# alazarteka/Self-Forcing

Hardware: AMD Instinct MI355X
Metric: decoded frames/sec/node, Wan-1.3B 832x480 4-step AR rollout (higher is better)
Workload: dtype bf16

## Files before the change

include/sf_hip.h:

```cpp
#ifndef SF_HIP_H
#define SF_HIP_H

#include <stddef.h>
#include <stdint.h>

#ifdef __cplusplus
extern "C" {
#endif

#define SF_HIP_ABI_VERSION 10

int sf_abi_version(void);
const char* sf_last_error(void);

enum sf_epilogue {
  SF_EPI_BIAS = 0,
  SF_EPI_BIAS_GELU = 1,
  SF_EPI_BIAS_RESID = 2,
  SF_EPI_BIAS_GATE_RESID = 3,
  SF_EPI_F32 = 4
};

typedef struct sf_gemm_args {
  const void* a;
  const void* w;
  const void* bias;
  void* out;
  const void* resid;
  const void* gate_mod;
  const void* gate_e0;
  int64_t gate_group_stride;
  int32_t rows_per_group;
  int32_t M, N, K;
  int32_t lda, ldw, ldo, ldr;
  int32_t epilogue;
  int32_t batch;
  int64_t a_bstride, w_bstride, o_bstride, r_bstride;
  int32_t structure;
} sf_gemm_args;

enum sf_gemm_structure { SF_GEMM_AUTO = 0, SF_GEMM_T128 = 1 ,
                         SF_GEMM_PP256 = 2 ,
                         SF_GEMM_PP128 = 3 ,
                         SF_GEMM_PP224 = 4, SF_GEMM_PP192 = 5  };

int sf_gemm_bf16(const sf_gemm_args* args, void* stream);

#define SF_FP8_AMAX_PARTS 1024
int sf_quantize_fp8(const void* x, int ldx, int M, int K, int rows_per_segment, void* q_out, float* scale_out, void* stream);

int sf_gemm_fp8(const sf_gemm_args* args, const float* a_scale, int rows_per_segment, const float* w_scale, void* stream);

int sf_small_linear_fp8(const void* x, const void* w_q, const float* w_scale, const void* bias, void* out, int M, int N, int K,
                        int rows_per_segment, int act_in, int act_out, void* stream);

int sf_small_linear(const void* x, const void* w, const void* bias, void* out, int M, int N, int K,
                    int act_in, int act_out, void* stream);

int sf_sinusoid_embedding(const void* t, int t_is_int64, void* out, int n, int dim, void* stream);

int sf_layernorm_modulate(const void* x, void* out, int M, int C, float eps, const void* mod_shift,
                          const void* mod_scale, const void* e0_shift, const void* e0_scale,
                          int64_t e0_group_stride, int rows_per_group, void* stream);

int sf_layernorm_affine(const void* x, const void* weight, const void* bias, void* out, int M, int C,
                        float eps, void* stream);

int sf_rmsnorm(const void* x, int ldx, const void* weight, void* out, int ldo, int M, int C, float eps,
               void* stream);

int sf_qkv_norm_rope_cache(const void* qkv, const void* norm_q_w, const void* norm_k_w, void* q_out,
                           void* k_cache, void* v_cache, const float* rope_cos, const float* rope_sin,
                           int B, int f, int h, int w, int C, int num_heads, int64_t cache_tokens,
                           int write_start, int start_frame, float eps, void* stream);

int sf_kv_evict(void* cache, int B, int64_t cache_tokens, int row_elems, int sink, int evict, int keep,
                void* scratch, size_t scratch_bytes, void* stream);

int sf_attention(const void* q, const void* k, const void* v, void* out, int B, int H, int Lq, int Lk,
                 int64_t q_stride, int64_t q_bstride, int64_t kv_stride, int64_t kv_bstride,
                 int64_t o_stride, int64_t o_bstride, void* stream);

enum sf_attn_structure { SF_ATTN_AUTO = 0, SF_ATTN_R64 = 1, SF_ATTN_W8 = 2, SF_ATTN_W4 = 3 };
int sf_attention_ex(const void* q, const void* k, const void* v, void* out, int B, int H, int Lq, int Lk,
                    int64_t q_stride, int64_t q_bstride, int64_t kv_stride, int64_t kv_bstride,
                    int64_t o_stride, int64_t o_bstride, int structure, void* stream);

int sf_attention_fold(const void* q, const void* k, const void* v, void* out, int B, int H, int Lq, int Lk,
                      int64_t q_stride, int64_t q_bstride, int64_t kv_stride, int64_t kv_bstride,
                      int64_t o_stride, int64_t o_bstride, int structure, const int32_t* keys, const float* log2w,
                      void* stream);

int sf_attention_accum(const void* q, const void* k, const void* v, void* out, int B, int H, int Lq, int Lk,
                       int64_t q_stride, int64_t q_bstride, int64_t kv_stride, int64_t kv_bstride,
                       int64_t o_stride, int64_t o_bstride, int structure, void* stream);

int sf_cross_fold_scan(const void* const* ck_cache_host, const void* const* cv_cache_host, int layers, int B, int text_len,
                       int row_elems, int32_t* keys, float* log2w, void* stream);

int sf_patchify(const void* x, void* cols, int B, int F, int Cin, int H, int W, void* stream);

int sf_unpatchify_x0(const void* head_out, const void* xt, const void* timestep, int t_is_int64,
                     const float* sigmas, const float* timesteps, int n_table, void* flow, void* x0,
                     int B, int F, int groups, int Cout, int H, int W, void* stream);

int sf_add_noise(const void* x0, const void* eps, const void* timestep, int t_is_int64,
                 const float* sigmas, const float* timesteps, int n_table, void* out, int n_outer,
                 int64_t inner, void* stream);

#define SF_LINCOMB_MAX 6
int sf_lincomb_bf16(void* out, const void* const* xs, const float* coefs, int n_terms, int64_t n, void* stream);

typedef struct sf_layer_weights {
  const void* modulation;
  const void *norm3_w, *norm3_b;
  const void *qkv_w, *qkv_b;
  const void *norm_q_w, *norm_k_w;
  const void *o_w, *o_b;
  const void *cq_w, *cq_b;
  const void *ckv_w, *ckv_b;
  const void *cnorm_q_w, *cnorm_k_w;
  const void *co_w, *co_b;
  const void *ffn0_w, *ffn0_b;
  const void *ffn2_w, *ffn2_b;
} sf_layer_weights;

typedef struct sf_model {
  int32_t dim, ffn_dim, num_heads, num_layers, in_dim, out_dim, freq_dim, text_dim, text_len;
  float eps;
  const void *patch_w, *patch_b;
  const void *text0_w, *text0_b, *text2_w, *text2_b;
  const void *time0_w, *time0_b, *time2_w, *time2_b;
  const void *tproj_w, *tproj_b;
  const void *head_w, *head_b;
  const void* head_mod;
  const void *pose_w, *pose_b;
  int32_t pose_dim;
  const sf_layer_weights* layers_host;
  const float *rope_cos, *rope_sin;
  const float *sched_sigmas, *sched_timesteps;
  int32_t n_table;
  int32_t fp8;
  const void *text0_q, *text2_q, *time0_q, *time2_q, *tproj_q, *head_q, *pose_q;
  const float *text0_s, *text2_s, *time0_s, *time2_s, *tproj_s, *head_s, *pose_s;
  const struct sf_layer_fp8* layers_fp8_host;
} sf_model;

typedef struct sf_layer_fp8 {
  const void *qkv_q, *o_q, *cq_q, *ckv_q, *co_q, *ffn0_q, *ffn2_q;
  const float *qkv_s, *o_s, *cq_s, *ckv_s, *co_s, *ffn0_s, *ffn2_s;
} sf_layer_fp8;

typedef struct sf_forward_args {
  int32_t batch, frames, lat_h, lat_w;
  int32_t groups;
  const void* noisy;
  const void* timestep;
  int32_t t_is_int64;
  const void* prompt_embeds;
  int32_t init_cross;
  const void* add_condition;
  void* const* k_cache_host;
  void* const* v_cache_host;
  void* const* ck_cache_host;
  void* const* cv_cache_host;
  int64_t cache_tokens;
  int32_t sink_tokens, evict, keep;
  int32_t write_start;
  int32_t attn_start, attn_end;
  int32_t start_frame;
  void* evict_scratch;
  size_t evict_scratch_bytes;
  int32_t cache_only;
  void* flow_out;
  void* x0_out;
  void* workspace;
  size_t workspace_bytes;
  void* kv_index_out;
  int64_t global_end;
} sf_forward_args;

size_t sf_dit_workspace_bytes(const sf_model* model, int batch, int frames, int lat_h, int lat_w,
                              int groups);
int sf_dit_forward(const sf_model* model, const sf_forward_args* args, void* stream);
int sf_dit_forward_pair(const sf_model* model, const sf_forward_args* context_pass, const sf_forward_args* next_pass,
                        void* stream);
int sf_dit_forward_fold(const sf_model* model, const sf_forward_args* args, int32_t* cross_keys, float* cross_log2w,
                        void* stream);
int sf_dit_forward_pair_fold(const sf_model* model, const sf_forward_args* context_pass, const sf_forward_args* next_pass,
                             const int32_t* cross_keys, const float* cross_log2w, void* stream);


int sf_patchify_i2v(const void* x, const void* y, void* cols, int B, int F, int x_channels, int y_channels, int pad_channels,
                    int H, int W, int64_t y_bstride, int64_t y_cstride, int64_t y_fstride, void* stream);

int sf_layernorm_rows(const void* x, const void* weight, const void* bias, void* out, int M, int C, float eps, void* stream);

int sf_i2v_assemble_y(const void* latent, const void* ref_map, void* y, int frames, int mask_channels, int latent_channels, int h, int w,
                      int64_t y_cstride, int64_t y_fstride, int first_is_frame0, void* stream);

typedef struct sf_i2v_layer {
  const void *kvimg_w, *kvimg_b;
  const void* norm_k_img_w;
} sf_i2v_layer;

typedef struct sf_i2v_model {
  int32_t clip_dim, clip_len;
  float img_eps;
  const void *img_ln0_w, *img_ln0_b;
  const void *img_fc1_w, *img_fc1_b;
  const void *img_fc2_w, *img_fc2_b;
  const void *img_ln1_w, *img_ln1_b;
  const sf_i2v_layer* layers_host;
} sf_i2v_model;

typedef struct sf_i2v_args {
  const void* clip_feature;
  const void* y;
  int64_t y_bstride, y_cstride, y_fstride;
  int32_t y_channels;
  void* const* kimg_cache_host;
  void* const* vimg_cache_host;
} sf_i2v_args;

size_t sf_dit_i2v_workspace_bytes(const sf_model* model, const sf_i2v_model* i2v_model, int batch, int frames, int lat_h,
                                  int lat_w, int groups);
int sf_dit_forward_i2v(const sf_model* model, const sf_i2v_model* i2v_model, const sf_forward_args* args, const sf_i2v_args* i2v_args,
                       int32_t* cross_keys, float* cross_log2w, void* stream);


enum sf_conv_epilogue {
  SF_CONV_BIAS = 0,
  SF_CONV_BIAS_RESID = 1,
  SF_CONV_BIAS_CLAMP_F32 = 2
};

typedef struct sf_conv_args {
  const void* x;
  const void* w;
  const void* bias;
  void* out;
  const void* resid;
  float* out_f32;
  int32_t Tout, H, W;
  int32_t Hin, Win;
  int32_t Cin, Cout;
  int32_t kt, kh, kw;
  int32_t upsample;
  int32_t t_in_offset;
  int32_t ldw, ldo, ldr;
  int32_t out_frame_offset;
  int32_t interleave_c;
  int32_t epilogue;
  int32_t structure;
  void* norm_out;
  const void* norm_gamma;
  int32_t norm_ld, norm_frame_offset;
  int32_t stride_hw, stride_t;
} sf_conv_args;

enum sf_conv_structure { SF_CONV_AUTO = 0, SF_CONV_IGEMM = 1 ,
                         SF_CONV_HALO = 2  };

int sf_conv_igemm(const sf_conv_args* args, void* stream);
int sf_conv_pick_nt(int cout);

int sf_rmsnorm_silu_cl(const void* x, const void* gamma, void* out, int64_t rows, int C, int silu,
                       void* stream);

int sf_softmax_rows(const float* s, int64_t lds, void* p, int64_t ldp, int rows, int cols,
                    int cols_padded, float scale, void* stream);

int sf_vae_prepare_latent(const void* latent, const float* mean, const float* std, const void* conv2_w,
                          const void* conv2_b, void* out, int z, int h, int w, int c_pad, void* stream);

typedef struct sf_vae_conv {
  const void* w;
  const void* bias;
  int32_t cin, cout, kt, kh, kw, ldw;
} sf_vae_conv;

typedef struct sf_vae_resblock {
  const void* gamma1;
  const void* gamma2;
  sf_vae_conv conv1;
  sf_vae_conv conv2;
  sf_vae_conv shortcut;
} sf_vae_resblock;

#define SF_VAE_MAX_STAGES 4

typedef struct sf_vae_model {
  int32_t z_dim;
  int32_t n_stages;
  int32_t res_per_stage;
  int32_t temporal_up[SF_VAE_MAX_STAGES];
  const float* latent_mean;
  const float* latent_std;
  const void *conv2_w, *conv2_b;
  sf_vae_conv conv1;
  sf_vae_resblock mid0, mid2;
  const void* attn_gamma;
  const void *attn_qk_w, *attn_qk_b;
  const void *attn_v_w, *attn_v_b;
  const void *attn_proj_w, *attn_proj_b;
  const sf_vae_resblock* res_host;
  sf_vae_conv time_conv[SF_VAE_MAX_STAGES];
  sf_vae_conv up_conv[SF_VAE_MAX_STAGES];
  const void* head_gamma;
  sf_vae_conv head_conv;
} sf_vae_model;

size_t sf_vae_state_bytes(const sf_vae_model* model, int lat_h, int lat_w, int window_frames);
size_t sf_vae_scratch_bytes(const sf_vae_model* model, int lat_h, int lat_w, int window_frames);
int sf_vae_reset(const sf_vae_model* model, void* state, size_t state_bytes, int lat_h, int lat_w,
                 int window_frames, void* stream);
int sf_vae_decode_frames(const sf_vae_model* model, void* state, size_t state_bytes, void* scratch,
                         size_t scratch_bytes, const void* latent_frames, int lat_h, int lat_w, int window_frames,
                         int frame_index, int n_frames, int window, int history_at, float* pixels_out, void* stream);


int sf_vae_prepare_pixels(const void* pixels, int is_f32, int64_t c_stride, void* out, int T, int H, int W, int c_pad,
                          void* stream);

int sf_vae_finish_latent(const void* head_out, int ld_in, int cin, const void* conv1_w, int ld_w, const void* conv1_b,
                         const float* mean, const float* std, float* out, int T, int z, int h, int w, void* stream);

typedef struct sf_vae_encoder {
  int32_t z_dim;
  int32_t n_stages;
  int32_t res_per_stage;
  int32_t temporal_down[SF_VAE_MAX_STAGES];
  const float* latent_mean;
  const float* latent_std;
  const void *conv1_w, *conv1_b;
  sf_vae_conv in_conv;
  const sf_vae_resblock* res_host;
  sf_vae_conv down_conv[SF_VAE_MAX_STAGES];
  sf_vae_conv time_conv[SF_VAE_MAX_STAGES];
  sf_vae_resblock mid0, mid2;
  const void* attn_gamma;
  const void *attn_qk_w, *attn_qk_b;
  const void *attn_v_w, *attn_v_b;
  const void *attn_proj_w, *attn_proj_b;
// ... 284 lines not shown
```

self-forcing_amd/_lib.py:

```python
from __future__ import annotations

import ctypes as C
import os
import subprocess
from typing import Optional

os.environ.setdefault("ROC_SIGNAL_POOL_SIZE", "1024")

_HERE = os.path.dirname(os.path.abspath(__file__))
CSRC = os.path.join(_HERE, "csrc")
LIB_PATH = os.environ.get("SF_HIP_LIB") or os.path.join(CSRC, "libsf_hip.so")

ABI_VERSION = 10
FP8_AMAX_PARTS = 1024

EPI_BIAS, EPI_BIAS_GELU, EPI_BIAS_RESID, EPI_BIAS_GATE_RESID, EPI_F32 = 0, 1, 2, 3, 4
CONV_BIAS, CONV_BIAS_RESID, CONV_BIAS_CLAMP_F32 = 0, 1, 2
VAE_MAX_STAGES = 4
TAEHV_EPILOGUES = {"bias_relu": 0, "bias_resid_relu": 1, "plain": 2, "relu": 3, "head_f32": 4, "latent_f32": 5}
TAEHV_STAGES, TAEHV_BLOCKS = 3, 3
TAEHV_PIXEL_DTYPES = {"bfloat16": 0, "float32": 1}
POSE_DTYPES = {"uint8": 0, "float32": 1, "bfloat16": 2}
POSE_CONVS = 6
JPEG_SUBSAMPLINGS = {"420": 0, "444": 1}
JPEG_DTYPES = {"uint8": 0, "float32": 1, "bfloat16": 2}
JPEG_RANGES = {(-1, 1): 0, (0, 1): 1}
JPEG_STATUS = {1: "an interval outgrew its worst-case slot", 2: "a coefficient is outside the baseline range",
               4: "the files do not fit the output buffer"}
CLIP_DTYPES = {"float32": 0, "bfloat16": 1}
ACT_NONE, ACT_SILU, ACT_GELU = 0, 1, 2
ATTN_STRUCTURES = {"auto": 0, "r64": 1, "w8": 2, "w4": 3}
CONV_STRUCTURES = {"auto": 0, "igemm": 1, "halo": 2}
GEMM_STRUCTURES = {"auto": 0, "t128": 1, "pp256": 2, "pp128": 3, "pp224": 4, "pp192": 5}


class GemmArgs(C.Structure):
    _fields_ = [
        ("a", C.c_void_p), ("w", C.c_void_p), ("bias", C.c_void_p), ("out", C.c_void_p),
        ("resid", C.c_void_p), ("gate_mod", C.c_void_p), ("gate_e0", C.c_void_p),
        ("gate_group_stride", C.c_int64), ("rows_per_group", C.c_int32),
        ("M", C.c_int32), ("N", C.c_int32), ("K", C.c_int32),
        ("lda", C.c_int32), ("ldw", C.c_int32), ("ldo", C.c_int32), ("ldr", C.c_int32),
        ("epilogue", C.c_int32), ("batch", C.c_int32),
        ("a_bstride", C.c_int64), ("w_bstride", C.c_int64), ("o_bstride", C.c_int64), ("r_bstride", C.c_int64),
        ("structure", C.c_int32),
    ]


class LayerWeights(C.Structure):
    _fields_ = [(n, C.c_void_p) for n in (
        "modulation", "norm3_w", "norm3_b", "qkv_w", "qkv_b", "norm_q_w", "norm_k_w", "o_w", "o_b",
        "cq_w", "cq_b", "ckv_w", "ckv_b", "cnorm_q_w", "cnorm_k_w", "co_w", "co_b",
        "ffn0_w", "ffn0_b", "ffn2_w", "ffn2_b")]


class LayerFp8(C.Structure):
    _fields_ = [(n, C.c_void_p) for n in (
        "qkv_q", "o_q", "cq_q", "ckv_q", "co_q", "ffn0_q", "ffn2_q",
        "qkv_s", "o_s", "cq_s", "ckv_s", "co_s", "ffn0_s", "ffn2_s")]


FP8_MODEL_LINEARS = (("text0", ("text_embedding.0",)), ("text2", ("text_embedding.2",)), ("time0", ("time_embedding.0",)),
                     ("time2", ("time_embedding.2",)), ("tproj", ("time_projection.1",)), ("head", ("head.head",)),
                     ("pose", ("pose_proj",)))
FP8_LAYER_LINEARS = (("qkv", ("self_attn.q", "self_attn.k", "self_attn.v")), ("o", ("self_attn.o",)), ("cq", ("cross_attn.q",)),
                     ("ckv", ("cross_attn.k", "cross_attn.v")), ("co", ("cross_attn.o",)), ("ffn0", ("ffn.0",)), ("ffn2", ("ffn.2",)))


class Model(C.Structure):
    _fields_ = (
        [(n, C.c_int32) for n in ("dim", "ffn_dim", "num_heads", "num_layers", "in_dim", "out_dim",
                                  "freq_dim", "text_dim", "text_len")]
        + [("eps", C.c_float)]
        + [(n, C.c_void_p) for n in ("patch_w", "patch_b", "text0_w", "text0_b", "text2_w", "text2_b",
                                     "time0_w", "time0_b", "time2_w", "time2_b", "tproj_w", "tproj_b",
                                     "head_w", "head_b", "head_mod", "pose_w", "pose_b")]
        + [("pose_dim", C.c_int32)]
        + [("layers_host", C.POINTER(LayerWeights)),
           ("rope_cos", C.c_void_p), ("rope_sin", C.c_void_p),
           ("sched_sigmas", C.c_void_p), ("sched_timesteps", C.c_void_p),
           ("n_table", C.c_int32)]
        + [("fp8", C.c_int32)]
        + [(n + "_q", C.c_void_p) for n, _ in FP8_MODEL_LINEARS]
        + [(n + "_s", C.c_void_p) for n, _ in FP8_MODEL_LINEARS]
        + [("layers_fp8_host", C.POINTER(LayerFp8))]
    )


class ForwardArgs(C.Structure):
    _fields_ = [
        ("batch", C.c_int32), ("frames", C.c_int32), ("lat_h", C.c_int32), ("lat_w", C.c_int32),
        ("groups", C.c_int32),
        ("noisy", C.c_void_p), ("timestep", C.c_void_p), ("t_is_int64", C.c_int32),
        ("prompt_embeds", C.c_void_p), ("init_cross", C.c_int32), ("add_condition", C.c_void_p),
        ("k_cache_host", C.POINTER(C.c_void_p)), ("v_cache_host", C.POINTER(C.c_void_p)),
        ("ck_cache_host", C.POINTER(C.c_void_p)), ("cv_cache_host", C.POINTER(C.c_void_p)),
        ("cache_tokens", C.c_int64),
        ("sink_tokens", C.c_int32), ("evict", C.c_int32), ("keep", C.c_int32),
        ("write_start", C.c_int32), ("attn_start", C.c_int32), ("attn_end", C.c_int32),
        ("start_frame", C.c_int32),
        ("evict_scratch", C.c_void_p), ("evict_scratch_bytes", C.c_size_t),
        ("cache_only", C.c_int32),
        ("flow_out", C.c_void_p), ("x0_out", C.c_void_p),
        ("workspace", C.c_void_p), ("workspace_bytes", C.c_size_t),
        ("kv_index_out", C.c_void_p), ("global_end", C.c_int64),
    ]


class I2VLayer(C.Structure):
    _fields_ = [(n, C.c_void_p) for n in ("kvimg_w", "kvimg_b", "norm_k_img_w")]


class I2VModel(C.Structure):
    _fields_ = ([("clip_dim", C.c_int32), ("clip_len", C.c_int32), ("img_eps", C.c_float)]
                + [(n, C.c_void_p) for n in ("img_ln0_w", "img_ln0_b", "img_fc1_w", "img_fc1_b", "img_fc2_w", "img_fc2_b",
                                             "img_ln1_w", "img_ln1_b")]
                + [("layers_host", C.POINTER(I2VLayer))])


class I2VArgs(C.Structure):
    _fields_ = [("clip_feature", C.c_void_p), ("y", C.c_void_p),
                ("y_bstride", C.c_int64), ("y_cstride", C.c_int64), ("y_fstride", C.c_int64), ("y_channels", C.c_int32),
                ("kimg_cache_host", C.POINTER(C.c_void_p)), ("vimg_cache_host", C.POINTER(C.c_void_p))]


class ConvArgs(C.Structure):
    _fields_ = (
        [(n, C.c_void_p) for n in ("x", "w", "bias", "out", "resid", "out_f32")]
        + [(n, C.c_int32) for n in ("Tout", "H", "W", "Hin", "Win", "Cin", "Cout", "kt", "kh", "kw", "upsample",
                                    "t_in_offset", "ldw", "ldo", "ldr", "out_frame_offset", "interleave_c", "epilogue", "structure")]
        + [("norm_out", C.c_void_p), ("norm_gamma", C.c_void_p), ("norm_ld", C.c_int32), ("norm_frame_offset", C.c_int32)]
        + [("stride_hw", C.c_int32), ("stride_t", C.c_int32)]
    )


class VaeConv(C.Structure):
    _fields_ = [("w", C.c_void_p), ("bias", C.c_void_p)] + [(n, C.c_int32) for n in ("cin", "cout", "kt", "kh", "kw", "ldw")]


class VaeResBlock(C.Structure):
    _fields_ = [("gamma1", C.c_void_p), ("gamma2", C.c_void_p), ("conv1", VaeConv), ("conv2", VaeConv), ("shortcut", VaeConv)]


class VaeModel(C.Structure):
    _fields_ = [
        ("z_dim", C.c_int32), ("n_stages", C.c_int32), ("res_per_stage", C.c_int32),
        ("temporal_up", C.c_int32 * VAE_MAX_STAGES),
        ("latent_mean", C.c_void_p), ("latent_std", C.c_void_p), ("conv2_w", C.c_void_p), ("conv2_b", C.c_void_p),
        ("conv1", VaeConv), ("mid0", VaeResBlock), ("mid2", VaeResBlock),
        ("attn_gamma", C.c_void_p), ("attn_qk_w", C.c_void_p), ("attn_qk_b", C.c_void_p),
        ("attn_v_w", C.c_void_p), ("attn_v_b", C.c_void_p), ("attn_proj_w", C.c_void_p), ("attn_proj_b", C.c_void_p),
        ("res_host", C.POINTER(VaeResBlock)),
        ("time_conv", VaeConv * VAE_MAX_STAGES), ("up_conv", VaeConv * VAE_MAX_STAGES),
        ("head_gamma", C.c_void_p), ("head_conv", VaeConv),
    ]


class VaeEncoder(C.Structure):
    _fields_ = [
        ("z_dim", C.c_int32), ("n_stages", C.c_int32), ("res_per_stage", C.c_int32),
        ("temporal_down", C.c_int32 * VAE_MAX_STAGES),
        ("latent_mean", C.c_void_p), ("latent_std", C.c_void_p), ("conv1_w", C.c_void_p), ("conv1_b", C.c_void_p),
        ("in_conv", VaeConv), ("res_host", C.POINTER(VaeResBlock)),
        ("down_conv", VaeConv * VAE_MAX_STAGES), ("time_conv", VaeConv * VAE_MAX_STAGES),
        ("mid0", VaeResBlock), ("mid2", VaeResBlock),
        ("attn_gamma", C.c_void_p), ("attn_qk_w", C.c_void_p), ("attn_qk_b", C.c_void_p),
        ("attn_v_w", C.c_void_p), ("attn_v_b", C.c_void_p), ("attn_proj_w", C.c_void_p), ("attn_proj_b", C.c_void_p),
        ("head_gamma", C.c_void_p), ("head_conv", VaeConv),
    ]


class TaehvConvArgs(C.Structure):
    _fields_ = ([(n, C.c_void_p) for n in ("x", "w", "bias", "out", "resid", "out_f32")]
                + [(n, C.c_int32) for n in ("Tout", "H", "W", "Cin", "Cout", "kt", "upsample", "ldw", "ldo", "ldr", "tgrow", "epilogue", "clamp")])


class TaehvLayer(C.Structure):
    _fields_ = [("w", C.c_void_p), ("bias", C.c_void_p)] + [(n, C.c_int32) for n in ("cin", "cout", "kt", "ldw")]


class TaehvModel(C.Structure):
    _fields_ = [("z_dim", C.c_int32), ("in_conv", TaehvLayer), ("block", ((TaehvLayer * 3) * TAEHV_BLOCKS) * TAEHV_STAGES),
                ("exit_conv", TaehvLayer * TAEHV_STAGES), ("tgrow", C.c_int32 * TAEHV_STAGES), ("head", TaehvLayer)]


class TaehvDownConvArgs(C.Structure):
    _fields_ = ([(n, C.c_void_p) for n in ("x", "w", "out")]
                + [(n, C.c_int32) for n in ("Tout", "H", "W", "Cin", "Cout", "kt", "ldw", "ldo")])


class TaehvEncoder(C.Structure):
    _fields_ = [("stem", TaehvLayer), ("down", TaehvLayer * TAEHV_STAGES), ("block", ((TaehvLayer * 3) * TAEHV_BLOCKS) * TAEHV_STAGES),
                ("head", TaehvLayer)]


class PoseConvArgs(C.Structure):
    _fields_ = ([(n, C.c_void_p) for n in ("x", "w", "bias", "out")]
                + [(n, C.c_int32) for n in ("T", "H", "W", "Cin", "Cout", "kt", "stride_t", "stride_s", "ldw", "ldo", "silu")])


class PoseWindow(C.Structure):
    _fields_ = [(n, C.c_int32) for n in ("x_t0", "t_end", "closed", "t_out0", "n_out")]


class PosePushPlan(C.Structure):
    _fields_ = [("first", C.c_int32 * (POSE_CONVS + 1)), ("count", C.c_int32 * (POSE_CONVS + 1))]


class PoseLayer(C.Structure):
    _fields_ = [("w", C.c_void_p), ("bias", C.c_void_p)] + [(n, C.c_int32) for n in ("cin", "cout", "kt", "stride_t", "stride_s", "ldw", "silu")]


class PoseModel(C.Structure):
    _fields_ = [("conv", PoseLayer * POSE_CONVS), ("embed_w", C.c_void_p), ("embed_b", C.c_void_p), ("pose_dim", C.c_int32),
                ("ref_conv", PoseLayer * POSE_CONVS)]


class T5Layer(C.Structure):
    _fields_ = [(n, C.c_void_p) for n in ("norm1_w", "qk_w", "v_w", "o_w", "norm2_w", "gate_w", "fc1_w", "fc2_w", "pos_emb")]


class T5Model(C.Structure):
    _fields_ = ([(n, C.c_int32) for n in ("vocab", "dim", "dim_attn", "dim_ffn", "num_heads", "num_layers", "num_buckets")]
                + [("eps", C.c_float), ("token_embedding", C.c_void_p), ("layers_host", C.POINTER(T5Layer)),
                   ("final_norm_w", C.c_void_p)])


class ClipLayer(C.Structure):
    _fields_ = [(n, C.c_void_p) for n in ("norm1_w", "norm1_b", "qkv_w", "qkv_b", "proj_w", "proj_b", "norm2_w", "norm2_b",
                                          "fc1_w", "fc1_b", "fc2_w", "fc2_b")]


class ClipModel(C.Structure):
    _fields_ = ([(n, C.c_int32) for n in ("image_size", "patch", "dim", "heads", "mlp_dim", "layers_built")]
                + [("eps", C.c_float)]
                + [(n, C.c_void_p) for n in ("patch_w", "cls", "pos", "pre_norm_w", "pre_norm_b")]
                + [("layers_host", C.POINTER(ClipLayer))])


_vp, _i, _i64, _f, _sz = C.c_void_p, C.c_int, C.c_int64, C.c_float, C.c_size_t
SIGNATURES = {
    "sf_abi_version": (C.c_int, []),
    "sf_last_error": (C.c_char_p, []),
    "sf_gemm_bf16": (C.c_int, [C.POINTER(GemmArgs), _vp]),
    "sf_small_linear": (C.c_int, [_vp, _vp, _vp, _vp, _i, _i, _i, _i, _i, _vp]),
    "sf_quantize_fp8": (C.c_int, [_vp, _i, _i, _i, _i, _vp, _vp, _vp]),
    "sf_gemm_fp8": (C.c_int, [C.POINTER(GemmArgs), _vp, _i, _vp, _vp]),
    "sf_small_linear_fp8": (C.c_int, [_vp, _vp, _vp, _vp, _vp, _i, _i, _i, _i, _i, _i, _vp]),
    "sf_sinusoid_embedding": (C.c_int, [_vp, _i, _vp, _i, _i, _vp]),
    "sf_layernorm_modulate": (C.c_int, [_vp, _vp, _i, _i, _f, _vp, _vp, _vp, _vp, _i64, _i, _vp]),
    "sf_layernorm_affine": (C.c_int, [_vp, _vp, _vp, _vp, _i, _i, _f, _vp]),
    "sf_rmsnorm": (C.c_int, [_vp, _i, _vp, _vp, _i, _i, _i, _f, _vp]),
    "sf_qkv_norm_rope_cache": (C.c_int, [_vp, _vp, _vp, _vp, _vp, _vp, _vp, _vp, _i, _i, _i, _i, _i, _i, _i64,
                                         _i, _i, _f, _vp]),
    "sf_kv_evict": (C.c_int, [_vp, _i, _i64, _i, _i, _i, _i, _vp, _sz, _vp]),
    "sf_attention": (C.c_int, [_vp, _vp, _vp, _vp, _i, _i, _i, _i, _i64, _i64, _i64, _i64, _i64, _i64, _vp]),
    "sf_attention_ex": (C.c_int, [_vp, _vp, _vp, _vp, _i, _i, _i, _i, _i64, _i64, _i64, _i64, _i64, _i64, _i, _vp]),
    "sf_attention_fold": (C.c_int, [_vp, _vp, _vp, _vp, _i, _i, _i, _i, _i64, _i64, _i64, _i64, _i64, _i64, _i, _vp, _vp, _vp]),
    "sf_attention_accum": (C.c_int, [_vp, _vp, _vp, _vp, _i, _i, _i, _i, _i64, _i64, _i64, _i64, _i64, _i64, _i, _vp]),
    "sf_cross_fold_scan": (C.c_int, [C.POINTER(C.c_void_p), C.POINTER(C.c_void_p), _i, _i, _i, _i, _vp, _vp, _vp]),
    "sf_patchify": (C.c_int, [_vp, _vp, _i, _i, _i, _i, _i, _vp]),
    "sf_unpatchify_x0": (C.c_int, [_vp, _vp, _vp, _i, _vp, _vp, _i, _vp, _vp, _i, _i, _i, _i, _i, _i, _vp]),
    "sf_add_noise": (C.c_int, [_vp, _vp, _vp, _i, _vp, _vp, _i, _vp, _i, _i64, _vp]),
    "sf_lincomb_bf16": (C.c_int, [_vp, C.POINTER(C.c_void_p), C.POINTER(C.c_float), _i, _i64, _vp]),
    "sf_dit_workspace_bytes": (C.c_size_t, [C.POINTER(Model), _i, _i, _i, _i, _i]),
    "sf_dit_forward": (C.c_int, [C.POINTER(Model), C.POINTER(ForwardArgs), _vp]),
    "sf_dit_forward_pair": (C.c_int, [C.POINTER(Model), C.POINTER(ForwardArgs), C.POINTER(ForwardArgs), _vp]),
    "sf_dit_forward_fold": (C.c_int, [C.POINTER(Model), C.POINTER(ForwardArgs), _vp, _vp, _vp]),
    "sf_dit_forward_pair_fold": (C.c_int, [C.POINTER(Model), C.POINTER(ForwardArgs), C.POINTER(ForwardArgs), _vp, _vp, _vp]),
    "sf_patchify_i2v": (C.c_int, [_vp, _vp, _vp, _i, _i, _i, _i, _i, _i, _i, _i64, _i64, _i64, _vp]),
    "sf_layernorm_rows": (C.c_int, [_vp, _vp, _vp, _vp, _i, _i, _f, _vp]),
    "sf_i2v_assemble_y": (C.c_int, [_vp, _vp, _vp, _i, _i, _i, _i, _i, _i64, _i64, _i, _vp]),
    "sf_dit_i2v_workspace_bytes": (C.c_size_t, [C.POINTER(Model), C.POINTER(I2VModel), _i, _i, _i, _i, _i]),
    "sf_dit_forward_i2v": (C.c_int, [C.POINTER(Model), C.POINTER(I2VModel), C.POINTER(ForwardArgs), C.POINTER(I2VArgs), _vp, _vp, _vp]),
    "sf_conv_igemm": (C.c_int, [C.POINTER(ConvArgs), _vp]),
    "sf_conv_pick_nt": (C.c_int, [_i]),
    "sf_rmsnorm_silu_cl": (C.c_int, [_vp, _vp, _vp, _i64, _i, _i, _vp]),
    "sf_softmax_rows": (C.c_int, [_vp, _i64, _vp, _i64, _i, _i, _i, _f, _vp]),
    "sf_vae_prepare_latent": (C.c_int, [_vp, _vp, _vp, _vp, _vp, _vp, _i, _i, _i, _i, _vp]),
    "sf_vae_state_bytes": (C.c_size_t, [C.POINTER(VaeModel), _i, _i, _i]),
    "sf_vae_scratch_bytes": (C.c_size_t, [C.POINTER(VaeModel), _i, _i, _i]),
    "sf_vae_reset": (C.c_int, [C.POINTER(VaeModel), _vp, _sz, _i, _i, _i, _vp]),
    "sf_vae_decode_frames": (C.c_int, [C.POINTER(VaeModel), _vp, _sz, _vp, _sz, _vp, _i, _i, _i, _i, _i, _i, _i, _vp, _vp]),
    "sf_vae_prepare_pixels": (C.c_int, [_vp, _i, _i64, _vp, _i, _i, _i, _i, _vp]),
    "sf_vae_finish_latent": (C.c_int, [_vp, _i, _i, _vp, _i, _vp, _vp, _vp, _vp, _i, _i, _i, _i, _vp]),
    "sf_vae_encode_state_bytes": (C.c_size_t, [C.POINTER(VaeEncoder), _i, _i, _i]),
    "sf_vae_encode_scratch_bytes": (C.c_size_t, [C.POINTER(VaeEncoder), _i, _i, _i]),
    "sf_vae_encode_reset": (C.c_int, [C.POINTER(VaeEncoder), _vp, _sz, _i, _i, _i, _vp]),
    "sf_vae_encode_frames": (C.c_int, [C.POINTER(VaeEncoder), _vp, _sz, _vp, _sz, _vp, _i, _i64, _i, _i, _i, _i, _i, _i, _i, _vp,
                                       _vp]),
    "sf_taehv_conv": (C.c_int, [C.POINTER(TaehvConvArgs), _vp]),
    "sf_taehv_pick_nt": (C.c_int, [_i]),
    "sf_taehv_prepare_latent": (C.c_int, [_vp, _vp, _i, _i, _i, _i, _i, _vp]),
    "sf_taehv_state_bytes": (C.c_size_t, [C.POINTER(TaehvModel), _i, _i]),
    "sf_taehv_scratch_bytes": (C.c_size_t, [C.POINTER(TaehvModel), _i, _i, _i]),
    "sf_taehv_reset": (C.c_int, [C.POINTER(TaehvModel), _vp, _sz, _i, _i, _vp]),
    "sf_taehv_decode_frames": (C.c_int, [C.POINTER(TaehvModel), _vp, _sz, _vp, _sz, _vp, _i, _i, _i, _i, _vp, _vp]),
    "sf_taehv_encode_stem": (C.c_int, [_vp, _i, _i64, _i, _i, _i, _i, _vp, _vp, _vp, _vp]),
    "sf_taehv_down_conv": (C.c_int, [C.POINTER(TaehvDownConvArgs), _vp]),
    "sf_taehv_encode_state_bytes": (C.c_size_t, [C.POINTER(TaehvEncoder), _i, _i]),
    "sf_taehv_encode_scratch_bytes": (C.c_size_t, [C.POINTER(TaehvEncoder), _i, _i, _i]),
    "sf_taehv_encode_reset": (C.c_int, [C.POINTER(TaehvEncoder), _vp, _sz, _i, _i, _vp]),
    "sf_taehv_encode_frames": (C.c_int, [C.POINTER(TaehvEncoder), _vp, _sz, _vp, _sz, _vp, _i, _i64, _i, _i, _i, _i, _vp, _vp]),
    "sf_pose_out_size": (C.c_int, [_i, _i, _i]),
    "sf_pose_conv": (C.c_int, [C.POINTER(PoseConvArgs), _vp]),
    "sf_pose_conv_window": (C.c_int, [C.POINTER(PoseConvArgs), C.POINTER(PoseWindow), _vp]),
    "sf_pose_prepare": (C.c_int, [_vp, _i, _i, _i, _i, _i, _i, _vp, _vp]),
    "sf_pose_patch_embed": (C.c_int, [_vp, _i, _i, _i, _vp, _vp, _i, _vp, _vp, _vp]),
    "sf_pose_scratch_bytes": (C.c_size_t, [C.POINTER(PoseModel), _i, _i, _i]),
    "sf_pose_embed": (C.c_int, [C.POINTER(PoseModel), _vp, _i, _i, _i, _i, _vp, _sz, _vp, _i64, _vp]),
    "sf_pose_embed_ref": (C.c_int, [C.POINTER(PoseModel), _vp, _i, _i, _i, _vp, _sz, _vp, _vp]),
    "sf_pose_stream_plan": (C.c_int, [_i, _i, _i, C.POINTER(PosePushPlan)]),
    "sf_pose_stream_state_bytes": (C.c_size_t, [C.POINTER(PoseModel), _i, _i]),
    "sf_pose_stream_scratch_bytes": (C.c_size_t, [C.POINTER(PoseModel), _i, _i, _i]),
    "sf_pose_stream_push": (C.c_int, [C.POINTER(PoseModel), _vp, _i, _vp, _i, _i, _i, _i, _i, _vp, _sz, _vp, _i64, C.POINTER(C.c_int32), _vp]),
    "sf_jpeg_workspace_bytes": (C.c_size_t, [_i, _i, _i, _i, _i]),
    "sf_jpeg_transform": (C.c_int, [_vp, _i, _i, _i, _i, _i, _i, _i, _vp, _vp]),
    "sf_jpeg_entropy": (C.c_int, [_vp, _i, _i, _i, _i, _i, _i, _vp, _sz, _vp, _sz, _vp, _vp, _vp]),
    "sf_jpeg_encode_frames": (C.c_int, [_vp, _i, _i, _i, _i, _i, _i, _i, _i, _vp, _sz, _vp, _sz, _vp, _vp, _vp]),
    "sf_embedding_gather": (C.c_int, [_vp, _vp, _vp, _i, _i, _i, _vp]),
    "sf_t5_softmax_bias": (C.c_int, [_vp, _vp, _vp, _vp, _vp, _i, _i, _i, _vp]),
    "sf_mul_bf16": (C.c_int, [_vp, _vp, _vp, _i64, _vp]),
    "sf_zero_masked_rows": (C.c_int, [_vp, _vp, _i, _i, _vp]),
    "sf_t5_workspace_bytes": (C.c_size_t, [C.POINTER(T5Model), _i, _i]),
    "sf_t5_encode": (C.c_int, [C.POINTER(T5Model), _vp, _vp, _vp, _i, _i, _vp, _vp, _sz, _vp]),
    "sf_clip_preprocess": (C.c_int, [_vp, _i, _i, _i, _i, _i, _i, _i, _vp, _vp]),
    "sf_clip_embed_norm": (C.c_int, [_vp, _vp, _vp, _vp, _vp, _vp, _vp, _vp, _vp, _i, _i, _i, _f, _vp]),
    "sf_clip_add_layernorm": (C.c_int, [_vp, _vp, _vp, _vp, _vp, _i, _i, _f, _vp]),
    "sf_clip_attention": (C.c_int, [_vp, _vp, _i, _i, _i, _vp]),
    "sf_clip_gelu": (C.c_int, [_vp, _vp, _i64, _vp]),
    "sf_clip_workspace_bytes": (C.c_size_t, [C.POINTER(ClipModel), _i]),
    "sf_clip_encode": (C.c_int, [C.POINTER(ClipModel), _vp, _i, _i, _i, _i, _vp, _vp, _sz, _vp]),
    "sf_probe_mfma": (C.c_int, [_i, _i, _i, _vp, _vp, C.POINTER(C.c_double), _vp]),
    "sf_probe_copy": (C.c_int, [_vp, _vp, _sz, _vp]),
}

_lib: Optional[C.CDLL] = None


class SfHipError(RuntimeError):
    pass


def build(verbose: bool = False) -> str:
    cmd = ["make", "-C", CSRC, "-j8"]
    res = subprocess.run(cmd, capture_output=True, text=True)
    if verbose or res.returncode != 0:
        print(res.stdout)
        print(res.stderr)
    if res.returncode != 0:
        raise SfHipError(f"building {LIB_PATH} failed (exit {res.returncode})")
    return LIB_PATH


def lib() -> C.CDLL:
    global _lib
    if _lib is not None:
        return _lib
    if not os.path.exists(LIB_PATH):
        raise SfHipError(
            f"{LIB_PATH} not found: the HIP extension is not built. Run "
            f"`python -c 'import __graft_entry__ as g; g.build()'` (or `make -C {CSRC}`). "
            "There is no CPU/eager fallback for this path.")
    handle = C.CDLL(LIB_PATH)
    for name, (res, args) in SIGNATURES.items():
        fn = getattr(handle, name)
        fn.restype = res
        fn.argtypes = args
    ver = handle.sf_abi_version()
    if ver != ABI_VERSION:
        raise SfHipError(f"{LIB_PATH}: ABI version {ver}, expected {ABI_VERSION}; rebuild")
    _lib = handle
    return handle


def check(rc: int, what: str = "") -> None:
    if rc != 0:
        msg = lib().sf_last_error()
        raise SfHipError(f"{what or 'sf_hip'} failed (rc={rc}): {msg.decode() if msg else '?'}")
```

self-forcing_amd/csrc/dit_forward.hip:

```cpp
#include <algorithm>
#include "sf_host.h"

int sf_internal_write_kv_indices(void* buf, int layers, int64_t global_end, int64_t local_end, void* stream);

namespace {

struct Work {
  void *x, *xn, *qkv, *q, *att, *hbuf, *cols, *headout, *sin, *etmp, *e, *e0, *ctx1, *ctx;
  void* xq;
  float* xs;
  size_t total;
};

constexpr int FP8_MAX_SEGMENTS = 8;

Work carve(const sf_model* m, void* ws, int B, int F, int lat_h, int lat_w, int groups) {
  const size_t M = (size_t)B * F * (lat_h / 2) * (lat_w / 2);
  const size_t C = m->dim, BG = (size_t)B * groups, T = (size_t)B * m->text_len;
  Carve c(ws);
  Work w;
  w.x = c.take(M * C * 2);
  w.xn = c.take(M * C * 2);
  w.qkv = c.take(M * 3 * C * 2);
  w.q = c.take(M * C * 2);
  w.att = c.take(M * C * 2);
  w.hbuf = c.take(M * (size_t)m->ffn_dim * 2);
  w.cols = c.take(M * (size_t)m->in_dim * 4 * 2);
  w.headout = c.take(M * (size_t)m->out_dim * 4 * 2);
  w.sin = c.take(BG * m->freq_dim * 2);
  w.etmp = c.take(BG * C * 2);
  w.e = c.take(BG * C * 2);
  w.e0 = c.take(BG * 6 * C * 2);
  w.ctx1 = c.take(T * C * 2);
  w.ctx = c.take(T * C * 2);
  w.xq = nullptr;
  w.xs = nullptr;
  if (m->fp8) {
    const size_t pose = m->pose_dim > 0 ? (size_t)m->pose_dim : C;
    const size_t widest_tok = std::max({(size_t)m->ffn_dim, C, pose}), widest_txt = std::max((size_t)m->text_dim, C);
    w.xq = c.take(std::max(M * widest_tok, T * widest_txt));
    w.xs = (float*)c.take(FP8_MAX_SEGMENTS * (1 + SF_FP8_AMAX_PARTS) * sizeof(float));
  }
  w.total = c.off;
  return w;
}

inline const char* bptr(const void* p, size_t elems) { return (const char*)p + elems * 2; }

struct I2V {
  const sf_i2v_model* m;
  const sf_i2v_args* a;
};
struct ImgWork {
  void *t0, *t1, *ctx;
  size_t total;
};
ImgWork carve_img(const sf_model* m, const sf_i2v_model* im, void* ws, size_t base, int B) {
  const size_t R = (size_t)B * im->clip_len;
  Carve c(ws);
  c.off = base;
  ImgWork w;
  w.t0 = c.take(R * im->clip_dim * 2);
  w.t1 = c.take(R * im->clip_dim * 2);
  w.ctx = c.take(2 * R * (size_t)m->dim * 2);
  w.total = c.off;
  return w;
}

}

extern "C" size_t sf_dit_workspace_bytes(const sf_model* model, int batch, int frames, int lat_h, int lat_w, int groups) {
  if (!model || batch <= 0 || frames <= 0 || lat_h <= 0 || lat_w <= 0 || groups <= 0) return 0;
  return carve(model, nullptr, batch, frames, lat_h, lat_w, groups).total;
}

static int forward_passes(const sf_model* m, const sf_forward_args* const* ps, int np, int32_t* cross_keys, float* cross_log2w, void* stream,
                          const I2V* iv = nullptr) {
  SF_CHECK((cross_keys == nullptr) == (cross_log2w == nullptr), "sf_dit_forward: cross_keys and cross_log2w come together");
  const sf_forward_args* a = ps[0];
  SF_CHECK(m && a, "sf_dit_forward: null argument");
  if (iv) {
    SF_CHECK(np == 1, "sf_dit_forward_i2v: the two-pass call is not built for the i2v model type");
    SF_CHECK(!m->fp8, "sf_dit_forward_i2v: fp8 Linears are not built for the i2v model type");
    SF_CHECK(iv->m->layers_host && iv->m->clip_len > 0 && iv->m->clip_dim > 0 && iv->m->clip_dim % 64 == 0,
             "sf_dit_forward_i2v: bad image context shape (clip_len=%d, clip_dim=%d: a positive multiple of 64)", iv->m->clip_len, iv->m->clip_dim);
    SF_CHECK(iv->a->y, "sf_dit_forward_i2v: y is missing (an i2v generator needs clip_feature and y)");
    SF_CHECK(m->in_dim >= m->out_dim + iv->a->y_channels && iv->a->y_channels > 0 && (m->in_dim * 4) % 64 == 0,
             "sf_dit_forward_i2v: %d latent + %d conditioning channels do not fit the padded in_dim %d", m->out_dim, iv->a->y_channels, m->in_dim);
    SF_CHECK(iv->a->kimg_cache_host && iv->a->vimg_cache_host, "sf_dit_forward_i2v: null image cache table");
    SF_CHECK(!a->init_cross || iv->a->clip_feature, "sf_dit_forward_i2v: init_cross needs clip_feature");
  }
  SF_CHECK(m->layers_host && m->num_layers > 0, "sf_dit_forward: model has no layers");
  SF_CHECK(m->dim == m->num_heads * 128, "sf_dit_forward: head_dim must be 128 (dim=%d heads=%d)", m->dim, m->num_heads);
  SF_CHECK(a->batch > 0 && a->frames > 0 && a->groups > 0, "sf_dit_forward: empty input");
  SF_CHECK(a->lat_h % 2 == 0 && a->lat_w % 2 == 0, "sf_dit_forward: latent size must be even");
  const int B = a->batch, F = a->frames, h = a->lat_h / 2, w = a->lat_w / 2;
  const int L = F * h * w, M = B * L, C = m->dim, G = a->groups, BG = B * G;
  const int Mt = np * M, BGt = np * BG;
  SF_CHECK(F % G == 0, "sf_dit_forward: frames=%d not divisible by timestep groups=%d", F, G);
  const int rpg = L / G;
  SF_CHECK(BGt <= 32, "sf_dit_forward: passes*batch*groups=%d exceeds the small-linear limit of 32", BGt);
  int first_full = np;
  for (int p = 0; p < np; ++p) {
    const sf_forward_args* q = ps[p];
    SF_CHECK(q, "sf_dit_forward: null pass");
    SF_CHECK(q->batch == B && q->frames == F && q->lat_h == a->lat_h && q->lat_w == a->lat_w && q->groups == G,
             "sf_dit_forward: the passes of one call must share batch, frames, latent size and timestep groups");
    SF_CHECK(q->k_cache_host == a->k_cache_host && q->v_cache_host == a->v_cache_host && q->ck_cache_host == a->ck_cache_host &&
             q->cv_cache_host == a->cv_cache_host && q->cache_tokens == a->cache_tokens, "sf_dit_forward: the passes of one call must share their caches");
    SF_CHECK(q->noisy && q->timestep, "sf_dit_forward: null tensor");
    SF_CHECK(q->cache_only || (q->flow_out && q->x0_out), "sf_dit_forward: null output tensor");
    SF_CHECK(q->attn_start >= 0 && q->attn_end > q->attn_start && q->attn_end <= q->cache_tokens, "sf_dit_forward: bad attention window [%d, %d) of %lld",
             q->attn_start, q->attn_end, (long long)q->cache_tokens);
    SF_CHECK(q->write_start >= 0 && (int64_t)q->write_start + L <= q->cache_tokens,
             "sf_dit_forward: KV cache overflow: write_start=%d + %d new tokens > capacity %lld", q->write_start, L, (long long)q->cache_tokens);
    SF_CHECK(q->write_start + L == q->attn_end, "sf_dit_forward: the new tokens must end the attention window");
    if (q->evict > 0) SF_CHECK(q->evict_scratch && q->keep >= 0, "sf_dit_forward: eviction needs evict_scratch");
    SF_CHECK(np == 1 || !q->init_cross, "sf_dit_forward_pair: the cross-attention cache must be initialised by an earlier single pass");
    if (!q->cache_only && first_full == np) first_full = p;
    SF_CHECK(!(q->cache_only && first_full != np), "sf_dit_forward_pair: cache_only passes must come first");
  }
  SF_CHECK(a->k_cache_host && a->v_cache_host && a->ck_cache_host && a->cv_cache_host, "sf_dit_forward: null cache table");
  const Work ws = carve(m, a->workspace, np * B, F, a->lat_h, a->lat_w, G);
  const size_t ws_need = iv ? carve_img(m, iv->m, nullptr, ws.total, B).total : ws.total;
  SF_CHECK(a->workspace && a->workspace_bytes >= ws_need, "sf_dit_forward: workspace too small (%zu < %zu)", a->workspace_bytes, ws_need);
  SF_CHECK(!a->init_cross || a->prompt_embeds, "sf_dit_forward: init_cross needs prompt_embeds");

  const bool f8 = m->fp8 != 0;
  static const sf_layer_fp8 no_fp8 = {};
  SF_CHECK(!f8 || m->layers_fp8_host, "sf_dit_forward: fp8 model without per-layer fp8 weights");
  auto run = [&](const Gemm& g) -> int { return f8 ? g.fp8(ws.xq, ws.xs, stream) : g.bf16(stream); };
  auto lin = [&](const Gemm& g) -> int {
    if (f8) SF_TRY(sf_quantize_fp8(g.g.a, g.g.lda, g.g.M, g.g.K, g.rows_per_segment, ws.xq, ws.xs, stream));
    return run(g);
  };
  auto small = [&](const void* x, const void* w16, const void* w8, const float* s8, const void* bias, void* out, int N, int K, int act_in,
                   int act_out) -> int {
    if (!f8) return sf_small_linear(x, w16, bias, out, BGt, N, K, act_in, act_out, stream);
    return sf_small_linear_fp8(x, w8, s8, bias, out, BGt, N, K, BG, act_in, act_out, stream);
  };

  const int Kp = m->in_dim * 4, Nh = m->out_dim * 4;
  const long cache_b = (long)a->cache_tokens * C;
  const long ctx_b = (long)m->text_len * C;
  const sf_forward_args* last = ps[np - 1];
  auto finish_indices = [&]() -> int {
    if (last->kv_index_out) return sf_internal_write_kv_indices(last->kv_index_out, m->num_layers, last->global_end, last->attn_end, stream);
    return 0;
  };

  if (iv)
    SF_TRY(sf_patchify_i2v(a->noisy, iv->a->y, ws.cols, B, F, m->out_dim, iv->a->y_channels, m->in_dim, a->lat_h, a->lat_w, iv->a->y_bstride,
                           iv->a->y_cstride, iv->a->y_fstride, stream));
  else
    for (int p = 0; p < np; ++p)
      SF_TRY(sf_patchify(ps[p]->noisy, (void*)bptr(ws.cols, (size_t)p * M * Kp), B, F, m->in_dim, a->lat_h, a->lat_w, stream));
  SF_TRY(Gemm(ws.cols, Kp, m->patch_w, Kp, ws.x, C, Mt, C, Kp).bias(m->patch_b).bf16(stream));

  for (int p = 0; p < np; ++p) {
    if (!ps[p]->add_condition) continue;
    void* xp = (void*)bptr(ws.x, (size_t)p * M * C);
    if (m->pose_w || (f8 && m->pose_q)) {
      SF_CHECK(m->pose_dim > 0, "sf_dit_forward: pose_proj weights without pose_dim");
      SF_TRY(lin(Gemm(ps[p]->add_condition, m->pose_dim, m->pose_w, m->pose_dim, xp, C, M, C, m->pose_dim).bias(m->pose_b)
                     .epi(SF_EPI_BIAS_RESID).resid(xp, C).fp8w(m->pose_q, m->pose_s, M)));
    } else {
      SF_CHECK(m->pose_dim == C, "sf_dit_forward: add_condition without pose_proj weights needs pose_dim == dim (%d != %d)", m->pose_dim, C);
      const void* terms[2] = {xp, ps[p]->add_condition};
      const float ones[2] = {1.0f, 1.0f};
      SF_TRY(sf_lincomb_bf16(xp, terms, ones, 2, (int64_t)M * C, stream));
    }
  }

  for (int p = 0; p < np; ++p)
    SF_TRY(sf_sinusoid_embedding(ps[p]->timestep, ps[p]->t_is_int64, (void*)bptr(ws.sin, (size_t)p * BG * m->freq_dim), BG, m->freq_dim, stream));
  SF_TRY(small(ws.sin, m->time0_w, m->time0_q, m->time0_s, m->time0_b, ws.etmp, C, m->freq_dim, 0, 1));
  SF_TRY(small(ws.etmp, m->time2_w, m->time2_q, m->time2_s, m->time2_b, ws.e, C, C, 0, 0));
  SF_TRY(small(ws.e, m->tproj_w, m->tproj_q, m->tproj_s, m->tproj_b, ws.e0, 6 * C, C, 1, 0));

  if (a->init_cross) {
    const int T = B * m->text_len;
    SF_TRY(lin(Gemm(a->prompt_embeds, m->text_dim, m->text0_w, m->text_dim, ws.ctx1, C, T, C, m->text_dim).bias(m->text0_b).epi(SF_EPI_BIAS_GELU)
                   .fp8w(m->text0_q, m->text0_s, T)));
    SF_TRY(lin(Gemm(ws.ctx1, C, m->text2_w, C, ws.ctx, C, T, C, C).bias(m->text2_b).fp8w(m->text2_q, m->text2_s, T)));
    if (f8) SF_TRY(sf_quantize_fp8(ws.ctx, C, T, C, T, ws.xq, ws.xs, stream));
    for (int l = 0; l < m->num_layers; ++l) {
      const sf_layer_weights& lw = m->layers_host[l];
      const sf_layer_fp8& lq = f8 ? m->layers_fp8_host[l] : no_fp8;
      SF_TRY(run(Gemm(ws.ctx, C, lw.ckv_w, C, a->ck_cache_host[l], C, T, C, C).bias(lw.ckv_b).fp8w(lq.ckv_q, lq.ckv_s, T)));
      SF_TRY(sf_rmsnorm(a->ck_cache_host[l], C, lw.cnorm_k_w, a->ck_cache_host[l], C, T, C, m->eps, stream));
      SF_TRY(run(Gemm(ws.ctx, C, bptr(lw.ckv_w, (size_t)C * C), C, a->cv_cache_host[l], C, T, C, C).bias(bptr(lw.ckv_b, C))
                     .fp8w(f8 ? (const char*)lq.ckv_q + (size_t)C * C : nullptr, f8 ? lq.ckv_s + C : nullptr, T)));
    }
    if (cross_keys) SF_TRY(sf_cross_fold_scan(a->ck_cache_host, a->cv_cache_host, m->num_layers, B, m->text_len, C, cross_keys, cross_log2w, stream));
    if (iv) {
      const sf_i2v_model* im = iv->m;
      const ImgWork iw = carve_img(m, im, a->workspace, ws.total, B);
      const int R = B * im->clip_len, D = im->clip_dim;
      void* ctx_raw = iw.ctx;
      void* ctx_img = (void*)bptr(iw.ctx, (size_t)R * C);
      SF_TRY(sf_layernorm_rows(iv->a->clip_feature, im->img_ln0_w, im->img_ln0_b, iw.t0, R, D, im->img_eps, stream));
      SF_TRY(Gemm(iw.t0, D, im->img_fc1_w, D, iw.t1, D, R, D, D).bias(im->img_fc1_b).bf16(stream));
      SF_TRY(sf_clip_gelu(iw.t1, iw.t1, (int64_t)R * D, stream));
      SF_TRY(Gemm(iw.t1, D, im->img_fc2_w, D, ctx_raw, C, R, C, D).bias(im->img_fc2_b).bf16(stream));
      SF_TRY(sf_layernorm_affine(ctx_raw, im->img_ln1_w, im->img_ln1_b, ctx_img, R, C, im->img_eps, stream));
      for (int l = 0; l < m->num_layers; ++l) {
        const sf_i2v_layer& il = im->layers_host[l];
        SF_TRY(Gemm(ctx_img, C, il.kvimg_w, C, iv->a->kimg_cache_host[l], C, R, C, C).bias(il.kvimg_b).bf16(stream));
        SF_TRY(sf_rmsnorm(iv->a->kimg_cache_host[l], C, il.norm_k_img_w, iv->a->kimg_cache_host[l], C, R, C, m->eps, stream));
        SF_TRY(Gemm(ctx_img, C, bptr(il.kvimg_w, (size_t)C * C), C, iv->a->vimg_cache_host[l], C, R, C, C).bias(bptr(il.kvimg_b, C)).bf16(stream));
      }
    }
  }

  for (int l = 0; l < m->num_layers; ++l) {
    const sf_layer_weights& lw = m->layers_host[l];
    const sf_layer_fp8& lq = f8 ? m->layers_fp8_host[l] : no_fp8;
    const void* mod = lw.modulation;
    const bool last_layer = l == m->num_layers - 1;
    SF_TRY(sf_layernorm_modulate(ws.x, ws.xn, Mt, C, m->eps, bptr(mod, 0), bptr(mod, C), bptr(ws.e0, 0), bptr(ws.e0, C), 6L * C, rpg, stream));
    SF_TRY(lin(Gemm(ws.xn, C, lw.qkv_w, C, ws.qkv, 3 * C, Mt, 3 * C, C).bias(lw.qkv_b).fp8w(lq.qkv_q, lq.qkv_s, M)));
    for (int p = 0; p < np; ++p) {
      const sf_forward_args* q = ps[p];
      const size_t roff = (size_t)p * M;
      if (q->evict > 0) {
        SF_TRY(sf_kv_evict(q->k_cache_host[l], B, q->cache_tokens, C, q->sink_tokens, q->evict, q->keep, q->evict_scratch, q->evict_scratch_bytes, stream));
        SF_TRY(sf_kv_evict(q->v_cache_host[l], B, q->cache_tokens, C, q->sink_tokens, q->evict, q->keep, q->evict_scratch, q->evict_scratch_bytes, stream));
      }
      SF_TRY(sf_qkv_norm_rope_cache(bptr(ws.qkv, roff * 3 * C), lw.norm_q_w, lw.norm_k_w, (void*)bptr(ws.q, roff * C), q->k_cache_host[l], q->v_cache_host[l],
                                    m->rope_cos, m->rope_sin, B, F, h, w, C, m->num_heads, q->cache_tokens, q->write_start, q->start_frame, m->eps, stream));
      if (q->cache_only && last_layer) continue;
      SF_TRY(sf_attention(bptr(ws.q, roff * C), bptr(q->k_cache_host[l], (size_t)q->attn_start * C), bptr(q->v_cache_host[l], (size_t)q->attn_start * C),
                          (void*)bptr(ws.att, roff * C), B, m->num_heads, L, q->attn_end - q->attn_start, C, (long)L * C, C, cache_b, C, (long)L * C, stream));
    }
    const int p0 = last_layer ? first_full : 0;
    if (p0 == np) return finish_indices();
    const size_t r0 = (size_t)p0 * M;
    const int Mr = (np - p0) * M;
    void* x = (void*)bptr(ws.x, r0 * C);
    void* xn = (void*)bptr(ws.xn, r0 * C);
    void* qb = (void*)bptr(ws.q, r0 * C);
    void* att = (void*)bptr(ws.att, r0 * C);
    void* hb = (void*)bptr(ws.hbuf, r0 * m->ffn_dim);
    const void* e0r = bptr(ws.e0, (size_t)p0 * BG * 6 * C);
    SF_TRY(lin(Gemm(att, C, lw.o_w, C, x, C, Mr, C, C).bias(lw.o_b).epi(SF_EPI_BIAS_GATE_RESID).resid(x, C)
                   .gate(bptr(mod, 2 * (size_t)C), bptr(e0r, 2 * (size_t)C), 6L * C, rpg).fp8w(lq.o_q, lq.o_s, M)));
    SF_TRY(sf_layernorm_affine(x, lw.norm3_w, lw.norm3_b, xn, Mr, C, m->eps, stream));
    SF_TRY(lin(Gemm(xn, C, lw.cq_w, C, qb, C, Mr, C, C).bias(lw.cq_b).fp8w(lq.cq_q, lq.cq_s, M)));
    SF_TRY(sf_rmsnorm(qb, C, lw.cnorm_q_w, qb, C, Mr, C, m->eps, stream));
    for (int p = p0; p < np; ++p)
      SF_TRY(sf_attention_fold(bptr(ws.q, (size_t)p * M * C), a->ck_cache_host[l], a->cv_cache_host[l], (void*)bptr(ws.att, (size_t)p * M * C), B, m->num_heads, L,
                               m->text_len, C, (long)L * C, C, ctx_b, C, (long)L * C, SF_ATTN_AUTO, cross_keys ? cross_keys + (size_t)l * B : nullptr,
                               cross_keys ? cross_log2w + (size_t)l * B : nullptr, stream));
    if (iv)
      SF_TRY(sf_attention_accum(ws.q, iv->a->kimg_cache_host[l], iv->a->vimg_cache_host[l], ws.att, B, m->num_heads, L, iv->m->clip_len, C, (long)L * C,
                                C, (long)iv->m->clip_len * C, C, (long)L * C, SF_ATTN_AUTO, stream));
    SF_TRY(lin(Gemm(att, C, lw.co_w, C, x, C, Mr, C, C).bias(lw.co_b).epi(SF_EPI_BIAS_RESID).resid(x, C).fp8w(lq.co_q, lq.co_s, M)));
    SF_TRY(sf_layernorm_modulate(x, xn, Mr, C, m->eps, bptr(mod, 3 * (size_t)C), bptr(mod, 4 * (size_t)C), bptr(e0r, 3 * (size_t)C),
                                 bptr(e0r, 4 * (size_t)C), 6L * C, rpg, stream));
    SF_TRY(lin(Gemm(xn, C, lw.ffn0_w, C, hb, m->ffn_dim, Mr, m->ffn_dim, C).bias(lw.ffn0_b).epi(SF_EPI_BIAS_GELU).fp8w(lq.ffn0_q, lq.ffn0_s, M)));
    SF_TRY(lin(Gemm(hb, m->ffn_dim, lw.ffn2_w, m->ffn_dim, x, C, Mr, C, m->ffn_dim).bias(lw.ffn2_b).epi(SF_EPI_BIAS_GATE_RESID).resid(x, C)
                   .gate(bptr(mod, 5 * (size_t)C), bptr(e0r, 5 * (size_t)C), 6L * C, rpg).fp8w(lq.ffn2_q, lq.ffn2_s, M)));
  }

  {
    const size_t r0 = (size_t)first_full * M;
    const int Mr = (np - first_full) * M;
    const void* er = bptr(ws.e, (size_t)first_full * BG * C);
    SF_TRY(sf_layernorm_modulate(bptr(ws.x, r0 * C), (void*)bptr(ws.xn, r0 * C), Mr, C, m->eps, bptr(m->head_mod, 0), bptr(m->head_mod, C), er, er, (long)C, rpg, stream));
    SF_TRY(lin(Gemm(bptr(ws.xn, r0 * C), C, m->head_w, C, (void*)bptr(ws.headout, r0 * Nh), Nh, Mr, Nh, C).bias(m->head_b)
                   .fp8w(m->head_q, m->head_s, M)));
    for (int p = first_full; p < np; ++p)
      SF_TRY(sf_unpatchify_x0(bptr(ws.headout, (size_t)p * M * Nh), ps[p]->noisy, ps[p]->timestep, ps[p]->t_is_int64, m->sched_sigmas, m->sched_timesteps, m->n_table,
                              ps[p]->flow_out, ps[p]->x0_out, B, F, G, m->out_dim, a->lat_h, a->lat_w, stream));
  }
  return finish_indices();
}

extern "C" int sf_dit_forward(const sf_model* m, const sf_forward_args* a, void* stream) {
  SF_CHECK(m && a, "sf_dit_forward: null argument");
  const sf_forward_args* one[1] = {a};
  return forward_passes(m, one, 1, nullptr, nullptr, stream);
}

extern "C" int sf_dit_forward_fold(const sf_model* m, const sf_forward_args* a, int32_t* cross_keys, float* cross_log2w, void* stream) {
  SF_CHECK(m && a, "sf_dit_forward: null argument");
  const sf_forward_args* one[1] = {a};
  return forward_passes(m, one, 1, cross_keys, cross_log2w, stream);
}

extern "C" size_t sf_dit_i2v_workspace_bytes(const sf_model* model, const sf_i2v_model* i2v_model, int batch, int frames, int lat_h, int lat_w,
                                             int groups) {
  const size_t base = sf_dit_workspace_bytes(model, batch, frames, lat_h, lat_w, groups);
  if (!base || !i2v_model || i2v_model->clip_len <= 0 || i2v_model->clip_dim <= 0) return 0;
  return carve_img(model, i2v_model, nullptr, base, batch).total;
}

extern "C" int sf_dit_forward_i2v(const sf_model* m, const sf_i2v_model* im, const sf_forward_args* a, const sf_i2v_args* ia, int32_t* cross_keys,
                                  float* cross_log2w, void* stream) {
  SF_CHECK(m && im && a && ia, "sf_dit_forward_i2v: null argument");
  const sf_forward_args* one[1] = {a};
  const I2V iv = {im, ia};
  return forward_passes(m, one, 1, cross_keys, cross_log2w, stream, &iv);
}

extern "C" int sf_dit_forward_pair_fold(const sf_model* m, const sf_forward_args* context_pass, const sf_forward_args* next_pass,
                                        const int32_t* cross_keys, const float* cross_log2w, void* stream) {
  SF_CHECK(m && context_pass && next_pass, "sf_dit_forward_pair: null argument");
  SF_CHECK(context_pass->workspace == next_pass->workspace && context_pass->workspace_bytes == next_pass->workspace_bytes,
           "sf_dit_forward_pair: both passes name the same workspace (sized for 2 x batch)");
  const sf_forward_args* two[2] = {context_pass, next_pass};
  return forward_passes(m, two, 2, const_cast<int32_t*>(cross_keys), const_cast<float*>(cross_log2w), stream);
}

extern "C" int sf_dit_forward_pair(const sf_model* m, const sf_forward_args* context_pass, const sf_forward_args* next_pass, void* stream) {
  return sf_dit_forward_pair_fold(m, context_pass, next_pass, nullptr, nullptr, stream);
}
```

self-forcing_amd/csrc/elementwise.hip:

```cpp
#include "sf_common.h"
#include "../../include/sf_hip.h"

namespace {

constexpr int ROWS_PER_BLOCK = 4;

template <int NCH>
__device__ __forceinline__ void load_row(const bf16_t* row, int lane, float (&v)[NCH][8]) {
#pragma unroll
  for (int i = 0; i < NCH; ++i) {
    const bf16x8 t = *reinterpret_cast<const bf16x8*>(row + (i * 64 + lane) * 8);
#pragma unroll
    for (int j = 0; j < 8; ++j) v[i][j] = (float)t[j];
  }
}

template <int NCH>
__device__ __forceinline__ void ln_stats(const float (&v)[NCH][8], int C, float eps, float& mean, float& rstd) {
  float s = 0.f;
#pragma unroll
  for (int i = 0; i < NCH; ++i)
#pragma unroll
    for (int j = 0; j < 8; ++j) s += v[i][j];
  mean = wave_sum(s) / (float)C;
  float q = 0.f;
#pragma unroll
  for (int i = 0; i < NCH; ++i)
#pragma unroll
    for (int j = 0; j < 8; ++j) {
      const float d = v[i][j] - mean;
      q += d * d;
    }
  rstd = rsqrtf(wave_sum(q) / (float)C + eps);
}

#ifndef SF_LN_RPW
#define SF_LN_RPW 2
#endif
template <int NCH> struct LnRows { static constexpr int value = NCH <= 4 ? SF_LN_RPW : (NCH <= 6 ? 2 : 1); };
template <int NCH, int MODE>
__global__ __launch_bounds__(64) void layernorm_kernel(const bf16_t* __restrict__ x, bf16_t* __restrict__ out,
                                                       int M, int C, float eps, const bf16_t* __restrict__ p0,
                                                       const bf16_t* __restrict__ p1, const bf16_t* __restrict__ e0_shift,
                                                       const bf16_t* __restrict__ e0_scale, long e0_group_stride,
                                                       int rows_per_group) {
  constexpr int LN_RPW = LnRows<NCH>::value;
  const int lane = threadIdx.x;
  const int row0 = blockIdx.x * LN_RPW;
  bf16x8 raw[LN_RPW][NCH];
#pragma unroll
  for (int r = 0; r < LN_RPW; ++r) {
    const long row = min(row0 + r, M - 1);
#pragma unroll
    for (int i = 0; i < NCH; ++i) raw[r][i] = *reinterpret_cast<const bf16x8*>(x + row * C + (i * 64 + lane) * 8);
  }
  bf16x8 scl[NCH], add[NCH];
  int cur_group = -1;
#pragma unroll
  for (int r = 0; r < LN_RPW; ++r) {
    const int row = row0 + r;
    if (row >= M) break;
    const int grp = MODE == 0 ? row / rows_per_group : 0;
    if (grp != cur_group) {
      cur_group = grp;
      const long goff = (long)grp * e0_group_stride;
#pragma unroll
      for (int i = 0; i < NCH; ++i) {
        const int e = (i * 64 + lane) * 8;
        if (MODE == 0) {
          const bf16x8 ms = *reinterpret_cast<const bf16x8*>(p0 + e);
          const bf16x8 mc = *reinterpret_cast<const bf16x8*>(p1 + e);
          const bf16x8 es = *reinterpret_cast<const bf16x8*>(e0_shift + goff + e);
          const bf16x8 ec = *reinterpret_cast<const bf16x8*>(e0_scale + goff + e);
#pragma unroll
          for (int j = 0; j < 8; ++j) {
            add[i][j] = (bf16_t)((float)ms[j] + (float)es[j]);
            scl[i][j] = (bf16_t)((float)mc[j] + (float)ec[j]);
          }
        } else {
          scl[i] = *reinterpret_cast<const bf16x8*>(p0 + e);
          add[i] = *reinterpret_cast<const bf16x8*>(p1 + e);
        }
      }
    }
    float v[NCH][8];
#pragma unroll
    for (int i = 0; i < NCH; ++i)
#pragma unroll
      for (int j = 0; j < 8; ++j) v[i][j] = (float)raw[r][i][j];
    float mean, rstd;
    ln_stats<NCH>(v, C, eps, mean, rstd);
#pragma unroll
    for (int i = 0; i < NCH; ++i) {
      bf16x8 o;
#pragma unroll
      for (int j = 0; j < 8; ++j)
        o[j] = (bf16_t)((v[i][j] - mean) * rstd * (MODE == 0 ? 1.0f + (float)scl[i][j] : (float)scl[i][j]) + (float)add[i][j]);
      *reinterpret_cast<bf16x8*>(out + (long)row * C + (i * 64 + lane) * 8) = o;
    }
  }
}

template <int NCH>
__global__ __launch_bounds__(256) void rmsnorm_kernel(const bf16_t* __restrict__ x, int ldx, const bf16_t* __restrict__ w,
                                                      bf16_t* __restrict__ out, int ldo, int M, int C, float eps) {
  const int lane = threadIdx.x & 63;
  const int row = blockIdx.x * ROWS_PER_BLOCK + (threadIdx.x >> 6);
  if (row >= M) return;
  float v[NCH][8];
  load_row<NCH>(x + (long)row * ldx, lane, v);
  float q = 0.f;
#pragma unroll
  for (int i = 0; i < NCH; ++i)
#pragma unroll
    for (int j = 0; j < 8; ++j) q += v[i][j] * v[i][j];
  const float r = rsqrtf(wave_sum(q) / (float)C + eps);
#pragma unroll
  for (int i = 0; i < NCH; ++i) {
    const int e = (i * 64 + lane) * 8;
    const bf16x8 wt = *reinterpret_cast<const bf16x8*>(w + e);
    bf16x8 o;
#pragma unroll
    for (int j = 0; j < 8; ++j) o[j] = (bf16_t)((float)(bf16_t)(v[i][j] * r) * (float)wt[j]);
    *reinterpret_cast<bf16x8*>(out + (long)row * ldo + e) = o;
  }
}

template <int NCH>
__global__ __launch_bounds__(256) void qkv_norm_rope_cache_kernel(
    const bf16_t* __restrict__ qkv, const bf16_t* __restrict__ wq, const bf16_t* __restrict__ wk,
    bf16_t* __restrict__ q_out, bf16_t* __restrict__ k_cache, bf16_t* __restrict__ v_cache,
    const float* __restrict__ rope_cos, const float* __restrict__ rope_sin, int rows, int L, int hgt, int wid, int C,
    long cache_tokens, int write_start, int start_frame, float eps, int c0, int c1) {
  const int lane = threadIdx.x & 63;
  const int row = blockIdx.x * ROWS_PER_BLOCK + (threadIdx.x >> 6);
  if (row >= rows) return;
  const int b = row / L, t = row - b * L;
  const int fi = t / (hgt * wid), rem = t - fi * (hgt * wid);
  const int hi = rem / wid, wi = rem - hi * wid;
  const int pos_t = start_frame + fi;
  const bf16_t* src = qkv + (long)row * 3 * C;
  const long crow = ((long)b * cache_tokens + write_start + t) * C;

#pragma unroll
  for (int i = 0; i < NCH; ++i) {
    const int e = (i * 64 + lane) * 8;
    *reinterpret_cast<u32x4*>(v_cache + crow + e) = *reinterpret_cast<const u32x4*>(src + 2 * C + e);
  }

#pragma unroll
  for (int which = 0; which < 2; ++which) {
    float v[NCH][8];
    load_row<NCH>(src + which * C, lane, v);
    float q = 0.f;
#pragma unroll
    for (int i = 0; i < NCH; ++i)
#pragma unroll
      for (int j = 0; j < 8; ++j) q += v[i][j] * v[i][j];
    const float r = rsqrtf(wave_sum(q) / (float)C + eps);
    const bf16_t* wn = which ? wk : wq;
    bf16_t* dst = which ? (k_cache + crow) : (q_out + (long)row * C);
#pragma unroll
    for (int i = 0; i < NCH; ++i) {
      const int e = (i * 64 + lane) * 8;
      const bf16x8 wt = *reinterpret_cast<const bf16x8*>(wn + e);
      const int pair0 = (e & 127) >> 1;
      bf16x8 o;
#pragma unroll
      for (int pp = 0; pp < 4; ++pp) {
        const int pj = pair0 + pp;
        const int pos = pj < c0 ? pos_t : (pj < c0 + c1 ? hi : wi);
        const float cs = rope_cos[pos * 64 + pj];
        const float sn = rope_sin[pos * 64 + pj];
        const float re = (float)(bf16_t)((float)(bf16_t)(v[i][2 * pp] * r) * (float)wt[2 * pp]);
        const float im = (float)(bf16_t)((float)(bf16_t)(v[i][2 * pp + 1] * r) * (float)wt[2 * pp + 1]);
        o[2 * pp] = (bf16_t)(re * cs - im * sn);
        o[2 * pp + 1] = (bf16_t)(re * sn + im * cs);
      }
      *reinterpret_cast<bf16x8*>(dst + e) = o;
    }
  }
}

__global__ __launch_bounds__(256) void copy_rows_kernel(const char* __restrict__ src, long src_bstride,
                                                        char* __restrict__ dst, long dst_bstride, long bytes_per_batch) {
  const long n16 = bytes_per_batch >> 4;
  const char* s = src + (long)blockIdx.y * src_bstride;
  char* d = dst + (long)blockIdx.y * dst_bstride;
  for (long i = (long)blockIdx.x * blockDim.x + threadIdx.x; i < n16; i += (long)gridDim.x * blockDim.x)
    reinterpret_cast<u32x4*>(d)[i] = reinterpret_cast<const u32x4*>(s)[i];
}

__global__ __launch_bounds__(256) void patchify_kernel(const bf16_t* __restrict__ x, bf16_t* __restrict__ cols, long total,
                                                       int Cin, int H, int W) {
  const int h2 = H >> 1, w2 = W >> 1;
  for (long i = (long)blockIdx.x * blockDim.x + threadIdx.x; i < total; i += (long)gridDim.x * blockDim.x) {
    const int cch = (int)(i % Cin);
    long r = i / Cin;
    const int ww = (int)(r % w2); r /= w2;
    const int hh = (int)(r % h2);
    const long bf = r / h2;
    const bf16_t* s = x + ((bf * Cin + cch) * H + 2 * hh) * (long)W + 2 * ww;
    bf16x4 o;
    o[0] = s[0]; o[1] = s[1]; o[2] = s[W]; o[3] = s[W + 1];
    *reinterpret_cast<bf16x4*>(cols + ((bf * h2 + hh) * w2 + ww) * (long)(Cin * 4) + cch * 4) = o;
  }
}

__device__ __forceinline__ double block_sigma_lookup(double t, const float* __restrict__ sigmas,
                                                     const float* __restrict__ timesteps, int n_table) {
  __shared__ double s_val[4];
  __shared__ int s_idx[4];
  double best = 1e300;
  int bi = 0x7fffffff;
  for (int j = threadIdx.x; j < n_table; j += blockDim.x) {
    const double d = fabs((double)timesteps[j] - t);
    if (d < best) { best = d; bi = j; }
  }
#pragma unroll
  for (int o = 32; o > 0; o >>= 1) {
    const double ob = __shfl_xor(best, o, 64);
    const int oi = __shfl_xor(bi, o, 64);
    if (ob < best || (ob == best && oi < bi)) { best = ob; bi = oi; }
  }
  const int wv = threadIdx.x >> 6;
  if ((threadIdx.x & 63) == 0) { s_val[wv] = best; s_idx[wv] = bi; }
  __syncthreads();
  best = s_val[0]; bi = s_idx[0];
  for (int k = 1; k < (int)(blockDim.x >> 6); ++k)
    if (s_val[k] < best || (s_val[k] == best && s_idx[k] < bi)) { best = s_val[k]; bi = s_idx[k]; }
  return (double)sigmas[bi];
}

__device__ __forceinline__ bf16_t double_to_bf16(double d) {
  const float f = (float)d;
  const unsigned u = __float_as_uint(f);
  if (f != f) return __builtin_bit_cast(bf16_t, (unsigned short)((u >> 16) | 0x40u));
  return __builtin_bit_cast(bf16_t, (unsigned short)((u + 0x7FFFu + ((u >> 16) & 1u)) >> 16));
}

__device__ __forceinline__ double read_timestep(const void* t, int is_i64, long idx) {
  return is_i64 ? (double)reinterpret_cast<const long long*>(t)[idx] : (double)reinterpret_cast<const float*>(t)[idx];
}

__global__ __launch_bounds__(256) void unpatchify_x0_kernel(const bf16_t* __restrict__ head_out, const bf16_t* __restrict__ xt,
                                                            const void* __restrict__ timestep, int t_is_i64,
                                                            const float* __restrict__ sigmas, const float* __restrict__ timesteps,
                                                            int n_table, bf16_t* __restrict__ flow, bf16_t* __restrict__ x0,
                                                            int F, int groups, int Cout, int H, int W) {
#pragma clang fp contract(off)
  const int bf = blockIdx.y;
  const int b = bf / F, f = bf - b * F;
  const int grp = f / (F / groups);
  const double sigma = block_sigma_lookup(read_timestep(timestep, t_is_i64, (long)b * groups + grp), sigmas, timesteps, n_table);
  const int h2 = H >> 1, w2 = W >> 1;
  const int total = Cout * H * w2;
  for (int i = blockIdx.x * blockDim.x + threadIdx.x; i < total; i += gridDim.x * blockDim.x) {
    const int ww = i % w2;
    int r = i / w2;
    const int y = r % H;
    const int cch = r / H;
    const int hh = y >> 1, pq = y & 1;
    const long tok = ((long)bf * h2 + hh) * w2 + ww;
    const bf16_t* hs = head_out + tok * (4 * Cout) + (pq * 2) * Cout + cch;
    const long o = (((long)bf * Cout + cch) * H + y) * W + 2 * ww;
    const bf16_t f0 = hs[0], f1 = hs[Cout];
    bf16x2 fo; fo[0] = f0; fo[1] = f1;
    *reinterpret_cast<bf16x2*>(flow + o) = fo;
    const bf16x2 xv = *reinterpret_cast<const bf16x2*>(xt + o);
    bf16x2 xo;
    xo[0] = double_to_bf16((double)(float)xv[0] - sigma * (double)(float)f0);
    xo[1] = double_to_bf16((double)(float)xv[1] - sigma * (double)(float)f1);
    *reinterpret_cast<bf16x2*>(x0 + o) = xo;
  }
}

__global__ __launch_bounds__(256) void add_noise_kernel(const bf16_t* __restrict__ x0, const bf16_t* __restrict__ eps,
                                                        const void* __restrict__ timestep, int t_is_i64,
                                                        const float* __restrict__ sigmas, const float* __restrict__ timesteps,
                                                        int n_table, bf16_t* __restrict__ out, long inner) {
#pragma clang fp contract(off)
  const long base = (long)blockIdx.y * inner;
  const float sigma = (float)block_sigma_lookup(read_timestep(timestep, t_is_i64, blockIdx.y), sigmas, timesteps, n_table);
  const float om = 1.0f - sigma;
  const long n8 = inner >> 3;
  for (long i = (long)blockIdx.x * blockDim.x + threadIdx.x; i < n8; i += (long)gridDim.x * blockDim.x) {
    const bf16x8 a = *reinterpret_cast<const bf16x8*>(x0 + base + i * 8);
    const bf16x8 e = *reinterpret_cast<const bf16x8*>(eps + base + i * 8);
    bf16x8 o;
#pragma unroll
    for (int j = 0; j < 8; ++j) o[j] = (bf16_t)(om * (float)a[j] + sigma * (float)e[j]);
    *reinterpret_cast<bf16x8*>(out + base + i * 8) = o;
  }
}

struct LinCombP {
  const bf16_t* x[SF_LINCOMB_MAX];
  float c[SF_LINCOMB_MAX];
  bf16_t* out;
  long n8;
  int n_terms;
};
template <int NT>
__global__ __launch_bounds__(256) void lincomb_kernel(const LinCombP p) {
#pragma clang fp contract(off)
  for (long i = (long)blockIdx.x * blockDim.x + threadIdx.x; i < p.n8; i += (long)gridDim.x * blockDim.x) {
    float acc[8];
#pragma unroll
    for (int k = 0; k < NT; ++k) {
      const bf16x8 v = *reinterpret_cast<const bf16x8*>(p.x[k] + i * 8);
#pragma unroll
      for (int j = 0; j < 8; ++j) acc[j] = k == 0 ? p.c[0] * (float)v[j] : acc[j] + p.c[k] * (float)v[j];
    }
    bf16x8 o;
#pragma unroll
    for (int j = 0; j < 8; ++j) o[j] = (bf16_t)acc[j];
    *reinterpret_cast<bf16x8*>(p.out + i * 8) = o;
  }
}

__global__ __launch_bounds__(256) void sinusoid_kernel(const void* __restrict__ t, int t_is_i64, bf16_t* __restrict__ out,
                                                       int n, int dim) {
  const int half = dim >> 1;
  const int i = blockIdx.x * blockDim.x + threadIdx.x;
  if (i >= n * half) return;
  const int r = i / half, k = i - r * half;
  const double pos = read_timestep(t, t_is_i64, r);
  const double ang = pos * pow(10000.0, -(double)k / (double)half);
  out[(long)r * dim + k] = double_to_bf16(cos(ang));
  out[(long)r * dim + half + k] = double_to_bf16(sin(ang));
}

template <int MODE>
int launch_layernorm(const bf16_t* x, bf16_t* out, int M, int C, float eps, const bf16_t* p0, const bf16_t* p1,
                     const bf16_t* e0s, const bf16_t* e0c, long gs, int rpg, hipStream_t s) {
  const dim3 block(64);
  switch (C / 512) {
#define SF_LN_CASE(N) \
  case N: hipLaunchKernelGGL((layernorm_kernel<N, MODE>), dim3((M + LnRows<N>::value - 1) / LnRows<N>::value), block, 0, s, x, out, M, C, eps, p0, p1, e0s, e0c, gs, rpg); break;
    SF_LN_CASE(1) SF_LN_CASE(2) SF_LN_CASE(3) SF_LN_CASE(4) SF_LN_CASE(5) SF_LN_CASE(6) SF_LN_CASE(8) SF_LN_CASE(10)
#undef SF_LN_CASE
    default: sf_set_error("layernorm: unsupported channel count %d", C); return -1;
  }
  return 0;
}

bool channels_ok(int C) {
  if (C % 512 != 0) return false;
  const int n = C / 512;
  return n == 1 || n == 2 || n == 3 || n == 4 || n == 5 || n == 6 || n == 8 || n == 10;
}

}

extern "C" int sf_layernorm_modulate(const void* x, void* out, int M, int C, float eps, const void* mod_shift,
                                     const void* mod_scale, const void* e0_shift, const void* e0_scale,
                                     int64_t e0_group_stride, int rows_per_group, void* stream) {
  SF_CHECK(x && out && mod_shift && mod_scale && e0_shift && e0_scale, "sf_layernorm_modulate: null tensor");
  SF_CHECK(M > 0 && channels_ok(C), "sf_layernorm_modulate: unsupported shape M=%d C=%d (C must be 512*{1,2,3,4,5,6,8,10})", M, C);
  SF_CHECK(rows_per_group > 0 && e0_group_stride % 8 == 0, "sf_layernorm_modulate: bad group layout");
  if (launch_layernorm<0>((const bf16_t*)x, (bf16_t*)out, M, C, eps, (const bf16_t*)mod_shift, (const bf16_t*)mod_scale,
                          (const bf16_t*)e0_shift, (const bf16_t*)e0_scale, e0_group_stride, rows_per_group,
                          (hipStream_t)stream) != 0)
    return -1;
  SF_HIP_LAUNCH_CHECK("sf_layernorm_modulate");
  return 0;
}

extern "C" int sf_layernorm_affine(const void* x, const void* weight, const void* bias, void* out, int M, int C,
                                   float eps, void* stream) {
  SF_CHECK(x && out && weight && bias, "sf_layernorm_affine: null tensor");
  SF_CHECK(M > 0 && channels_ok(C), "sf_layernorm_affine: unsupported shape M=%d C=%d", M, C);
  if (launch_layernorm<1>((const bf16_t*)x, (bf16_t*)out, M, C, eps, (const bf16_t*)weight, (const bf16_t*)bias, nullptr,
                          nullptr, 0, 1, (hipStream_t)stream) != 0)
    return -1;
  SF_HIP_LAUNCH_CHECK("sf_layernorm_affine");
  return 0;
}

extern "C" int sf_rmsnorm(const void* x, int ldx, const void* weight, void* out, int ldo, int M, int C, float eps,
                          void* stream) {
  SF_CHECK(x && out && weight, "sf_rmsnorm: null tensor");
  SF_CHECK(M > 0 && channels_ok(C) && ldx >= C && ldo >= C && ldx % 8 == 0 && ldo % 8 == 0, "sf_rmsnorm: unsupported shape M=%d C=%d", M, C);
  const dim3 grid((M + ROWS_PER_BLOCK - 1) / ROWS_PER_BLOCK), block(256);
  hipStream_t s = (hipStream_t)stream;
  switch (C / 512) {
#define SF_RMS_CASE(N) \
  case N: hipLaunchKernelGGL((rmsnorm_kernel<N>), grid, block, 0, s, (const bf16_t*)x, ldx, (const bf16_t*)weight, (bf16_t*)out, ldo, M, C, eps); break;
    SF_RMS_CASE(1) SF_RMS_CASE(2) SF_RMS_CASE(3) SF_RMS_CASE(4) SF_RMS_CASE(5) SF_RMS_CASE(6) SF_RMS_CASE(8) SF_RMS_CASE(10)
#undef SF_RMS_CASE
  }
  SF_HIP_LAUNCH_CHECK("sf_rmsnorm");
  return 0;
}

extern "C" int sf_qkv_norm_rope_cache(const void* qkv, const void* norm_q_w, const void* norm_k_w, void* q_out,
                                      void* k_cache, void* v_cache, const float* rope_cos, const float* rope_sin,
                                      int B, int f, int h, int w, int C, int num_heads, int64_t cache_tokens,
                                      int write_start, int start_frame, float eps, void* stream) {
  SF_CHECK(qkv && norm_q_w && norm_k_w && q_out && k_cache && v_cache && rope_cos && rope_sin, "sf_qkv_norm_rope_cache: null tensor");
  SF_CHECK(B > 0 && f > 0 && h > 0 && w > 0 && channels_ok(C), "sf_qkv_norm_rope_cache: unsupported shape");
  SF_CHECK(num_heads > 0 && C == num_heads * 128, "sf_qkv_norm_rope_cache: head_dim must be 128 (C=%d heads=%d)", C, num_heads);
  const int L = f * h * w;
  SF_CHECK(write_start >= 0 && (int64_t)write_start + L <= cache_tokens, "sf_qkv_norm_rope_cache: cache overflow: write_start=%d + L=%d > capacity=%lld",
           write_start, L, (long long)cache_tokens);
  SF_CHECK(start_frame >= 0 && start_frame + f <= 1024 && h <= 1024 && w <= 1024, "sf_qkv_norm_rope_cache: RoPE position out of the 1024-entry table");
  const int rows = B * L;
  const dim3 grid((rows + ROWS_PER_BLOCK - 1) / ROWS_PER_BLOCK), block(256);
  hipStream_t s = (hipStream_t)stream;
  const int c = 64, c1 = c / 3, c0 = c - 2 * c1;
  switch (C / 512) {
#define SF_QKV_CASE(N)                                                                                                   \
  case N: hipLaunchKernelGGL((qkv_norm_rope_cache_kernel<N>), grid, block, 0, s, (const bf16_t*)qkv, (const bf16_t*)norm_q_w, \
                             (const bf16_t*)norm_k_w, (bf16_t*)q_out, (bf16_t*)k_cache, (bf16_t*)v_cache, rope_cos, rope_sin,  \
                             rows, L, h, w, C, (long)cache_tokens, write_start, start_frame, eps, c0, c1); break;
    SF_QKV_CASE(1) SF_QKV_CASE(2) SF_QKV_CASE(3) SF_QKV_CASE(4) SF_QKV_CASE(5) SF_QKV_CASE(6) SF_QKV_CASE(8) SF_QKV_CASE(10)
#undef SF_QKV_CASE
  }
  SF_HIP_LAUNCH_CHECK("sf_qkv_norm_rope_cache");
  return 0;
}

extern "C" int sf_kv_evict(void* cache, int B, int64_t cache_tokens, int row_elems, int sink, int evict, int keep,
                           void* scratch, size_t scratch_bytes, void* stream) {
  SF_CHECK(cache && B > 0 && row_elems > 0 && (row_elems % 8) == 0, "sf_kv_evict: bad arguments");
  SF_CHECK(sink >= 0 && evict >= 0 && keep >= 0 && (int64_t)sink + evict + keep <= cache_tokens, "sf_kv_evict: window out of range");
  if (evict == 0 || keep == 0) return 0;
  const long row_b = (long)row_elems * 2;
  const long bytes = (long)keep * row_b;
  SF_CHECK(scratch && scratch_bytes >= (size_t)(bytes * B), "sf_kv_evict: scratch too small (%zu < %ld)", scratch_bytes, bytes * B);
  char* base = (char*)cache;
  const long bstride = (long)cache_tokens * row_b;
  const int gx = (int)min((long)2048, (bytes / 16 + 255) / 256);
  const dim3 grid(gx, B), block(256);
  hipStream_t s = (hipStream_t)stream;
  hipLaunchKernelGGL(copy_rows_kernel, grid, block, 0, s, base + (long)(sink + evict) * row_b, bstride, (char*)scratch, bytes, bytes);
  hipLaunchKernelGGL(copy_rows_kernel, grid, block, 0, s, (const char*)scratch, bytes, base + (long)sink * row_b, bstride, bytes);
  SF_HIP_LAUNCH_CHECK("sf_kv_evict");
  return 0;
}

extern "C" int sf_patchify(const void* x, void* cols, int B, int F, int Cin, int H, int W, void* stream) {
  SF_CHECK(x && cols && B > 0 && F > 0 && Cin > 0, "sf_patchify: bad arguments");
  SF_CHECK(H % 2 == 0 && W % 2 == 0, "sf_patchify: latent H=%d W=%d must be even (patch 2x2)", H, W);
  const long total = (long)B * F * (H / 2) * (W / 2) * Cin;
  const int gx = (int)min((long)4096, (total + 255) / 256);
  hipLaunchKernelGGL(patchify_kernel, dim3(gx), dim3(256), 0, (hipStream_t)stream, (const bf16_t*)x, (bf16_t*)cols, total, Cin, H, W);
  SF_HIP_LAUNCH_CHECK("sf_patchify");
  return 0;
}

extern "C" int sf_unpatchify_x0(const void* head_out, const void* xt, const void* timestep, int t_is_int64,
                                const float* sigmas, const float* timesteps, int n_table, void* flow, void* x0,
                                int B, int F, int groups, int Cout, int H, int W, void* stream) {
  SF_CHECK(head_out && xt && timestep && sigmas && timesteps && flow && x0, "sf_unpatchify_x0: null tensor");
  SF_CHECK(B > 0 && F > 0 && groups > 0 && F % groups == 0, "sf_unpatchify_x0: frames=%d not divisible by groups=%d", F, groups);
  SF_CHECK(H % 2 == 0 && W % 2 == 0 && n_table > 0, "sf_unpatchify_x0: bad shape");
  const int total = Cout * H * (W / 2);
  const dim3 grid(min(64, (total + 255) / 256), B * F), block(256);
  hipLaunchKernelGGL(unpatchify_x0_kernel, grid, block, 0, (hipStream_t)stream, (const bf16_t*)head_out, (const bf16_t*)xt, timestep,
                     t_is_int64, sigmas, timesteps, n_table, (bf16_t*)flow, (bf16_t*)x0, F, groups, Cout, H, W);
  SF_HIP_LAUNCH_CHECK("sf_unpatchify_x0");
  return 0;
}

extern "C" int sf_add_noise(const void* x0, const void* eps, const void* timestep, int t_is_int64, const float* sigmas,
                            const float* timesteps, int n_table, void* out, int n_outer, int64_t inner, void* stream) {
  SF_CHECK(x0 && eps && timestep && sigmas && timesteps && out, "sf_add_noise: null tensor");
  SF_CHECK(n_outer > 0 && inner > 0 && inner % 8 == 0 && n_table > 0, "sf_add_noise: bad shape (inner must be a multiple of 8)");
  const dim3 grid((unsigned)min((long)64, (long)((inner / 8 + 255) / 256)), n_outer), block(256);
  hipLaunchKernelGGL(add_noise_kernel, grid, block, 0, (hipStream_t)stream, (const bf16_t*)x0, (const bf16_t*)eps, timestep, t_is_int64,
                     sigmas, timesteps, n_table, (bf16_t*)out, (long)inner);
  SF_HIP_LAUNCH_CHECK("sf_add_noise");
  return 0;
}

extern "C" int sf_lincomb_bf16(void* out, const void* const* xs, const float* coefs, int n_terms, int64_t n, void* stream) {
  SF_CHECK(out && xs && coefs, "sf_lincomb_bf16: null argument");
  SF_CHECK(n_terms >= 1 && n_terms <= SF_LINCOMB_MAX, "sf_lincomb_bf16: n_terms must be 1..%d, got %d", SF_LINCOMB_MAX, n_terms);
  SF_CHECK(n > 0 && n % 8 == 0, "sf_lincomb_bf16: element count must be a positive multiple of 8");
  LinCombP p;
  for (int k = 0; k < SF_LINCOMB_MAX; ++k) {
    p.x[k] = k < n_terms ? (const bf16_t*)xs[k] : nullptr;
    p.c[k] = k < n_terms ? coefs[k] : 0.0f;
    SF_CHECK(k >= n_terms || xs[k], "sf_lincomb_bf16: null input %d", k);
  }
  p.out = (bf16_t*)out;
  p.n8 = n / 8;
  p.n_terms = n_terms;
  const dim3 grid((unsigned)min((long)2048, (p.n8 + 255) / 256)), block(256);
  switch (n_terms) {
    case 1: hipLaunchKernelGGL(lincomb_kernel<1>, grid, block, 0, (hipStream_t)stream, p); break;
    case 2: hipLaunchKernelGGL(lincomb_kernel<2>, grid, block, 0, (hipStream_t)stream, p); break;
    case 3: hipLaunchKernelGGL(lincomb_kernel<3>, grid, block, 0, (hipStream_t)stream, p); break;
    case 4: hipLaunchKernelGGL(lincomb_kernel<4>, grid, block, 0, (hipStream_t)stream, p); break;
    case 5: hipLaunchKernelGGL(lincomb_kernel<5>, grid, block, 0, (hipStream_t)stream, p); break;
    default: hipLaunchKernelGGL(lincomb_kernel<6>, grid, block, 0, (hipStream_t)stream, p); break;
  }
  SF_HIP_LAUNCH_CHECK("sf_lincomb_bf16");
  return 0;
}

__global__ void kv_index_kernel(long long* __restrict__ buf, int layers, long long global_end, long long local_end) {
  const int i = blockIdx.x * blockDim.x + threadIdx.x;
  if (i < 2 * layers) buf[i] = (i & 1) ? local_end : global_end;
}
__attribute__((visibility("hidden"))) int sf_internal_write_kv_indices(void* buf, int layers, int64_t global_end, int64_t local_end, void* stream) {
  hipLaunchKernelGGL(kv_index_kernel, dim3((2 * layers + 63) / 64), dim3(64), 0, (hipStream_t)stream, (long long*)buf, layers,
                     (long long)global_end, (long long)local_end);
  SF_HIP_LAUNCH_CHECK("kv_index_kernel");
  return 0;
}

extern "C" int sf_sinusoid_embedding(const void* t, int t_is_int64, void* out, int n, int dim, void* stream) {
  SF_CHECK(t && out && n > 0 && dim > 0 && dim % 2 == 0, "sf_sinusoid_embedding: bad arguments");
  const int total = n * (dim / 2);
  hipLaunchKernelGGL(sinusoid_kernel, dim3((total + 255) / 256), dim3(256), 0, (hipStream_t)stream, t, t_is_int64, (bf16_t*)out, n, dim);
  SF_HIP_LAUNCH_CHECK("sf_sinusoid_embedding");
  return 0;
}

__global__ void fold_reset_kernel(int* __restrict__ keys, int n) {
  const int i = blockIdx.x * blockDim.x + threadIdx.x;
  if (i < n) keys[i] = -1;
}

__global__ __launch_bounds__(256) void fold_scan_kernel(const uint4* __restrict__ k, const uint4* __restrict__ v, int text_len, int row_chunks,
                                                        int* __restrict__ last_diff) {
  const int b = blockIdx.y, lane = threadIdx.x & 63;
  const int row = blockIdx.x * 4 + (threadIdx.x >> 6);
  if (row >= text_len - 1) return;
  const size_t slab = (size_t)b * text_len * row_chunks;
  const uint4* kr = k + slab + (size_t)row * row_chunks;
  const uint4* vr = v + slab + (size_t)row * row_chunks;
  const uint4* kl = k + slab + (size_t)(text_len - 1) * row_chunks;
  const uint4* vl = v + slab + (size_t)(text_len - 1) * row_chunks;
  unsigned diff = 0;
  for (int c = lane; c < row_chunks; c += 64) {
    const uint4 a = kr[c], al = kl[c], d = vr[c], dl = vl[c];
    diff |= (a.x ^ al.x) | (a.y ^ al.y) | (a.z ^ al.z) | (a.w ^ al.w) | (d.x ^ dl.x) | (d.y ^ dl.y) | (d.z ^ dl.z) | (d.w ^ dl.w);
  }
  if (__any(diff != 0) && lane == 0) atomicMax(last_diff + b, row);
}

__global__ void fold_finish_kernel(int* __restrict__ keys, float* __restrict__ log2w, int n, int text_len) {
  const int i = blockIdx.x * blockDim.x + threadIdx.x;
  if (i >= n) return;
  const int same = text_len - 1 - keys[i];
  keys[i] = text_len - same + 1;
  log2w[i] = log2f((float)same);
}

extern "C" int sf_cross_fold_scan(const void* const* ck_cache_host, const void* const* cv_cache_host, int layers, int B, int text_len,
                                  int row_elems, int32_t* keys, float* log2w, void* stream) {
  SF_CHECK(ck_cache_host && cv_cache_host && keys && log2w, "sf_cross_fold_scan: null argument");
  SF_CHECK(layers > 0 && B > 0 && text_len > 0 && row_elems > 0 && row_elems % 8 == 0, "sf_cross_fold_scan: bad shape layers=%d B=%d text_len=%d row=%d",
           layers, B, text_len, row_elems);
  hipStream_t s = (hipStream_t)stream;
  const int n = layers * B;
  hipLaunchKernelGGL(fold_reset_kernel, dim3((n + 255) / 256), dim3(256), 0, s, keys, n);
  if (text_len > 1)
    for (int l = 0; l < layers; ++l) {
      SF_CHECK(ck_cache_host[l] && cv_cache_host[l], "sf_cross_fold_scan: null cache of layer %d", l);
      SF_CHECK(((uintptr_t)ck_cache_host[l] | (uintptr_t)cv_cache_host[l]) % 16 == 0, "sf_cross_fold_scan: misaligned cache of layer %d", l);
      hipLaunchKernelGGL(fold_scan_kernel, dim3((text_len - 1 + 3) / 4, B), dim3(256), 0, s, (const uint4*)ck_cache_host[l],
                         (const uint4*)cv_cache_host[l], text_len, row_elems / 8, keys + (size_t)l * B);
    }
  hipLaunchKernelGGL(fold_finish_kernel, dim3((n + 255) / 256), dim3(256), 0, s, keys, log2w, n, text_len);
  SF_HIP_LAUNCH_CHECK("sf_cross_fold_scan");
  return 0;
}
```

self-forcing_amd/csrc/gemm_bf16.hip:

```cpp
#include <type_traits>
#include "sf_common.h"
#include "lds_dma.h"
#include "../../include/sf_hip.h"

namespace {

constexpr int BM = 128, BN = 128, BK = 64;
constexpr int GEMM_THREADS = 256;
constexpr int TILE_BYTES = BM * BK * 2;
constexpr int STAGE_BYTES = 2 * TILE_BYTES;
constexpr int GEMM_LDS = 2 * STAGE_BYTES;

struct GemmP {
  const bf16_t* a;
  const bf16_t* w;
  const bf16_t* bias;
  bf16_t* out;
  const bf16_t* resid;
  const bf16_t* gate_mod;
  const bf16_t* gate_e0;
  long gate_group_stride;
  int rows_per_group;
  int M, N, K, lda, ldw, ldo, ldr;
  int tiles_m, tiles_n;
  long a_bs, w_bs, o_bs, r_bs;
  const float* a_scale;
  const float* w_scale;
  int rows_per_seg;
};

typedef int i32x4 __attribute__((ext_vector_type(4)));
typedef int i32x8 __attribute__((ext_vector_type(8)));

__device__ __forceinline__ f32x4 mfma_f8(const bf16x8& w0, const bf16x8& w1, const bf16x8& x0, const bf16x8& x1, const f32x4& acc) {
  const i32x8 wv = __builtin_shufflevector(__builtin_bit_cast(i32x4, w0), __builtin_bit_cast(i32x4, w1), 0, 1, 2, 3, 4, 5, 6, 7);
  const i32x8 xv = __builtin_shufflevector(__builtin_bit_cast(i32x4, x0), __builtin_bit_cast(i32x4, x1), 0, 1, 2, 3, 4, 5, 6, 7);
  return __builtin_amdgcn_mfma_scale_f32_16x16x128_f8f6f4(wv, xv, acc, 0, 0, 0, 127, 0, 127);
}

template <int MT>
__device__ __forceinline__ void fp8_scale_acc(const GemmP& p, f32x4 (&acc)[MT][4], int m_base, int n_base, int lane) {
  f32x4 ws[4];
#pragma unroll
  for (int nt = 0; nt < 4; ++nt) ws[nt] = *reinterpret_cast<const f32x4*>(p.w_scale + min(n_base + nt * 16 + (lane >> 4) * 4, p.N - 4));
#pragma unroll
  for (int mt = 0; mt < MT; ++mt) {
    const float sa = p.a_scale[min(m_base + mt * 16 + (lane & 15), p.M - 1) / p.rows_per_seg];
#pragma unroll
    for (int nt = 0; nt < 4; ++nt)
#pragma unroll
      for (int j = 0; j < 4; ++j) acc[mt][nt][j] = acc[mt][nt][j] * (sa * ws[nt][j]);
  }
}

template <int EPI>
__device__ __forceinline__ bf16x4 epi_apply(const GemmP& p, const f32x4& a4, int m, int n, const bf16_t* e0row) {
  float y[4];
#pragma unroll
  for (int j = 0; j < 4; ++j) y[j] = a4[j];
  if (p.bias) {
    const bf16x4 b = *reinterpret_cast<const bf16x4*>(p.bias + n);
#pragma unroll
    for (int j = 0; j < 4; ++j) y[j] += (float)b[j];
  }
  if (EPI == SF_EPI_BIAS_GELU) {
#pragma unroll
    for (int j = 0; j < 4; ++j) y[j] = gelu_tanh_f(y[j]);
  }
  if (EPI == SF_EPI_BIAS_GATE_RESID) {
    const bf16x4 gm = *reinterpret_cast<const bf16x4*>(p.gate_mod + n);
    const bf16x4 ge = *reinterpret_cast<const bf16x4*>(e0row + n);
#pragma unroll
    for (int j = 0; j < 4; ++j) y[j] *= (float)(bf16_t)((float)gm[j] + (float)ge[j]);
  }
  if (EPI == SF_EPI_BIAS_RESID || EPI == SF_EPI_BIAS_GATE_RESID) {
    const bf16x4 rv = *reinterpret_cast<const bf16x4*>(p.resid + (long)m * p.ldr + n);
#pragma unroll
    for (int j = 0; j < 4; ++j) y[j] += (float)rv[j];
  }
  bf16x4 o;
#pragma unroll
  for (int j = 0; j < 4; ++j) o[j] = (bf16_t)y[j];
  return o;
}

template <int EPI, int MT>
__device__ __forceinline__ void gemm_epilogue(const GemmP& p, f32x4 (&acc)[MT][4], int mrow, int ncol) {
#pragma unroll
  for (int mt = 0; mt < MT; ++mt) {
    const int m = mrow + mt * 16;
    if (m >= p.M) continue;
    const bf16_t* e0row = nullptr;
    if (EPI == SF_EPI_BIAS_GATE_RESID) e0row = p.gate_e0 + (long)(m / p.rows_per_group) * p.gate_group_stride;
#pragma unroll
    for (int nt = 0; nt < 4; ++nt) {
      const int n = ncol + nt * 16;
      if (n >= p.N) continue;
      if (EPI == SF_EPI_F32) {
        *reinterpret_cast<f32x4*>(reinterpret_cast<float*>(p.out) + (long)m * p.ldo + n) = acc[mt][nt];
        continue;
      }
      *reinterpret_cast<bf16x4*>(p.out + (long)m * p.ldo + n) = epi_apply<EPI>(p, acc[mt][nt], m, n, e0row);
    }
  }
}

template <int EPI>
__device__ __forceinline__ bf16x4 epi_math(const f32x4& a4, const bf16x4& b, const bf16x4& gm, const bf16x4& ge, const bf16x4& rv) {
  float y[4];
#pragma unroll
  for (int j = 0; j < 4; ++j) y[j] = a4[j] + (float)b[j];
  if (EPI == SF_EPI_BIAS_GELU) {
#pragma unroll
    for (int j = 0; j < 4; ++j) y[j] = gelu_tanh_f(y[j]);
  }
  if (EPI == SF_EPI_BIAS_GATE_RESID) {
#pragma unroll
    for (int j = 0; j < 4; ++j) y[j] *= (float)(bf16_t)((float)gm[j] + (float)ge[j]);
  }
  if (EPI == SF_EPI_BIAS_RESID || EPI == SF_EPI_BIAS_GATE_RESID) {
#pragma unroll
    for (int j = 0; j < 4; ++j) y[j] += (float)rv[j];
  }
  bf16x4 o;
#pragma unroll
  for (int j = 0; j < 4; ++j) o[j] = (bf16_t)y[j];
  return o;
}

template <int EPI, int MT>
__device__ __forceinline__ void gemm_epilogue_lds(const GemmP& p, f32x4 (&acc)[MT][4], int m_base, int n_base, char* wbuf, int lane) {
  const int r16 = lane & 15, cg = lane >> 4;
  constexpr bool GATE = EPI == SF_EPI_BIAS_GATE_RESID;
  constexpr bool RESID = EPI == SF_EPI_BIAS_RESID || EPI == SF_EPI_BIAS_GATE_RESID;
  const bf16x4 zero4 = {(bf16_t)0.f, (bf16_t)0.f, (bf16_t)0.f, (bf16_t)0.f};
  int ncol[4];
  bf16x4 bias_v[4], gm_v[4];
#pragma unroll
  for (int nt = 0; nt < 4; ++nt) {
    ncol[nt] = min(n_base + nt * 16 + cg * 4, p.N - 4);
    bias_v[nt] = zero4;
    gm_v[nt] = zero4;
  }
  if (p.bias) {
#pragma unroll
    for (int nt = 0; nt < 4; ++nt) bias_v[nt] = *reinterpret_cast<const bf16x4*>(p.bias + ncol[nt]);
  }
  if (GATE) {
#pragma unroll
    for (int nt = 0; nt < 4; ++nt) gm_v[nt] = *reinterpret_cast<const bf16x4*>(p.gate_mod + ncol[nt]);
  }
  constexpr int MB = 4;
#pragma unroll
  for (int m0 = 0; m0 < MT; m0 += MB) {
    bf16x4 rv[MB][4], ge[MB][4];
#pragma unroll
    for (int i = 0; i < MB; ++i) {
      if (m0 + i >= MT) break;
      const int m = min(m_base + (m0 + i) * 16 + r16, p.M - 1);
      const bf16_t* e0row = GATE ? p.gate_e0 + (long)(m / p.rows_per_group) * p.gate_group_stride : nullptr;
#pragma unroll
      for (int nt = 0; nt < 4; ++nt) {
        rv[i][nt] = RESID ? *reinterpret_cast<const bf16x4*>(p.resid + (long)m * p.ldr + ncol[nt]) : zero4;
        ge[i][nt] = GATE ? *reinterpret_cast<const bf16x4*>(e0row + ncol[nt]) : zero4;
      }
    }
#pragma unroll
    for (int i = 0; i < MB; ++i) {
      if (m0 + i >= MT) break;
      const int row = (m0 + i) * 16 + r16;
#pragma unroll
      for (int nt = 0; nt < 4; ++nt) {
        const int col = nt * 16 + cg * 4;
        const bf16x4 o = epi_math<EPI>(acc[m0 + i][nt], bias_v[nt], gm_v[nt], ge[i][nt], rv[i][nt]);
        const int chunk = (col >> 3) ^ (row & 7);
        *reinterpret_cast<bf16x4*>(wbuf + row * 128 + (chunk << 4) + (col & 4) * 2) = o;
      }
    }
  }
  __builtin_amdgcn_s_waitcnt(0xc07f);
  const int rr = lane >> 3, ch = lane & 7;
#pragma unroll
  for (int i = 0; i < 2 * MT; ++i) {
    const int row = i * 8 + rr;
    const int m = m_base + row, n = n_base + ch * 8;
    const bf16x8 v = *reinterpret_cast<const bf16x8*>(wbuf + row * 128 + ((ch ^ (row & 7)) << 4));
    if (m < p.M && n < p.N) *reinterpret_cast<bf16x8*>(p.out + (long)m * p.ldo + n) = v;
  }
}

template <int EPI, bool F8>
__global__ __launch_bounds__(GEMM_THREADS, 2) void gemm_bf16_kernel(GemmP p) {
  extern __shared__ __attribute__((aligned(16))) char smem[];
  const int tid = threadIdx.x;
  const int lane = tid & 63;
  const int wave = __builtin_amdgcn_readfirstlane(tid >> 6);

  if (blockIdx.y) {
    const long bz = blockIdx.y;
    p.a += bz * p.a_bs; p.w += bz * p.w_bs;
    if (EPI == SF_EPI_F32) p.out = reinterpret_cast<bf16_t*>(reinterpret_cast<float*>(p.out) + bz * p.o_bs); else p.out += bz * p.o_bs;
    if (p.resid) p.resid += bz * p.r_bs;
  }
  const int nwg = gridDim.x, bid = blockIdx.x;
  const int wg = sf_xcd_remap(bid, nwg);
  constexpr int GROUP_M = 8;
  const int width = GROUP_M * p.tiles_n;
  const int group = wg / width, first_m = group * GROUP_M;
  const int gsz = min(p.tiles_m - first_m, GROUP_M);
  const int in_group = wg - group * width;
  const int tm = first_m + in_group % gsz, tn = in_group / gsz;
  const int m0 = tm * BM, n0 = tn * BN;

  const bf16_t* a_src[4];
  const bf16_t* w_src[4];
#pragma unroll
  for (int i = 0; i < 4; ++i) {
    const int r = (wave * 4 + i) * 8 + (lane >> 3);
    const int c = (lane & 7) ^ ((r >> 1) & 7);
    const int am = min(m0 + r, p.M - 1);
    const int wn = min(n0 + r, p.N - 1);
    a_src[i] = p.a + (long)am * p.lda + c * 8;
    w_src[i] = p.w + (long)wn * p.ldw + c * 8;
  }
  auto stage = [&](int buf, int kt) {
    char* base = smem + buf * STAGE_BYTES + wave * 4096;
    const int k0 = kt * BK;
#pragma unroll
    for (int i = 0; i < 4; ++i) glds16(a_src[i] + k0, base + i * 1024);
#pragma unroll
    for (int i = 0; i < 4; ++i) glds16(w_src[i] + k0, base + TILE_BYTES + i * 1024);
  };

  const int wr = wave >> 1, wc = wave & 1;
  const int i16 = lane & 15, kq = lane >> 4;
  const int swz = (i16 >> 1) & 7;
  const int x_row_off = (wr * 64 + i16) * 128;
  const int w_row_off = TILE_BYTES + (wc * 64 + i16) * 128;
  const int coff0 = ((0 + kq) ^ swz) << 4;
  const int coff1 = ((4 + kq) ^ swz) << 4;

  f32x4 acc[4][4];
#pragma unroll
  for (int i = 0; i < 4; ++i)
#pragma unroll
    for (int j = 0; j < 4; ++j) acc[i][j] = f32x4{0.f, 0.f, 0.f, 0.f};

  const int nk = p.K / BK;
  stage(0, 0);
  __builtin_amdgcn_s_waitcnt(0);
  __syncthreads();

  for (int kt = 0; kt < nk; ++kt) {
    const int cur = kt & 1;
    const char* buf = smem + cur * STAGE_BYTES;
    const int kn = min(kt + 1, nk - 1) * BK;
    char* sbase = smem + (cur ^ 1) * STAGE_BYTES + wave * 4096;
    bf16x8 xf0[4], wf0[4], xf1[4], wf1[4];
    if constexpr (F8) {
#pragma unroll
      for (int t = 0; t < 4; ++t) {
        xf0[t] = *reinterpret_cast<const bf16x8*>(buf + x_row_off + t * 2048 + coff0);
        wf0[t] = *reinterpret_cast<const bf16x8*>(buf + w_row_off + t * 2048 + coff0);
        xf1[t] = *reinterpret_cast<const bf16x8*>(buf + x_row_off + t * 2048 + coff1);
        wf1[t] = *reinterpret_cast<const bf16x8*>(buf + w_row_off + t * 2048 + coff1);
      }
      __builtin_amdgcn_sched_barrier(0);
#pragma unroll
      for (int i = 0; i < 8; ++i) {
        const int mt = i >> 1, nt0 = (i & 1) * 2;
        acc[mt][nt0] = mfma_f8(wf0[nt0], wf1[nt0], xf0[mt], xf1[mt], acc[mt][nt0]);
        acc[mt][nt0 + 1] = mfma_f8(wf0[nt0 + 1], wf1[nt0 + 1], xf0[mt], xf1[mt], acc[mt][nt0 + 1]);
        if (i < 4) glds16(a_src[i] + kn, sbase + i * 1024);
        else glds16(w_src[i - 4] + kn, sbase + TILE_BYTES + (i - 4) * 1024);
        __builtin_amdgcn_sched_barrier(0);
      }
      __syncthreads();
      continue;
    }
#pragma unroll
    for (int t = 0; t < 4; ++t) {
      xf0[t] = *reinterpret_cast<const bf16x8*>(buf + x_row_off + t * 2048 + coff0);
      wf0[t] = *reinterpret_cast<const bf16x8*>(buf + w_row_off + t * 2048 + coff0);
    }
    __builtin_amdgcn_sched_barrier(0);
#pragma unroll
    for (int i = 0; i < 8; ++i) {
      const int mt = i >> 1, nt0 = (i & 1) * 2;
      acc[mt][nt0] = __builtin_amdgcn_mfma_f32_16x16x32_bf16(wf0[nt0], xf0[mt], acc[mt][nt0], 0, 0, 0);
      acc[mt][nt0 + 1] = __builtin_amdgcn_mfma_f32_16x16x32_bf16(wf0[nt0 + 1], xf0[mt], acc[mt][nt0 + 1], 0, 0, 0);
      if (i < 4) {
        xf1[i] = *reinterpret_cast<const bf16x8*>(buf + x_row_off + i * 2048 + coff1);
        glds16(a_src[i] + kn, sbase + i * 1024);
      } else {
        wf1[i - 4] = *reinterpret_cast<const bf16x8*>(buf + w_row_off + (i - 4) * 2048 + coff1);
        glds16(w_src[i - 4] + kn, sbase + TILE_BYTES + (i - 4) * 1024);
      }
      __builtin_amdgcn_sched_barrier(0);
    }
#pragma unroll
    for (int mt = 0; mt < 4; ++mt)
#pragma unroll
      for (int nt = 0; nt < 4; ++nt)
        acc[mt][nt] = __builtin_amdgcn_mfma_f32_16x16x32_bf16(wf1[nt], xf1[mt], acc[mt][nt], 0, 0, 0);
    __builtin_amdgcn_sched_barrier(0);
    __syncthreads();
  }

  if constexpr (F8) fp8_scale_acc<4>(p, acc, m0 + wr * 64, n0 + wc * 64, lane);
  const int mrow = m0 + wr * 64 + (lane & 15);
  const int ncol = n0 + wc * 64 + (lane >> 4) * 4;
  if (EPI != SF_EPI_F32 && (p.N & 7) == 0 && (p.ldo & 7) == 0)
    gemm_epilogue_lds<EPI, 4>(p, acc, m0 + wr * 64, n0 + wc * 64, smem + wave * 8192, lane);
  else
    gemm_epilogue<EPI, 4>(p, acc, mrow, ncol);
}


constexpr int PP_THREADS = 512;

template <int MT>
struct PPCfg {
  static constexpr int BM = 32 * MT;
  static constexpr int A_BYTES = BM * 128;
  static constexpr int B_BYTES = 256 * 128;
  static constexpr int STAGE = A_BYTES + B_BYTES;
  static constexpr int LDS = 2 * STAGE;
  static constexpr int PA = (2 * MT + 7) / 8;
};

template <int EPI, int MT, bool F8>
__global__ __launch_bounds__(PP_THREADS) void gemm_pp_kernel(GemmP p) {
  using Cfg = PPCfg<MT>;
  constexpr int BMp = Cfg::BM, PA = Cfg::PA;
  constexpr int HQA = (MT + 1) / 2, HQB = MT / 2;
  extern __shared__ __attribute__((aligned(16))) char smem[];
  const int tid = threadIdx.x;
  const int lane = tid & 63;
  const int wave = __builtin_amdgcn_readfirstlane(tid >> 6);
  const int grp = wave >> 2, wc = wave & 3;

  const int nwg = gridDim.x, bid = blockIdx.x;
  const int wg = sf_xcd_remap(bid, nwg);
  constexpr int GROUP_M = MT >= 6 ? 4 : 8;
  const int width = GROUP_M * p.tiles_n;
  const int group = wg / width, first_m = group * GROUP_M;
  const int gsz = min(p.tiles_m - first_m, GROUP_M);
  const int in_group = wg - group * width;
  const int tm = first_m + in_group % gsz, tn = in_group / gsz;
  const int m0 = tm * BMp, n0 = tn * 256;

  const bf16_t* a_src[2][PA];
  const bf16_t* w_src[2][2];
#pragma unroll
  for (int h = 0; h < 2; ++h) {
#pragma unroll
    for (int i = 0; i < PA; ++i) {
      const int r = h * (BMp / 2) + (wave + 8 * i) * 8 + (lane >> 3);
      const int c = (lane & 7) ^ ((r >> 1) & 7);
      a_src[h][i] = p.a + (long)min(m0 + r, p.M - 1) * p.lda + c * 8;
    }
#pragma unroll
    for (int i = 0; i < 2; ++i) {
      const int r = h * 128 + (wave + 8 * i) * 8 + (lane >> 3);
      const int c = (lane & 7) ^ ((r >> 1) & 7);
      w_src[h][i] = p.w + (long)min(n0 + r, p.N - 1) * p.ldw + c * 8;
    }
  }
  auto dma_a = [&](int h, int kt) {
    char* base = smem + (kt & 1) * Cfg::STAGE + h * (Cfg::A_BYTES / 2) + wave * 1024;
#pragma unroll
    for (int i = 0; i < PA; ++i)
      if (wave + 8 * i < 2 * MT) glds16(a_src[h][i] + kt * BK, base + i * 8192);
  };
  auto dma_b = [&](int h, int kt) {
    char* base = smem + (kt & 1) * Cfg::STAGE + Cfg::A_BYTES + h * (Cfg::B_BYTES / 2) + wave * 1024;
#pragma unroll
    for (int i = 0; i < 2; ++i) glds16(w_src[h][i] + kt * BK, base + i * 8192);
  };

  const int i16 = lane & 15, kq = lane >> 4;
  const int swz = (i16 >> 1) & 7;
  const int x_row_off = (grp * (BMp / 2) + i16) * 128;
  const int w_row_off = Cfg::A_BYTES + (wc * 64 + i16) * 128;
  const int coff[2] = {((0 + kq) ^ swz) << 4, ((4 + kq) ^ swz) << 4};

  f32x4 acc[MT][4];
#pragma unroll
  for (int i = 0; i < MT; ++i)
#pragma unroll
    for (int j = 0; j < 4; ++j) acc[i][j] = f32x4{0.f, 0.f, 0.f, 0.f};
  bf16x8 af[HQA][2], bfr[4][2];

#ifdef SF_STAMP
  unsigned long long* stamp = (EPI == SF_EPI_BIAS && p.gate_e0) ? reinterpret_cast<unsigned long long*>(const_cast<bf16_t*>(p.gate_e0)) + ((long)bid * 2 + grp) * 8 : nullptr;
  if (stamp && (tid & 255) == 0) { stamp[0] = __builtin_amdgcn_s_memtime(); stamp[4] = __builtin_amdgcn_s_memrealtime(); }
#endif
  const int nk = p.K / BK;
  dma_a(0, 0); dma_a(1, 0); dma_b(0, 0); dma_b(1, 0);
  if (nk > 1) { dma_b(0, 1); dma_b(1, 1); asm volatile("s_waitcnt vmcnt(4)" ::: "memory"); }
  else asm volatile("s_waitcnt vmcnt(0)" ::: "memory");
  __builtin_amdgcn_s_barrier();
#ifdef SF_STAMP
  if (stamp && (tid & 255) == 0) stamp[1] = __builtin_amdgcn_s_memtime();
#endif
  if (grp == 1) __builtin_amdgcn_s_barrier();

  auto end_load_segment = [&]() {
    __builtin_amdgcn_s_waitcnt(0xc07f);
    __builtin_amdgcn_sched_barrier(0);
    __builtin_amdgcn_s_barrier();
    __builtin_amdgcn_sched_barrier(0);
  };
  auto cluster = [&](auto qc, int c0) {
    constexpr int q = decltype(qc)::value, NQ = q == 0 ? HQA : HQB;
    __builtin_amdgcn_s_setprio(1);
    if constexpr (F8) {
#pragma unroll
      for (int mt = 0; mt < NQ; ++mt)
#pragma unroll
        for (int nt = 0; nt < 2; ++nt)
          acc[q * HQA + mt][c0 + nt] = mfma_f8(bfr[c0 + nt][0], bfr[c0 + nt][1], af[mt][0], af[mt][1], acc[q * HQA + mt][c0 + nt]);
    } else {
#pragma unroll
      for (int ks = 0; ks < 2; ++ks)
#pragma unroll
        for (int mt = 0; mt < NQ; ++mt)
#pragma unroll
          for (int nt = 0; nt < 2; ++nt)
            acc[q * HQA + mt][c0 + nt] = __builtin_amdgcn_mfma_f32_16x16x32_bf16(bfr[c0 + nt][ks], af[mt][ks], acc[q * HQA + mt][c0 + nt], 0, 0, 0);
    }
    __builtin_amdgcn_s_setprio(0);
    __builtin_amdgcn_sched_barrier(0);
    __builtin_amdgcn_s_barrier();
    __builtin_amdgcn_sched_barrier(0);
  };
  auto read_a = [&](const char* buf, auto qc) {
    constexpr int q = decltype(qc)::value, NQ = q == 0 ? HQA : HQB;
#pragma unroll
    for (int mt = 0; mt < NQ; ++mt)
#pragma unroll
      for (int ks = 0; ks < 2; ++ks)
        af[mt][ks] = *reinterpret_cast<const bf16x8*>(buf + x_row_off + (q * HQA + mt) * 2048 + coff[ks]);
  };
  auto read_b = [&](const char* buf, int c0) {
#pragma unroll
    for (int nt = 0; nt < 2; ++nt)
#pragma unroll
      for (int ks = 0; ks < 2; ++ks)
        bfr[c0 + nt][ks] = *reinterpret_cast<const bf16x8*>(buf + w_row_off + (c0 + nt) * 2048 + coff[ks]);
  };

  constexpr std::integral_constant<int, 0> Q0{};
  constexpr std::integral_constant<int, 1> Q1{};
  for (int kt = 0; kt < nk; ++kt) {
    const char* buf = smem + (kt & 1) * Cfg::STAGE;
    const bool more1 = kt + 1 < nk, more2 = kt + 2 < nk;
    read_a(buf, Q0);
    read_b(buf, 0);
    if (more1) dma_a(0, kt + 1);
    end_load_segment();
    cluster(Q0, 0);
    read_b(buf, 2);
    if (more1) dma_a(1, kt + 1);
    end_load_segment();
    cluster(Q0, 2);
    read_a(buf, Q1);
    if (more2) dma_b(0, kt + 2);
    end_load_segment();
    cluster(Q1, 2);
    if (more2) {
      dma_b(1, kt + 2);
      asm volatile("s_waitcnt vmcnt(4)" ::: "memory");
    } else {
      asm volatile("s_waitcnt vmcnt(0)" ::: "memory");
    }
    end_load_segment();
    cluster(Q1, 0);
  }
  if (grp == 0) __builtin_amdgcn_s_barrier();
#ifdef SF_STAMP
  if (stamp && (tid & 255) == 0) stamp[2] = __builtin_amdgcn_s_memtime();
#endif

  const int m_base = m0 + grp * (BMp / 2), n_base = n0 + wc * 64;
  if constexpr (F8) fp8_scale_acc<MT>(p, acc, m_base, n_base, lane);
  if ((p.N & 7) == 0 && (p.ldo & 7) == 0)
    gemm_epilogue_lds<EPI, MT>(p, acc, m_base, n_base, smem + wave * (MT * 2048), lane);
  else
    gemm_epilogue<EPI, MT>(p, acc, m_base + (lane & 15), n_base + (lane >> 4) * 4);
#ifdef SF_STAMP
  asm volatile("s_waitcnt vmcnt(0)" ::: "memory");
  if (stamp && (tid & 255) == 0) { stamp[3] = __builtin_amdgcn_s_memtime(); stamp[5] = __builtin_amdgcn_s_memrealtime(); }
#endif
}

constexpr int PP2_A = 128 * 128, PP2_B = 256 * 128;
constexpr int PP2_LDS = 3 * (PP2_A + PP2_B);

template <int EPI, bool F8>
__global__ __launch_bounds__(PP_THREADS) void gemm_pp2_kernel(GemmP p) {
  extern __shared__ __attribute__((aligned(16))) char smem[];
  const int tid = threadIdx.x;
  const int lane = tid & 63;
  const int wave = __builtin_amdgcn_readfirstlane(tid >> 6);
  const int grp = wave >> 2, wc = wave & 3;

  const int nwg = gridDim.x, bid = blockIdx.x;
  const int wg = sf_xcd_remap(bid, nwg);
  constexpr int GROUP_M = 8;
  const int width = GROUP_M * p.tiles_n;
  const int group = wg / width, first_m = group * GROUP_M;
  const int gsz = min(p.tiles_m - first_m, GROUP_M);
  const int in_group = wg - group * width;
  const int tm = first_m + in_group % gsz, tn = in_group / gsz;
  const int m0 = tm * 128, n0 = tn * 256;

  const bf16_t* a_src[2];
  const bf16_t* w_src[4];
#pragma unroll
  for (int i = 0; i < 2; ++i) {
    const int r = (wave + 8 * i) * 8 + (lane >> 3);
    a_src[i] = p.a + (long)min(m0 + r, p.M - 1) * p.lda + ((lane & 7) ^ ((r >> 1) & 7)) * 8;
  }
#pragma unroll
  for (int i = 0; i < 4; ++i) {
    const int r = (wave + 8 * i) * 8 + (lane >> 3);
    w_src[i] = p.w + (long)min(n0 + r, p.N - 1) * p.ldw + ((lane & 7) ^ ((r >> 1) & 7)) * 8;
  }
  auto dma_a = [&](int slot, int kt) {
    char* base = smem + slot * PP2_A + wave * 1024;
#pragma unroll
    for (int i = 0; i < 2; ++i) glds16(a_src[i] + kt * BK, base + i * 8192);
  };
  auto dma_b = [&](int slot, int kt) {
    char* base = smem + 3 * PP2_A + slot * PP2_B + wave * 1024;
#pragma unroll
    for (int i = 0; i < 4; ++i) glds16(w_src[i] + kt * BK, base + i * 8192);
  };

  const int i16 = lane & 15, kq = lane >> 4;
  const int swz = (i16 >> 1) & 7;
  const int x_row_off = (grp * 64 + i16) * 128;
  const int w_row_off = 3 * PP2_A + (wc * 64 + i16) * 128;
  const int coff[2] = {((0 + kq) ^ swz) << 4, ((4 + kq) ^ swz) << 4};

  f32x4 acc[4][4];
#pragma unroll
  for (int i = 0; i < 4; ++i)
#pragma unroll
    for (int j = 0; j < 4; ++j) acc[i][j] = f32x4{0.f, 0.f, 0.f, 0.f};
  bf16x8 af[4][2], bfr[4][2];

  const int nk = p.K / BK;
  dma_a(0, 0); dma_b(0, 0);
  if (nk > 1) { dma_a(1, 1); dma_b(1, 1); asm volatile("s_waitcnt vmcnt(6)" ::: "memory"); }
  else asm volatile("s_waitcnt vmcnt(0)" ::: "memory");
  __builtin_amdgcn_s_barrier();
  if (grp == 1) __builtin_amdgcn_s_barrier();

  auto end_load_segment = [&]() {
    __builtin_amdgcn_s_waitcnt(0xc07f);
    __builtin_amdgcn_sched_barrier(0);
    __builtin_amdgcn_s_barrier();
    __builtin_amdgcn_sched_barrier(0);
  };
  auto cluster = [&](int c0) {
    __builtin_amdgcn_s_setprio(1);
    if constexpr (F8) {
#pragma unroll
      for (int mt = 0; mt < 4; ++mt)
#pragma unroll
        for (int nt = 0; nt < 2; ++nt)
          acc[mt][c0 + nt] = mfma_f8(bfr[c0 + nt][0], bfr[c0 + nt][1], af[mt][0], af[mt][1], acc[mt][c0 + nt]);
    } else {
#pragma unroll
      for (int ks = 0; ks < 2; ++ks)
#pragma unroll
        for (int mt = 0; mt < 4; ++mt)
#pragma unroll
          for (int nt = 0; nt < 2; ++nt)
            acc[mt][c0 + nt] = __builtin_amdgcn_mfma_f32_16x16x32_bf16(bfr[c0 + nt][ks], af[mt][ks], acc[mt][c0 + nt], 0, 0, 0);
    }
    __builtin_amdgcn_s_setprio(0);
    __builtin_amdgcn_sched_barrier(0);
    __builtin_amdgcn_s_barrier();
    __builtin_amdgcn_sched_barrier(0);
  };

  int slot = 0;
  for (int kt = 0; kt < nk; ++kt) {
    const char* abuf = smem + slot * PP2_A;
    const char* bbuf = smem + slot * PP2_B;
    const int nslot = slot == 0 ? 2 : slot - 1;
    const bool more2 = kt + 2 < nk;
#pragma unroll
    for (int mt = 0; mt < 4; ++mt)
#pragma unroll
      for (int ks = 0; ks < 2; ++ks) af[mt][ks] = *reinterpret_cast<const bf16x8*>(abuf + x_row_off + mt * 2048 + coff[ks]);
#pragma unroll
    for (int nt = 0; nt < 2; ++nt)
#pragma unroll
      for (int ks = 0; ks < 2; ++ks) bfr[nt][ks] = *reinterpret_cast<const bf16x8*>(bbuf + w_row_off + nt * 2048 + coff[ks]);
    if (more2) dma_a(nslot, kt + 2);
    end_load_segment();
    cluster(0);
#pragma unroll
    for (int nt = 2; nt < 4; ++nt)
#pragma unroll
      for (int ks = 0; ks < 2; ++ks) bfr[nt][ks] = *reinterpret_cast<const bf16x8*>(bbuf + w_row_off + nt * 2048 + coff[ks]);
    if (more2) {
      dma_b(nslot, kt + 2);
      asm volatile("s_waitcnt vmcnt(6)" ::: "memory");
    } else {
      asm volatile("s_waitcnt vmcnt(0)" ::: "memory");
    }
    end_load_segment();
    cluster(2);
    slot = slot == 2 ? 0 : slot + 1;
  }
  if (grp == 0) __builtin_amdgcn_s_barrier();

  const int m_base = m0 + grp * 64, n_base = n0 + wc * 64;
  if constexpr (F8) fp8_scale_acc<4>(p, acc, m_base, n_base, lane);
  if ((p.N & 7) == 0 && (p.ldo & 7) == 0)
    gemm_epilogue_lds<EPI, 4>(p, acc, m_base, n_base, smem + wave * 8192, lane);
  else
    gemm_epilogue<EPI, 4>(p, acc, m_base + (lane & 15), n_base + (lane >> 4) * 4);
}

template <int EPI, bool F8>
int launch_pp2(GemmP& p, hipStream_t s) {
  static bool attr = false;
  if (!attr) {
    (void)hipFuncSetAttribute(reinterpret_cast<const void*>(&gemm_pp2_kernel<EPI, F8>), hipFuncAttributeMaxDynamicSharedMemorySize, PP2_LDS);
    attr = true;
  }
  p.tiles_m = (p.M + 127) / 128;
  p.tiles_n = (p.N + 255) / 256;
  hipLaunchKernelGGL((gemm_pp2_kernel<EPI, F8>), dim3(p.tiles_m * p.tiles_n), dim3(PP_THREADS), PP2_LDS, s, p);
  return 0;
}

template <bool F8>
int launch_pp2_epi(GemmP& p, int epilogue, hipStream_t s) {
  switch (epilogue) {
    case SF_EPI_BIAS: return launch_pp2<SF_EPI_BIAS, F8>(p, s);
    case SF_EPI_BIAS_GELU: return launch_pp2<SF_EPI_BIAS_GELU, F8>(p, s);
    case SF_EPI_BIAS_RESID: return launch_pp2<SF_EPI_BIAS_RESID, F8>(p, s);
    case SF_EPI_BIAS_GATE_RESID: return launch_pp2<SF_EPI_BIAS_GATE_RESID, F8>(p, s);
    default: return -1;
  }
}

template <int EPI, int MT, bool F8>
int launch_pp(GemmP& p, hipStream_t s) {
  using Cfg = PPCfg<MT>;
  static bool attr = false;
  if (!attr) {
    (void)hipFuncSetAttribute(reinterpret_cast<const void*>(&gemm_pp_kernel<EPI, MT, F8>), hipFuncAttributeMaxDynamicSharedMemorySize, Cfg::LDS);
    attr = true;
  }
  p.tiles_m = (p.M + Cfg::BM - 1) / Cfg::BM;
  p.tiles_n = (p.N + 255) / 256;
  hipLaunchKernelGGL((gemm_pp_kernel<EPI, MT, F8>), dim3(p.tiles_m * p.tiles_n), dim3(PP_THREADS), Cfg::LDS, s, p);
  return 0;
}

template <int MT, bool F8>
int launch_pp_epi(GemmP& p, int epilogue, hipStream_t s) {
  switch (epilogue) {
    case SF_EPI_BIAS: return launch_pp<SF_EPI_BIAS, MT, F8>(p, s);
    case SF_EPI_BIAS_GELU: return launch_pp<SF_EPI_BIAS_GELU, MT, F8>(p, s);
    case SF_EPI_BIAS_RESID: return launch_pp<SF_EPI_BIAS_RESID, MT, F8>(p, s);
    case SF_EPI_BIAS_GATE_RESID: return launch_pp<SF_EPI_BIAS_GATE_RESID, MT, F8>(p, s);
    default: return -1;
  }
}

int check_args(const sf_gemm_args* a, const char* name, int bk) {
  SF_CHECK(a != nullptr, "%s: null args", name);
  SF_CHECK(a->M > 0 && a->N > 0 && a->K > 0, "%s: empty problem M=%d N=%d K=%d", name, a->M, a->N, a->K);
  SF_CHECK(a->K % bk == 0, "%s: K=%d must be a multiple of %d", name, a->K, bk);
  SF_CHECK(a->N % 4 == 0, "%s: N=%d must be a multiple of 4", name, a->N);
  SF_CHECK(a->lda % (bk / 8) == 0 && a->ldw % (bk / 8) == 0 && a->ldo % 4 == 0, "%s: lda/ldw must be multiples of %d, ldo of 4", name, bk / 8);
  SF_CHECK(a->lda >= a->K && a->ldw >= a->K && a->ldo >= a->N, "%s: leading dimension too small", name);
  SF_CHECK(a->a && a->w && a->out, "%s: null tensor", name);
  SF_CHECK(((uintptr_t)a->a % 16 == 0) && ((uintptr_t)a->w % 16 == 0) && ((uintptr_t)a->out % 8 == 0), "%s: misaligned tensor", name);
  if (a->epilogue == SF_EPI_BIAS_RESID || a->epilogue == SF_EPI_BIAS_GATE_RESID) {
    SF_CHECK(a->resid != nullptr && a->ldr >= a->N && a->ldr % 4 == 0, "%s: residual epilogue needs resid/ldr", name);
  }
  if (a->epilogue == SF_EPI_BIAS_GATE_RESID) {
    SF_CHECK(a->gate_mod && a->gate_e0 && a->rows_per_group > 0, "%s: gate epilogue needs gate_mod/gate_e0/rows_per_group", name);
  }
  SF_CHECK(a->structure >= SF_GEMM_AUTO && a->structure <= SF_GEMM_PP192, "%s: unknown structure %d", name, a->structure);
  return 0;
}

template <bool F8>
int run_gemm(const sf_gemm_args* a, GemmP& p, const char* name, hipStream_t s) {
  int st = a->structure;
  const int nk = p.K / BK;
  const bool pp_ok = a->batch <= 1 && a->epilogue != SF_EPI_F32 && nk >= 2;
  if (st == SF_GEMM_AUTO) {
    st = SF_GEMM_T128;
    if (pp_ok && a->M >= 1024 && a->N >= 1024 && a->K >= 512) {
      static const struct { int st, rows; double rel; } cand[] = {
          {SF_GEMM_PP256, 256, 1.00}, {SF_GEMM_PP224, 224, 1.02}, {SF_GEMM_PP192, 192, 1.05}, {SF_GEMM_PP128, 128, 1.14}};
      const long tn = (a->N + 255) / 256;
      double best = 1e30;
      for (const auto& c : cand) {
        const long tiles = (long)((a->M + c.rows - 1) / c.rows) * tn;
        const double cost = (double)((tiles + 255) / 256) * (c.rows / 256.0 * c.rel + 0.04);
        if (cost < best - 1e-9) { best = cost; st = c.st; }
      }
    }
  }
  const bool is_pp = st == SF_GEMM_PP256 || st == SF_GEMM_PP224 || st == SF_GEMM_PP192 || st == SF_GEMM_PP128;
  if (is_pp && !pp_ok) st = SF_GEMM_T128;
  else if (is_pp) {
    const int rc = st == SF_GEMM_PP256 ? launch_pp_epi<8, F8>(p, a->epilogue, s)
                 : st == SF_GEMM_PP224 ? launch_pp_epi<7, F8>(p, a->epilogue, s)
                 : st == SF_GEMM_PP192 ? launch_pp_epi<6, F8>(p, a->epilogue, s) : launch_pp2_epi<F8>(p, a->epilogue, s);
    SF_CHECK(rc == 0, "%s: unknown epilogue %d", name, a->epilogue);
    SF_HIP_LAUNCH_CHECK(name);
    return 0;
  }
  const int batch = a->batch > 1 ? a->batch : 1;
  p.a_bs = a->a_bstride; p.w_bs = a->w_bstride; p.o_bs = a->o_bstride; p.r_bs = a->r_bstride;
  SF_CHECK(batch == 1 || (a->a_bstride % 8 == 0 && a->w_bstride % 8 == 0 && a->o_bstride % 4 == 0 && a->r_bstride % 4 == 0),
           "%s: batch strides must keep 16-byte (operands) / 8-byte (output) alignment", name);
  const dim3 grid(p.tiles_m * p.tiles_n, batch), block(GEMM_THREADS);
  switch (a->epilogue) {
    case SF_EPI_BIAS: hipLaunchKernelGGL((gemm_bf16_kernel<SF_EPI_BIAS, F8>), grid, block, GEMM_LDS, s, p); break;
    case SF_EPI_BIAS_GELU: hipLaunchKernelGGL((gemm_bf16_kernel<SF_EPI_BIAS_GELU, F8>), grid, block, GEMM_LDS, s, p); break;
    case SF_EPI_BIAS_RESID: hipLaunchKernelGGL((gemm_bf16_kernel<SF_EPI_BIAS_RESID, F8>), grid, block, GEMM_LDS, s, p); break;
    case SF_EPI_BIAS_GATE_RESID: hipLaunchKernelGGL((gemm_bf16_kernel<SF_EPI_BIAS_GATE_RESID, F8>), grid, block, GEMM_LDS, s, p); break;
    case SF_EPI_F32:
      if constexpr (F8) {
        SF_CHECK(false, "%s: the raw fp32 epilogue is bf16-only", name);
      } else {
        SF_CHECK((uintptr_t)a->out % 16 == 0, "%s: fp32 output must be 16-byte aligned", name);
        hipLaunchKernelGGL((gemm_bf16_kernel<SF_EPI_F32, false>), grid, block, GEMM_LDS, s, p);
      }
      break;
    default: SF_CHECK(false, "%s: unknown epilogue %d", name, a->epilogue);
  }
  SF_HIP_LAUNCH_CHECK(name);
  return 0;
}

void fill_params(const sf_gemm_args* a, GemmP& p, int unit) {
  p.a = (const bf16_t*)a->a; p.w = (const bf16_t*)a->w; p.bias = (const bf16_t*)a->bias;
  p.out = (bf16_t*)a->out; p.resid = (const bf16_t*)a->resid;
  p.gate_mod = (const bf16_t*)a->gate_mod; p.gate_e0 = (const bf16_t*)a->gate_e0;
  p.gate_group_stride = a->gate_group_stride; p.rows_per_group = a->rows_per_group;
  p.M = a->M; p.N = a->N; p.K = a->K / unit; p.lda = a->lda / unit; p.ldw = a->ldw / unit; p.ldo = a->ldo; p.ldr = a->ldr;
  p.tiles_n = (a->N + BN - 1) / BN;
  p.tiles_m = (a->M + BM - 1) / BM;
  p.a_scale = nullptr; p.w_scale = nullptr; p.rows_per_seg = 1;
}

}

extern "C" int sf_gemm_bf16(const sf_gemm_args* a, void* stream) {
  if (const int rc = check_args(a, "sf_gemm_bf16", BK)) return rc;
  GemmP p;
  fill_params(a, p, 1);
  return run_gemm<false>(a, p, "sf_gemm_bf16", (hipStream_t)stream);
}

extern "C" int sf_gemm_fp8(const sf_gemm_args* a, const float* a_scale, int rows_per_segment, const float* w_scale, void* stream) {
  if (const int rc = check_args(a, "sf_gemm_fp8", 2 * BK)) return rc;
  SF_CHECK(a->batch <= 1, "sf_gemm_fp8: batched products are bf16-only");
  SF_CHECK(a_scale && w_scale && rows_per_segment > 0, "sf_gemm_fp8: needs a_scale, w_scale and rows_per_segment > 0");
  SF_CHECK((uintptr_t)w_scale % 16 == 0, "sf_gemm_fp8: w_scale must be 16-byte aligned");
  GemmP p;
  fill_params(a, p, 2);
  p.a_scale = a_scale; p.w_scale = w_scale; p.rows_per_seg = rows_per_segment;
  return run_gemm<true>(a, p, "sf_gemm_fp8", (hipStream_t)stream);
}
```

self-forcing_amd/csrc/sf_host.h:

```cpp
#pragma once
#include <cstring>
#include "sf_common.h"
#include "../../include/sf_hip.h"

#define SF_TRY(expr)            \
  do {                          \
    int rc__ = (expr);          \
    if (rc__ != 0) return rc__; \
  } while (0)

inline int sf_hip_ok(hipError_t e, const char* who, const char* what) {
  SF_CHECK(e == hipSuccess, "%s: %s failed: %s", who, what, hipGetErrorString(e));
  return 0;
}

struct Carve {
  char* base;
  size_t off;
  explicit Carve(void* p) : base((char*)p), off(0) {}
  char* take(size_t bytes) {
    char* r = base ? base + off : nullptr;
    off += (bytes + 255) & ~(size_t)255;
    return r;
  }
};

struct Gemm {
  sf_gemm_args g;
  const void* wq = nullptr;
  const float* w_scale = nullptr;
  int rows_per_segment = 0;
  Gemm(const void* a, int lda, const void* w, int ldw, void* out, int ldo, int M, int N, int K) {
    memset(&g, 0, sizeof(g));
    g.a = a; g.lda = lda; g.w = w; g.ldw = ldw; g.out = out; g.ldo = ldo; g.M = M; g.N = N; g.K = K;
    g.epilogue = SF_EPI_BIAS;
    g.rows_per_group = 1;
  }
  Gemm& bias(const void* b) { g.bias = b; return *this; }
  Gemm& epi(int e) { g.epilogue = e; return *this; }
  Gemm& resid(const void* r, int ldr) { g.resid = r; g.ldr = ldr; return *this; }
  Gemm& gate(const void* gate_mod, const void* gate_e0, long group_stride, int rows_per_group) {
    g.gate_mod = gate_mod; g.gate_e0 = gate_e0; g.gate_group_stride = group_stride; g.rows_per_group = rows_per_group;
    return *this;
  }
  Gemm& batch(int n, long a_bstride, long w_bstride, long o_bstride) {
    g.batch = n; g.a_bstride = a_bstride; g.w_bstride = w_bstride; g.o_bstride = o_bstride;
    return *this;
  }
  Gemm& fp8w(const void* w_e4m3, const float* scale, int rows_per_seg) {
    wq = w_e4m3; w_scale = scale; rows_per_segment = rows_per_seg;
    return *this;
  }
  int bf16(void* stream) const { return sf_gemm_bf16(&g, stream); }
  int fp8(const void* aq, const float* a_scale, void* stream) const {
    sf_gemm_args q = g;
    q.a = aq; q.lda = g.K; q.w = wq;
    return sf_gemm_fp8(&q, a_scale, rows_per_segment, w_scale, stream);
  }
};
```

self-forcing_amd/ops.py:

```python
from __future__ import annotations

import ctypes as C
from typing import Optional

import torch

from . import _lib
from . import torch_ops
from ._lib import (ACT_GELU, ACT_NONE, ACT_SILU, CONV_BIAS, CONV_BIAS_CLAMP_F32, CONV_BIAS_RESID, EPI_BIAS,
                   EPI_BIAS_GATE_RESID, EPI_BIAS_GELU, EPI_BIAS_RESID, EPI_F32, ConvArgs, GemmArgs, check, lib)

Tensor = torch.Tensor
_EPI = {"bias": EPI_BIAS, "gelu": EPI_BIAS_GELU, "resid": EPI_BIAS_RESID, "gate_resid": EPI_BIAS_GATE_RESID,
        "f32": EPI_F32}
_ACT = {None: ACT_NONE, "none": ACT_NONE, "silu": ACT_SILU, "gelu": ACT_GELU}


def stream_handle() -> int:
    return torch.cuda.current_stream().cuda_stream


def _bf16(t: Tensor, name: str) -> Tensor:
    if not t.is_cuda:
        raise ValueError(f"{name}: expected a CUDA/ROCm tensor (the HIP path has no CPU fallback)")
    if t.dtype != torch.bfloat16:
        raise ValueError(f"{name}: expected bfloat16, got {t.dtype}")
    return t


def _rows(t: Tensor, name: str, dtype=torch.bfloat16) -> Tensor:
    if not t.is_cuda:
        raise ValueError(f"{name}: expected a CUDA/ROCm tensor (the HIP path has no CPU fallback)")
    if t.dtype != dtype:
        raise ValueError(f"{name}: expected {dtype}, got {t.dtype}")
    if t.dim() != 2 or t.stride(1) != 1:
        raise ValueError(f"{name}: expected a 2-D tensor with contiguous rows, got shape {tuple(t.shape)} strides {t.stride()}")
    return t


def _ptr(t: Optional[Tensor]) -> Optional[int]:
    return None if t is None else t.data_ptr()


def _timestep(t: Tensor):
    if t.dtype == torch.int64:
        return t.contiguous(), 1
    return t.to(torch.float32).contiguous(), 0


def gemm(a: Tensor, w: Tensor, bias: Optional[Tensor] = None, epilogue: str = "bias",
         resid: Optional[Tensor] = None, gate_mod: Optional[Tensor] = None, gate_e0: Optional[Tensor] = None,
         rows_per_group: int = 1, out: Optional[Tensor] = None, structure: str = "auto") -> Tensor:
    a, w = _rows(a, "a"), _rows(w, "w")
    epi, st = _EPI[epilogue], _lib.GEMM_STRUCTURES[structure]
    if out is None:
        return torch.ops.sf_hip.gemm(a, w, bias, epi, resid, gate_mod, gate_e0, rows_per_group, st)
    torch.ops.sf_hip.gemm_out(out, a, w, bias, epi, resid, gate_mod, gate_e0, rows_per_group, st)
    return out


def small_linear(x: Tensor, w: Tensor, bias: Optional[Tensor], act_in=None, act_out=None) -> Tensor:
    x, w = _rows(x, "x").contiguous(), _rows(w, "w").contiguous()
    M, K = x.shape
    N = w.shape[0]
    out = torch.empty(M, N, dtype=torch.bfloat16, device=x.device)
    check(lib().sf_small_linear(x.data_ptr(), w.data_ptr(), _ptr(bias), out.data_ptr(), M, N, K,
                                _ACT[act_in], _ACT[act_out], stream_handle()), "sf_small_linear")
    return out


def quantize_fp8(x: Tensor, rows_per_segment: Optional[int] = None):
    x = _rows(x, "x")
    return torch.ops.sf_hip.quantize_fp8(x, rows_per_segment or x.shape[0])


def gemm_fp8(a: Tensor, a_scale: Tensor, w: Tensor, w_scale: Tensor, bias: Optional[Tensor] = None, epilogue: str = "bias",
             resid: Optional[Tensor] = None, gate_mod: Optional[Tensor] = None, gate_e0: Optional[Tensor] = None,
             rows_per_group: int = 1, rows_per_segment: Optional[int] = None, structure: str = "auto") -> Tensor:
    a, w = _rows(a, "a", torch.float8_e4m3fn), _rows(w, "w", torch.float8_e4m3fn)
    if w_scale.numel() == 1:
        w_scale = w_scale.reshape(1).expand(w.shape[0])
    return torch.ops.sf_hip.gemm_fp8(a, a_scale.float().contiguous(), rows_per_segment or a.shape[0], w, w_scale.float().contiguous(), bias,
                                     _EPI[epilogue], resid, gate_mod, gate_e0, rows_per_group, _lib.GEMM_STRUCTURES[structure])


def small_linear_fp8(x: Tensor, w_q: Tensor, w_scale: Tensor, bias: Optional[Tensor], act_in=None, act_out=None,
                     rows_per_segment: Optional[int] = None) -> Tensor:
    x, w_q = _rows(x, "x").contiguous(), _rows(w_q, "w_q", torch.float8_e4m3fn).contiguous()
    M, K = x.shape
    N = w_q.shape[0]
    w_scale = (w_scale.reshape(1).expand(N) if w_scale.numel() == 1 else w_scale).float().contiguous()
    out = torch.empty(M, N, dtype=torch.bfloat16, device=x.device)
    check(lib().sf_small_linear_fp8(x.data_ptr(), w_q.data_ptr(), w_scale.data_ptr(), _ptr(bias), out.data_ptr(), M, N, K,
                                    rows_per_segment or M, _ACT[act_in], _ACT[act_out], stream_handle()), "sf_small_linear_fp8")
    return out


def sinusoid_embedding(t: Tensor, dim: int) -> Tensor:
    tt, is64 = _timestep(t.flatten())
    out = torch.empty(tt.numel(), dim, dtype=torch.bfloat16, device=t.device)
    check(lib().sf_sinusoid_embedding(tt.data_ptr(), is64, out.data_ptr(), tt.numel(), dim, stream_handle()),
          "sf_sinusoid_embedding")
    return out


def layernorm_modulate(x: Tensor, mod_shift: Tensor, mod_scale: Tensor, e0_shift: Tensor, e0_scale: Tensor,
                       rows_per_group: int, eps: float = 1e-6) -> Tensor:
    x = _rows(x, "x").contiguous()
    M, Cc = x.shape
    _rows(e0_shift, "e0_shift"), _rows(e0_scale, "e0_scale")
    if e0_shift.stride(0) != e0_scale.stride(0):
        raise ValueError("layernorm_modulate: e0_shift / e0_scale must share a row stride")
    out = torch.empty_like(x)
    check(lib().sf_layernorm_modulate(x.data_ptr(), out.data_ptr(), M, Cc, eps, mod_shift.data_ptr(), mod_scale.data_ptr(),
                                      e0_shift.data_ptr(), e0_scale.data_ptr(), e0_shift.stride(0), rows_per_group,
                                      stream_handle()), "sf_layernorm_modulate")
    return out


def layernorm_affine(x: Tensor, weight: Tensor, bias: Tensor, eps: float = 1e-6) -> Tensor:
    x = _rows(x, "x").contiguous()
    out = torch.empty_like(x)
    check(lib().sf_layernorm_affine(x.data_ptr(), weight.data_ptr(), bias.data_ptr(), out.data_ptr(), x.shape[0], x.shape[1],
                                    eps, stream_handle()), "sf_layernorm_affine")
    return out


def rmsnorm(x: Tensor, weight: Tensor, eps: float = 1e-6, out: Optional[Tensor] = None) -> Tensor:
    x = _rows(x, "x")
    if out is None:
        out = torch.empty(x.shape, dtype=torch.bfloat16, device=x.device)
    check(lib().sf_rmsnorm(x.data_ptr(), x.stride(0), weight.data_ptr(), out.data_ptr(), out.stride(0), x.shape[0], x.shape[1],
                           eps, stream_handle()), "sf_rmsnorm")
    return out


def qkv_norm_rope_cache(qkv: Tensor, norm_q_w: Tensor, norm_k_w: Tensor, k_cache: Tensor, v_cache: Tensor,
                        rope_cos: Tensor, rope_sin: Tensor, grid, write_start: int, start_frame: int,
                        eps: float = 1e-6) -> Tensor:
    qkv = _rows(qkv, "qkv").contiguous()
    B, S, H, D = k_cache.shape
    f, h, w = grid
    Cc = H * D
    if not (k_cache.is_contiguous() and v_cache.is_contiguous()):
        raise ValueError("qkv_norm_rope_cache: caches must be contiguous [B, S, H, D]")
    q = torch.empty(qkv.shape[0], Cc, dtype=torch.bfloat16, device=qkv.device)
    check(lib().sf_qkv_norm_rope_cache(qkv.data_ptr(), norm_q_w.data_ptr(), norm_k_w.data_ptr(), q.data_ptr(), k_cache.data_ptr(),
                                       v_cache.data_ptr(), rope_cos.data_ptr(), rope_sin.data_ptr(), B, f, h, w, Cc, H, S,
                                       write_start, start_frame, eps, stream_handle()), "sf_qkv_norm_rope_cache")
    return q


def kv_evict(cache: Tensor, sink: int, evict: int, keep: int, scratch: Tensor) -> None:
    B, S, H, D = cache.shape
    check(lib().sf_kv_evict(cache.data_ptr(), B, S, H * D, sink, evict, keep, scratch.data_ptr(),
                            scratch.numel() * scratch.element_size(), stream_handle()), "sf_kv_evict")


def attention(q: Tensor, k: Tensor, v: Tensor, structure: str = "auto", keys: Optional[Tensor] = None,
              log2w: Optional[Tensor] = None) -> Tensor:
    return torch.ops.sf_hip.attention(q, k, v, _lib.ATTN_STRUCTURES[structure], keys, log2w)


def attention_accum(q: Tensor, k: Tensor, v: Tensor, out: Tensor, structure: str = "auto") -> Tensor:
    torch.ops.sf_hip.attention_accum(q, k, v, out, _lib.ATTN_STRUCTURES[structure])
    return out


def cross_fold_scan(ck_cache, cv_cache) -> tuple:
    L, B = len(ck_cache), ck_cache[0].shape[0]
    keys = torch.empty(L, B, dtype=torch.int32, device=ck_cache[0].device)
    log2w = torch.empty(L, B, dtype=torch.float32, device=ck_cache[0].device)
    torch.ops.sf_hip.cross_fold_scan(list(ck_cache), list(cv_cache), keys, log2w)
    return keys, log2w


def patchify(x: Tensor) -> Tensor:
    x = _bf16(x, "x").contiguous()
    B, F, Cin, H, W = x.shape
    out = torch.empty(B * F * (H // 2) * (W // 2), Cin * 4, dtype=torch.bfloat16, device=x.device)
    check(lib().sf_patchify(x.data_ptr(), out.data_ptr(), B, F, Cin, H, W, stream_handle()), "sf_patchify")
    return out


def unpatchify_x0(head_out: Tensor, xt: Tensor, timestep: Tensor, sigmas: Tensor, timesteps: Tensor):
    xt = _bf16(xt, "xt").contiguous()
    B, F, Cout, H, W = xt.shape
    tt, is64 = _timestep(timestep)
    G = tt.shape[1]
    flow = torch.empty_like(xt)
    x0 = torch.empty_like(xt)
    check(lib().sf_unpatchify_x0(_rows(head_out, "head_out").contiguous().data_ptr(), xt.data_ptr(), tt.data_ptr(), is64,
                                 sigmas.data_ptr(), timesteps.data_ptr(), sigmas.numel(), flow.data_ptr(), x0.data_ptr(),
                                 B, F, G, Cout, H, W, stream_handle()), "sf_unpatchify_x0")
    return flow, x0


def add_noise(x0: Tensor, eps: Tensor, timestep: Tensor, sigmas: Tensor, timesteps: Tensor) -> Tensor:
    x0 = _bf16(x0, "x0").contiguous()
    eps = _bf16(eps, "eps").contiguous()
    tt, _ = _timestep(timestep.flatten())
    if tt.numel() != x0.shape[0]:
        raise ValueError(f"add_noise: {x0.shape[0]} samples but {tt.numel()} timesteps")
    return torch.ops.sf_hip.add_noise(x0, eps, tt, sigmas, timesteps)


LINCOMB_MAX = 6


def lincomb(tensors, coefs, out: Optional[Tensor] = None) -> Tensor:
    if not 1 <= len(tensors) <= LINCOMB_MAX or len(tensors) != len(coefs):
        raise ValueError(f"lincomb: 1..{LINCOMB_MAX} tensors with one coefficient each, got {len(tensors)} / {len(coefs)}")
    xs = [_bf16(t, f"tensors[{i}]").contiguous() for i, t in enumerate(tensors)]
    cf = [float(c) for c in coefs]
    if out is None:
        return torch.ops.sf_hip.lincomb(xs, cf)
    torch.ops.sf_hip.lincomb_out(out, xs, cf)
    return out


def conv_igemm(x: Tensor, w_packed: Tensor, bias: Tensor, kernel, t_out: int, upsample: bool = False,
               t_in_offset: int = 0, resid: Optional[Tensor] = None, interleave: bool = False,
               clamp_f32: bool = False, cin: Optional[int] = None, structure: str = "auto", stride=(1, 1)) -> Tensor:
    _bf16(x, "x"), _bf16(w_packed, "w_packed"), _bf16(bias, "bias")
    if x.dim() != 4 or not x.is_contiguous():
        raise ValueError("conv_igemm: x must be a contiguous [T, H, W, C] volume")
    tin, hin, win, c = x.shape
    kt, kh, kw = kernel
    cout = w_packed.shape[0]
    st, sh = stride
    H, W = (2 * hin, 2 * win) if upsample else (hin // 2, win // 2) if sh == 2 else (hin, win)
    if st * (t_out - 1) + kt + t_in_offset > tin:
        raise ValueError(f"conv_igemm: {tin} input frames do not cover {t_out} output frames (kt={kt}, offset={t_in_offset})")
    a = ConvArgs()
    a.x, a.w, a.bias = x.data_ptr(), w_packed.data_ptr(), bias.data_ptr()
    a.Tout, a.H, a.W, a.Hin, a.Win = t_out, H, W, hin, win
    a.Cin, a.Cout, a.kt, a.kh, a.kw = cin or c, cout, kt, kh, kw
    a.upsample, a.t_in_offset, a.ldw = int(upsample), t_in_offset, w_packed.stride(0)
    a.structure = _lib.CONV_STRUCTURES[structure]
    a.stride_t, a.stride_hw = st, sh
    if clamp_f32:
        out = torch.empty(t_out, cout, H, W, dtype=torch.float32, device=x.device)
        a.out_f32, a.epilogue = out.data_ptr(), CONV_BIAS_CLAMP_F32
    else:
        co = cout // 2 if interleave else cout
        out = torch.empty(2 * t_out if interleave else t_out, H, W, co, dtype=torch.bfloat16, device=x.device)
        a.out, a.ldo, a.epilogue = out.data_ptr(), co, CONV_BIAS
        a.interleave_c = co if interleave else 0
        if resid is not None:
            _bf16(resid, "resid")
            if tuple(resid.shape) != tuple(out.shape) or not resid.is_contiguous():
                raise ValueError("conv_igemm: resid must match the output volume")
            a.resid, a.ldr, a.epilogue = resid.data_ptr(), cout, CONV_BIAS_RESID
    check(lib().sf_conv_igemm(a, stream_handle()), "sf_conv_igemm")
    return out


def taehv_conv(x: Tensor, w_packed: Tensor, bias: Optional[Tensor], kt: int, t_out: int, epilogue: str = "bias_relu", upsample: bool = False,
               resid: Optional[Tensor] = None, tgrow: int = 1, clamp: bool = False, cin: Optional[int] = None) -> Tensor:
    _bf16(x, "x"), _bf16(w_packed, "w_packed")
    if bias is not None:
        _bf16(bias, "bias")
    if x.dim() != 4 or not x.is_contiguous():
        raise ValueError("taehv_conv: x must be a contiguous [T, H, W, C] volume")
    if epilogue not in _lib.TAEHV_EPILOGUES:
        raise ValueError(f"taehv_conv: unknown epilogue {epilogue!r}")
    tin, hin, win, c = x.shape
    if t_out - 1 + kt > tin:
        raise ValueError(f"taehv_conv: {tin} input frames do not cover {t_out} output frames (kt={kt})")
    cout = w_packed.shape[0]
    H, W = (2 * hin, 2 * win) if upsample else (hin, win)
    a = _lib.TaehvConvArgs()
    a.x, a.w, a.bias = x.data_ptr(), w_packed.data_ptr(), None if bias is None else bias.data_ptr()
    a.Tout, a.H, a.W, a.Cin, a.Cout, a.kt = t_out, H, W, cin or c, cout, kt
    a.upsample, a.ldw, a.tgrow, a.epilogue, a.clamp = int(upsample), w_packed.stride(0), tgrow, _lib.TAEHV_EPILOGUES[epilogue], int(clamp)
    if epilogue in ("head_f32", "latent_f32"):
        out = torch.empty(t_out, cout, H, W, dtype=torch.float32, device=x.device)
        a.out_f32 = out.data_ptr()
    else:
        if tgrow < 1 or cout % tgrow:
            raise ValueError(f"taehv_conv: tgrow={tgrow} does not divide Cout={cout}")
        co = cout // tgrow
        out = torch.empty(tgrow * t_out, H, W, co, dtype=torch.bfloat16, device=x.device)
        a.out, a.ldo = out.data_ptr(), co
        if resid is not None:
            _bf16(resid, "resid")
            if tuple(resid.shape) != tuple(out.shape) or not resid.is_contiguous():
                raise ValueError("taehv_conv: resid must match the output volume")
            a.resid, a.ldr = resid.data_ptr(), cout
    check(lib().sf_taehv_conv(a, stream_handle()), "sf_taehv_conv")
    return out


def taehv_encode_stem(pixels: Tensor, w_packed: Tensor, bias: Tensor, lead: int = 0) -> Tensor:
    _bf16(w_packed, "w_packed"), _bf16(bias, "bias")
    if not pixels.is_cuda or pixels.dtype not in (torch.bfloat16, torch.float32):
        raise ValueError("taehv_encode_stem: pixels must be a CUDA/ROCm bf16 or float32 tensor (the HIP path has no CPU fallback)")
    if pixels.dim() != 4 or pixels.shape[0] != 3 or not pixels[0].is_contiguous():
        raise ValueError(f"taehv_encode_stem: pixels must be [3, T, H, W] with contiguous frames, got {tuple(pixels.shape)}")
    if tuple(w_packed.shape) != (64, 32) or not w_packed.is_contiguous() or bias.numel() != 64:
        raise ValueError("taehv_encode_stem: w_packed [64, 32] and bias [64] expected")
    _, T, H, W = pixels.shape
    out = torch.empty(lead + T, H, W, 64, dtype=torch.bfloat16, device=pixels.device)
# ... 215 lines not shown
```

Measured before the change: 97.03.

## Write V columns of QKV GEMM directly into the KV cache

Adds a redirect epilogue to the bf16 and fp8 GEMMs so output columns from col0 onward are stored into per-segment destination bases. The DiT forward uses it to write the V part of the QKV projection straight into the V cache, and switches to a norm/rope kernel that skips the V copy. This removes one read and one write of the V activations per layer. In exchange it adds an overlap planner that falls back to the old path under eviction or aliasing between paired passes, plus extra epilogue branching in the GEMM.

New measurement: 97.24, median of 6. About the same (+0.2%).

```diff
diff --git a/include/sf_hip.h b/include/sf_hip.h
--- a/include/sf_hip.h
+++ b/include/sf_hip.h
@@ -46,10 +46,22 @@
 
 int sf_gemm_bf16(const sf_gemm_args* args, void* stream);
 
+#define SF_GEMM_REDIRECT_MAX 32
+typedef struct sf_gemm_redirect {
+  int32_t col0;
+  int32_t seg_rows;
+  int64_t ld;
+  int32_t n_seg;
+  void* seg_base[SF_GEMM_REDIRECT_MAX];
+} sf_gemm_redirect;
+int sf_gemm_bf16_redirect(const sf_gemm_args* args, const sf_gemm_redirect* redirect, void* stream);
+
 #define SF_FP8_AMAX_PARTS 1024
 int sf_quantize_fp8(const void* x, int ldx, int M, int K, int rows_per_segment, void* q_out, float* scale_out, void* stream);
 
 int sf_gemm_fp8(const sf_gemm_args* args, const float* a_scale, int rows_per_segment, const float* w_scale, void* stream);
+int sf_gemm_fp8_redirect(const sf_gemm_args* args, const float* a_scale, int rows_per_segment, const float* w_scale,
+                         const sf_gemm_redirect* redirect, void* stream);
 
 int sf_small_linear_fp8(const void* x, const void* w_q, const float* w_scale, const void* bias, void* out, int M, int N, int K,
                         int rows_per_segment, int act_in, int act_out, void* stream);
@@ -73,6 +85,10 @@
                            void* k_cache, void* v_cache, const float* rope_cos, const float* rope_sin,
                            int B, int f, int h, int w, int C, int num_heads, int64_t cache_tokens,
                            int write_start, int start_frame, float eps, void* stream);
+int sf_qk_norm_rope_cache(const void* qkv, const void* norm_q_w, const void* norm_k_w, void* q_out, void* k_cache,
+                          const float* rope_cos, const float* rope_sin, int B, int f, int h, int w, int C,
+                          int num_heads, int64_t cache_tokens, int write_start, int start_frame, float eps,
+                          void* stream);
 
 int sf_kv_evict(void* cache, int B, int64_t cache_tokens, int row_elems, int sink, int evict, int keep,
                 void* scratch, size_t scratch_bytes, void* stream);
@@ -190,6 +206,9 @@
 int sf_dit_forward_pair_fold(const sf_model* model, const sf_forward_args* context_pass, const sf_forward_args* next_pass,
                              const int32_t* cross_keys, const float* cross_log2w, void* stream);
 
+int sf_dit_v_redirect_plan(const sf_forward_args* pass0, const sf_forward_args* pass1, int dim);
+int sf_dit_v_redirect(int enable);
+
 
 int sf_patchify_i2v(const void* x, const void* y, void* cols, int B, int F, int x_channels, int y_channels, int pad_channels,
                     int H, int W, int64_t y_bstride, int64_t y_cstride, int64_t y_fstride, void* stream);
diff --git a/self-forcing_amd/_lib.py b/self-forcing_amd/_lib.py
--- a/self-forcing_amd/_lib.py
+++ b/self-forcing_amd/_lib.py
@@ -47,6 +47,14 @@
     ]
 
 
+GEMM_REDIRECT_MAX = 32
+
+
+class GemmRedirect(C.Structure):
+    _fields_ = [("col0", C.c_int32), ("seg_rows", C.c_int32), ("ld", C.c_int64), ("n_seg", C.c_int32),
+                ("seg_base", C.c_void_p * GEMM_REDIRECT_MAX)]
+
+
 class LayerWeights(C.Structure):
     _fields_ = [(n, C.c_void_p) for n in (
         "modulation", "norm3_w", "norm3_b", "qkv_w", "qkv_b", "norm_q_w", "norm_k_w", "o_w", "o_b",
@@ -243,9 +251,11 @@
     "sf_abi_version": (C.c_int, []),
     "sf_last_error": (C.c_char_p, []),
     "sf_gemm_bf16": (C.c_int, [C.POINTER(GemmArgs), _vp]),
+    "sf_gemm_bf16_redirect": (C.c_int, [C.POINTER(GemmArgs), C.POINTER(GemmRedirect), _vp]),
     "sf_small_linear": (C.c_int, [_vp, _vp, _vp, _vp, _i, _i, _i, _i, _i, _vp]),
     "sf_quantize_fp8": (C.c_int, [_vp, _i, _i, _i, _i, _vp, _vp, _vp]),
     "sf_gemm_fp8": (C.c_int, [C.POINTER(GemmArgs), _vp, _i, _vp, _vp]),
+    "sf_gemm_fp8_redirect": (C.c_int, [C.POINTER(GemmArgs), _vp, _i, _vp, C.POINTER(GemmRedirect), _vp]),
     "sf_small_linear_fp8": (C.c_int, [_vp, _vp, _vp, _vp, _vp, _i, _i, _i, _i, _i, _i, _vp]),
     "sf_sinusoid_embedding": (C.c_int, [_vp, _i, _vp, _i, _i, _vp]),
     "sf_layernorm_modulate": (C.c_int, [_vp, _vp, _i, _i, _f, _vp, _vp, _vp, _vp, _i64, _i, _vp]),
@@ -253,6 +263,7 @@
     "sf_rmsnorm": (C.c_int, [_vp, _i, _vp, _vp, _i, _i, _i, _f, _vp]),
     "sf_qkv_norm_rope_cache": (C.c_int, [_vp, _vp, _vp, _vp, _vp, _vp, _vp, _vp, _i, _i, _i, _i, _i, _i, _i64,
                                          _i, _i, _f, _vp]),
+    "sf_qk_norm_rope_cache": (C.c_int, [_vp, _vp, _vp, _vp, _vp, _vp, _vp, _i, _i, _i, _i, _i, _i, _i64, _i, _i, _f, _vp]),
     "sf_kv_evict": (C.c_int, [_vp, _i, _i64, _i, _i, _i, _i, _vp, _sz, _vp]),
     "sf_attention": (C.c_int, [_vp, _vp, _vp, _vp, _i, _i, _i, _i, _i64, _i64, _i64, _i64, _i64, _i64, _vp]),
     "sf_attention_ex": (C.c_int, [_vp, _vp, _vp, _vp, _i, _i, _i, _i, _i64, _i64, _i64, _i64, _i64, _i64, _i, _vp]),
@@ -268,6 +279,8 @@
     "sf_dit_forward_pair": (C.c_int, [C.POINTER(Model), C.POINTER(ForwardArgs), C.POINTER(ForwardArgs), _vp]),
     "sf_dit_forward_fold": (C.c_int, [C.POINTER(Model), C.POINTER(ForwardArgs), _vp, _vp, _vp]),
     "sf_dit_forward_pair_fold": (C.c_int, [C.POINTER(Model), C.POINTER(ForwardArgs), C.POINTER(ForwardArgs), _vp, _vp, _vp]),
+    "sf_dit_v_redirect_plan": (C.c_int, [C.POINTER(ForwardArgs), C.POINTER(ForwardArgs), _i]),
+    "sf_dit_v_redirect": (C.c_int, [_i]),
     "sf_patchify_i2v": (C.c_int, [_vp, _vp, _vp, _i, _i, _i, _i, _i, _i, _i, _i64, _i64, _i64, _vp]),
     "sf_layernorm_rows": (C.c_int, [_vp, _vp, _vp, _vp, _i, _i, _f, _vp]),
     "sf_i2v_assemble_y": (C.c_int, [_vp, _vp, _vp, _i, _i, _i, _i, _i, _i64, _i64, _i, _vp]),
@@ -370,6 +383,8 @@
     ver = handle.sf_abi_version()
     if ver != ABI_VERSION:
         raise SfHipError(f"{LIB_PATH}: ABI version {ver}, expected {ABI_VERSION}; rebuild")
+    if os.environ.get("SF_V_REDIRECT", "") != "":
+        handle.sf_dit_v_redirect(1 if int(os.environ["SF_V_REDIRECT"]) else 0)
     _lib = handle
     return handle
 
diff --git a/self-forcing_amd/csrc/dit_forward.hip b/self-forcing_amd/csrc/dit_forward.hip
--- a/self-forcing_amd/csrc/dit_forward.hip
+++ b/self-forcing_amd/csrc/dit_forward.hip
@@ -67,6 +67,24 @@
   return w;
 }
 
+}
+
+extern "C" int sf_dit_v_redirect_plan(const sf_forward_args* p0, const sf_forward_args* p1, int dim) {
+  if (!p0 || dim <= 0 || (2 * (int64_t)dim) % 64 != 0 || dim % 8 != 0) return 0;
+  if (!p1) return 1;
+  if (p0->evict > 0 || p1->evict > 0) return 0;
+  const int64_t L = (int64_t)p0->frames * (p0->lat_h / 2) * (p0->lat_w / 2);
+  const int64_t w1 = p1->write_start, w0 = p0->write_start;
+  const bool in_window = w1 < p0->attn_end && w1 + L > p0->attn_start;
+  const bool in_rows = w1 < w0 + L && w1 + L > w0;
+  return (in_window || in_rows) ? 0 : 2;
+}
+
+static int g_v_redirect = 1;
+extern "C" int sf_dit_v_redirect(int enable) {
+  const int old = __atomic_load_n(&g_v_redirect, __ATOMIC_RELAXED);
+  if (enable >= 0) __atomic_store_n(&g_v_redirect, enable ? 1 : 0, __ATOMIC_RELAXED);
+  return old;
 }
 
 extern "C" size_t sf_dit_workspace_bytes(const sf_model* model, int batch, int frames, int lat_h, int lat_w, int groups) {
@@ -213,22 +231,38 @@
     }
   }
 
+  const int v_plan = sf_dit_v_redirect(-1) ? sf_dit_v_redirect_plan(ps[0], np == 2 ? ps[1] : nullptr, C) : 0;
   for (int l = 0; l < m->num_layers; ++l) {
     const sf_layer_weights& lw = m->layers_host[l];
     const sf_layer_fp8& lq = f8 ? m->layers_fp8_host[l] : no_fp8;
     const void* mod = lw.modulation;
     const bool last_layer = l == m->num_layers - 1;
     SF_TRY(sf_layernorm_modulate(ws.x, ws.xn, Mt, C, m->eps, bptr(mod, 0), bptr(mod, C), bptr(ws.e0, 0), bptr(ws.e0, C), 6L * C, rpg, stream));
-    SF_TRY(lin(Gemm(ws.xn, C, lw.qkv_w, C, ws.qkv, 3 * C, Mt, 3 * C, C).bias(lw.qkv_b).fp8w(lq.qkv_q, lq.qkv_s, M)));
+    const bool v_direct = v_plan != 0 && (uintptr_t)a->v_cache_host[l] % 16 == 0;
+    auto evict = [&](const sf_forward_args* q) -> int {
+      if (q->evict <= 0) return 0;
+      SF_TRY(sf_kv_evict(q->k_cache_host[l], B, q->cache_tokens, C, q->sink_tokens, q->evict, q->keep, q->evict_scratch, q->evict_scratch_bytes, stream));
+      return sf_kv_evict(q->v_cache_host[l], B, q->cache_tokens, C, q->sink_tokens, q->evict, q->keep, q->evict_scratch, q->evict_scratch_bytes, stream);
+    };
+    sf_gemm_redirect vr;
+    if (v_direct) {
+      if (np == 1) SF_TRY(evict(a));
+      vr.col0 = 2 * C; vr.seg_rows = L; vr.ld = C; vr.n_seg = np * B;
+      for (int p = 0; p < np; ++p)
+        for (int b = 0; b < B; ++b) vr.seg_base[p * B + b] = (void*)bptr(a->v_cache_host[l], ((size_t)b * a->cache_tokens + ps[p]->write_start) * C);
+    }
+    SF_TRY(lin(Gemm(ws.xn, C, lw.qkv_w, C, ws.qkv, 3 * C, Mt, 3 * C, C).bias(lw.qkv_b).fp8w(lq.qkv_q, lq.qkv_s, M).redirect(v_direct ? &vr : nullptr)));
     for (int p = 0; p < np; ++p) {
       const sf_forward_args* q = ps[p];
       const size_t roff = (size_t)p * M;
-      if (q->evict > 0) {
-        SF_TRY(sf_kv_evict(q->k_cache_host[l], B, q->cache_tokens, C, q->sink_tokens, q->evict, q->keep, q->evict_scratch, q->evict_scratch_bytes, stream));
-        SF_TRY(sf_kv_evict(q->v_cache_host[l], B, q->cache_tokens, C, q->sink_tokens, q->evict, q->keep, q->evict_scratch, q->evict_scratch_bytes, stream));
+      if (!v_direct) {
+        SF_TRY(evict(q));
+        SF_TRY(sf_qkv_norm_rope_cache(bptr(ws.qkv, roff * 3 * C), lw.norm_q_w, lw.norm_k_w, (void*)bptr(ws.q, roff * C), q->k_cache_host[l], q->v_cache_host[l],
+                                      m->rope_cos, m->rope_sin, B, F, h, w, C, m->num_heads, q->cache_tokens, q->write_start, q->start_frame, m->eps, stream));
+      } else {
+        SF_TRY(sf_qk_norm_rope_cache(bptr(ws.qkv, roff * 3 * C), lw.norm_q_w, lw.norm_k_w, (void*)bptr(ws.q, roff * C), q->k_cache_host[l], m->rope_cos,
+                                     m->rope_sin, B, F, h, w, C, m->num_heads, q->cache_tokens, q->write_start, q->start_frame, m->eps, stream));
       }
-      SF_TRY(sf_qkv_norm_rope_cache(bptr(ws.qkv, roff * 3 * C), lw.norm_q_w, lw.norm_k_w, (void*)bptr(ws.q, roff * C), q->k_cache_host[l], q->v_cache_host[l],
-                                    m->rope_cos, m->rope_sin, B, F, h, w, C, m->num_heads, q->cache_tokens, q->write_start, q->start_frame, m->eps, stream));
       if (q->cache_only && last_layer) continue;
       SF_TRY(sf_attention(bptr(ws.q, roff * C), bptr(q->k_cache_host[l], (size_t)q->attn_start * C), bptr(q->v_cache_host[l], (size_t)q->attn_start * C),
                           (void*)bptr(ws.att, roff * C), B, m->num_heads, L, q->attn_end - q->attn_start, C, (long)L * C, C, cache_b, C, (long)L * C, stream));
diff --git a/self-forcing_amd/csrc/elementwise.hip b/self-forcing_amd/csrc/elementwise.hip
--- a/self-forcing_amd/csrc/elementwise.hip
+++ b/self-forcing_amd/csrc/elementwise.hip
@@ -126,7 +126,7 @@
   }
 }
 
-template <int NCH>
+template <int NCH, bool COPY_V>
 __global__ __launch_bounds__(256) void qkv_norm_rope_cache_kernel(
     const bf16_t* __restrict__ qkv, const bf16_t* __restrict__ wq, const bf16_t* __restrict__ wk,
     bf16_t* __restrict__ q_out, bf16_t* __restrict__ k_cache, bf16_t* __restrict__ v_cache,
@@ -142,10 +142,12 @@
   const bf16_t* src = qkv + (long)row * 3 * C;
   const long crow = ((long)b * cache_tokens + write_start + t) * C;
 
-#pragma unroll
-  for (int i = 0; i < NCH; ++i) {
-    const int e = (i * 64 + lane) * 8;
-    *reinterpret_cast<u32x4*>(v_cache + crow + e) = *reinterpret_cast<const u32x4*>(src + 2 * C + e);
+  if constexpr (COPY_V) {
+#pragma unroll
+    for (int i = 0; i < NCH; ++i) {
+      const int e = (i * 64 + lane) * 8;
+      *reinterpret_cast<u32x4*>(v_cache + crow + e) = *reinterpret_cast<const u32x4*>(src + 2 * C + e);
+    }
   }
 
 #pragma unroll
@@ -394,31 +396,48 @@
   return 0;
 }
 
+static int qkv_norm_rope_cache(const char* name, const void* qkv, const void* norm_q_w, const void* norm_k_w, void* q_out, void* k_cache,
+                               void* v_cache, bool copy_v, const float* rope_cos, const float* rope_sin, int B, int f, int h, int w, int C,
+                               int num_heads, int64_t cache_tokens, int write_start, int start_frame, float eps, void* stream) {
+  SF_CHECK(qkv && norm_q_w && norm_k_w && q_out && k_cache && (v_cache || !copy_v) && rope_cos && rope_sin, "%s: null tensor", name);
+  SF_CHECK(B > 0 && f > 0 && h > 0 && w > 0 && channels_ok(C), "%s: unsupported shape", name);
+  SF_CHECK(num_heads > 0 && C == num_heads * 128, "%s: head_dim must be 128 (C=%d heads=%d)", name, C, num_heads);
+  const int L = f * h * w;
+  SF_CHECK(write_start >= 0 && (int64_t)write_start + L <= cache_tokens, "%s: cache overflow: write_start=%d + L=%d > capacity=%lld", name,
+           write_start, L, (long long)cache_tokens);
+  SF_CHECK(start_frame >= 0 && start_frame + f <= 1024 && h <= 1024 && w <= 1024, "%s: RoPE position out of the 1024-entry table", name);
+  const int rows = B * L;
+  const dim3 grid((rows + ROWS_PER_BLOCK - 1) / ROWS_PER_BLOCK), block(256);
+  hipStream_t s = (hipStream_t)stream;
+  const int c = 64, c1 = c / 3, c0 = c - 2 * c1;
+#define SF_QKV_LAUNCH(N, V)                                                                                                       \
+  hipLaunchKernelGGL((qkv_norm_rope_cache_kernel<N, V>), grid, block, 0, s, (const bf16_t*)qkv, (const bf16_t*)norm_q_w,          \
+                     (const bf16_t*)norm_k_w, (bf16_t*)q_out, (bf16_t*)k_cache, (bf16_t*)v_cache, rope_cos, rope_sin, rows, L, h, w, C, \
+                     (long)cache_tokens, write_start, start_frame, eps, c0, c1)
+  switch (C / 512) {
+#define SF_QKV_CASE(N) \
+  case N: if (copy_v) SF_QKV_LAUNCH(N, true); else SF_QKV_LAUNCH(N, false); break;
+    SF_QKV_CASE(1) SF_QKV_CASE(2) SF_QKV_CASE(3) SF_QKV_CASE(4) SF_QKV_CASE(5) SF_QKV_CASE(6) SF_QKV_CASE(8) SF_QKV_CASE(10)
+#undef SF_QKV_CASE
+  }
+#undef SF_QKV_LAUNCH
+  SF_HIP_LAUNCH_CHECK(name);
+  return 0;
+}
+
 extern "C" int sf_qkv_norm_rope_cache(const void* qkv, const void* norm_q_w, const void* norm_k_w, void* q_out,
                                       void* k_cache, void* v_cache, const float* rope_cos, const float* rope_sin,
                                       int B, int f, int h, int w, int C, int num_heads, int64_t cache_tokens,
                                       int write_start, int start_frame, float eps, void* stream) {
-  SF_CHECK(qkv && norm_q_w && norm_k_w && q_out && k_cache && v_cache && rope_cos && rope_sin, "sf_qkv_norm_rope_cache: null tensor");
-  SF_CHECK(B > 0 && f > 0 && h > 0 && w > 0 && channels_ok(C), "sf_qkv_norm_rope_cache: unsupported shape");
-  SF_CHECK(num_heads > 0 && C == num_heads * 128, "sf_qkv_norm_rope_cache: head_dim must be 128 (C=%d heads=%d)", C, num_heads);
-  const int L = f * h * w;
-  SF_CHECK(write_start >= 0 && (int64_t)write_start + L <= cache_tokens, "sf_qkv_norm_rope_cache: cache overflow: write_start=%d + L=%d > capacity=%lld",
-           write_start, L, (long long)cache_tokens);
-  SF_CHECK(start_frame >= 0 && start_frame + f <= 1024 && h <= 1024 && w <= 1024, "sf_qkv_norm_rope_cache: RoPE position out of the 1024-entry table");
-  const int rows = B * L;
-  const dim3 grid((rows + ROWS_PER_BLOCK - 1) / ROWS_PER_BLOCK), block(256);
-  hipStream_t s = (hipStream_t)stream;
-  const int c = 64, c1 = c / 3, c0 = c - 2 * c1;
-  switch (C / 512) {
-#define SF_QKV_CASE(N)                                                                                                   \
-  case N: hipLaunchKernelGGL((qkv_norm_rope_cache_kernel<N>), grid, block, 0, s, (const bf16_t*)qkv, (const bf16_t*)norm_q_w, \
-                             (const bf16_t*)norm_k_w, (bf16_t*)q_out, (bf16_t*)k_cache, (bf16_t*)v_cache, rope_cos, rope_sin,  \
-                             rows, L, h, w, C, (long)cache_tokens, write_start, start_frame, eps, c0, c1); break;
-    SF_QKV_CASE(1) SF_QKV_CASE(2) SF_QKV_CASE(3) SF_QKV_CASE(4) SF_QKV_CASE(5) SF_QKV_CASE(6) SF_QKV_CASE(8) SF_QKV_CASE(10)
-#undef SF_QKV_CASE
-  }
-  SF_HIP_LAUNCH_CHECK("sf_qkv_norm_rope_cache");
-  return 0;
+  return qkv_norm_rope_cache("sf_qkv_norm_rope_cache", qkv, norm_q_w, norm_k_w, q_out, k_cache, v_cache, true, rope_cos, rope_sin, B, f, h, w, C,
+                             num_heads, cache_tokens, write_start, start_frame, eps, stream);
+}
+
+extern "C" int sf_qk_norm_rope_cache(const void* qkv, const void* norm_q_w, const void* norm_k_w, void* q_out, void* k_cache,
+                                     const float* rope_cos, const float* rope_sin, int B, int f, int h, int w, int C, int num_heads,
+                                     int64_t cache_tokens, int write_start, int start_frame, float eps, void* stream) {
+  return qkv_norm_rope_cache("sf_qk_norm_rope_cache", qkv, norm_q_w, norm_k_w, q_out, k_cache, nullptr, false, rope_cos, rope_sin, B, f, h, w, C,
+                             num_heads, cache_tokens, write_start, start_frame, eps, stream);
 }
 
 extern "C" int sf_kv_evict(void* cache, int B, int64_t cache_tokens, int row_elems, int sink, int evict, int keep,
diff --git a/self-forcing_amd/csrc/gemm_bf16.hip b/self-forcing_amd/csrc/gemm_bf16.hip
--- a/self-forcing_amd/csrc/gemm_bf16.hip
+++ b/self-forcing_amd/csrc/gemm_bf16.hip
@@ -29,6 +29,21 @@
   int rows_per_seg;
 };
 
+struct GemmRd {
+  int col0, seg_rows;
+  long ld;
+  bf16_t* base[SF_GEMM_REDIRECT_MAX];
+};
+struct GemmPRd : GemmP {
+  GemmRd rd;
+};
+template <class P> constexpr bool has_rd = std::is_same<P, GemmPRd>::value;
+
+__device__ __forceinline__ bf16_t* redirect_ptr(const GemmRd& rd, int m, int n) {
+  const int seg = m / rd.seg_rows;
+  return rd.base[seg] + (long)(m - seg * rd.seg_rows) * rd.ld + (n - rd.col0);
+}
+
 typedef int i32x4 __attribute__((ext_vector_type(4)));
 typedef int i32x8 __attribute__((ext_vector_type(8)));
 
@@ -84,8 +99,8 @@
   return o;
 }
 
-template <int EPI, int MT>
-__device__ __forceinline__ void gemm_epilogue(const GemmP& p, f32x4 (&acc)[MT][4], int mrow, int ncol) {
+template <int EPI, int MT, class P>
+__device__ __forceinline__ void gemm_epilogue(const P& p, f32x4 (&acc)[MT][4], int mrow, int ncol) {
 #pragma unroll
   for (int mt = 0; mt < MT; ++mt) {
     const int m = mrow + mt * 16;
@@ -100,6 +115,12 @@
         *reinterpret_cast<f32x4*>(reinterpret_cast<float*>(p.out) + (long)m * p.ldo + n) = acc[mt][nt];
         continue;
       }
+      if constexpr (has_rd<P>) {
+        if (n >= p.rd.col0) {
+          *reinterpret_cast<bf16x4*>(redirect_ptr(p.rd, m, n)) = epi_apply<EPI>(p, acc[mt][nt], m, n, e0row);
+          continue;
+        }
+      }
       *reinterpret_cast<bf16x4*>(p.out + (long)m * p.ldo + n) = epi_apply<EPI>(p, acc[mt][nt], m, n, e0row);
     }
   }
@@ -128,8 +149,8 @@
   return o;
 }
 
-template <int EPI, int MT>
-__device__ __forceinline__ void gemm_epilogue_lds(const GemmP& p, f32x4 (&acc)[MT][4], int m_base, int n_base, char* wbuf, int lane) {
+template <int EPI, int MT, class P>
+__device__ __forceinline__ void gemm_epilogue_lds(const P& p, f32x4 (&acc)[MT][4], int m_base, int n_base, char* wbuf, int lane) {
   const int r16 = lane & 15, cg = lane >> 4;
   constexpr bool GATE = EPI == SF_EPI_BIAS_GATE_RESID;
   constexpr bool RESID = EPI == SF_EPI_BIAS_RESID || EPI == SF_EPI_BIAS_GATE_RESID;
@@ -180,6 +201,27 @@
   }
   __builtin_amdgcn_s_waitcnt(0xc07f);
   const int rr = lane >> 3, ch = lane & 7;
+  if constexpr (has_rd<P>) {
+    const GemmRd* rd = &p.rd;
+    if (n_base >= rd->col0) {
+      int seg = (m_base + rr) / rd->seg_rows, rem = m_base + rr - seg * rd->seg_rows;
+      const int n = n_base + ch * 8;
+      bf16_t* dst = rd->base[min(seg, SF_GEMM_REDIRECT_MAX - 1)] + (long)rem * rd->ld + (n - rd->col0);
+#pragma unroll
+      for (int i = 0; i < 2 * MT; ++i) {
+        const int row = i * 8 + rr;
+        const bf16x8 v = *reinterpret_cast<const bf16x8*>(wbuf + row * 128 + ((ch ^ (row & 7)) << 4));
+        if (m_base + row < p.M && n < p.N) *reinterpret_cast<bf16x8*>(dst) = v;
+        rem += 8;
+        dst += 8 * rd->ld;
+        if (rem >= rd->seg_rows) {
+          do { rem -= rd->seg_rows; ++seg; } while (rem >= rd->seg_rows);
+          dst = rd->base[min(seg, SF_GEMM_REDIRECT_MAX - 1)] + (long)rem * rd->ld + (n - rd->col0);
+        }
+      }
+      return;
+    }
+  }
 #pragma unroll
   for (int i = 0; i < 2 * MT; ++i) {
     const int row = i * 8 + rr;
@@ -189,14 +231,14 @@
   }
 }
 
-template <int EPI, bool F8>
-__global__ __launch_bounds__(GEMM_THREADS, 2) void gemm_bf16_kernel(GemmP p) {
+template <int EPI, bool F8, class P>
+__global__ __launch_bounds__(GEMM_THREADS, 2) void gemm_bf16_kernel(P p) {
   extern __shared__ __attribute__((aligned(16))) char smem[];
   const int tid = threadIdx.x;
   const int lane = tid & 63;
   const int wave = __builtin_amdgcn_readfirstlane(tid >> 6);
 
-  if (blockIdx.y) {
+  if (!has_rd<P> && blockIdx.y) {
     const long bz = blockIdx.y;
     p.a += bz * p.a_bs; p.w += bz * p.w_bs;
     if (EPI == SF_EPI_F32) p.out = reinterpret_cast<bf16_t*>(reinterpret_cast<float*>(p.out) + bz * p.o_bs); else p.out += bz * p.o_bs;
@@ -329,8 +371,8 @@
   static constexpr int PA = (2 * MT + 7) / 8;
 };
 
-template <int EPI, int MT, bool F8>
-__global__ __launch_bounds__(PP_THREADS) void gemm_pp_kernel(GemmP p) {
+template <int EPI, int MT, bool F8, class P>
+__global__ __launch_bounds__(PP_THREADS) void gemm_pp_kernel(P p) {
   using Cfg = PPCfg<MT>;
   constexpr int BMp = Cfg::BM, PA = Cfg::PA;
   constexpr int HQA = (MT + 1) / 2, HQB = MT / 2;
@@ -498,8 +540,8 @@
 constexpr int PP2_A = 128 * 128, PP2_B = 256 * 128;
 constexpr int PP2_LDS = 3 * (PP2_A + PP2_B);
 
-template <int EPI, bool F8>
-__global__ __launch_bounds__(PP_THREADS) void gemm_pp2_kernel(GemmP p) {
+template <int EPI, bool F8, class P>
+__global__ __launch_bounds__(PP_THREADS) void gemm_pp2_kernel(P p) {
   extern __shared__ __attribute__((aligned(16))) char smem[];
   const int tid = threadIdx.x;
   const int lane = tid & 63;
@@ -629,16 +671,16 @@
     gemm_epilogue<EPI, 4>(p, acc, m_base + (lane & 15), n_base + (lane >> 4) * 4);
 }
 
-template <int EPI, bool F8>
-int launch_pp2(GemmP& p, hipStream_t s) {
+template <int EPI, bool F8, class P>
+int launch_pp2(P& p, hipStream_t s) {
   static bool attr = false;
   if (!attr) {
-    (void)hipFuncSetAttribute(reinterpret_cast<const void*>(&gemm_pp2_kernel<EPI, F8>), hipFuncAttributeMaxDynamicSharedMemorySize, PP2_LDS);
+    (void)hipFuncSetAttribute(reinterpret_cast<const void*>(&gemm_pp2_kernel<EPI, F8, P>), hipFuncAttributeMaxDynamicSharedMemorySize, PP2_LDS);
     attr = true;
   }
   p.tiles_m = (p.M + 127) / 128;
   p.tiles_n = (p.N + 255) / 256;
-  hipLaunchKernelGGL((gemm_pp2_kernel<EPI, F8>), dim3(p.tiles_m * p.tiles_n), dim3(PP_THREADS), PP2_LDS, s, p);
+  hipLaunchKernelGGL((gemm_pp2_kernel<EPI, F8, P>), dim3(p.tiles_m * p.tiles_n), dim3(PP_THREADS), PP2_LDS, s, p);
   return 0;
 }
 
@@ -653,17 +695,17 @@
   }
 }
 
-template <int EPI, int MT, bool F8>
-int launch_pp(GemmP& p, hipStream_t s) {
+template <int EPI, int MT, bool F8, class P>
+int launch_pp(P& p, hipStream_t s) {
   using Cfg = PPCfg<MT>;
   static bool attr = false;
   if (!attr) {
-    (void)hipFuncSetAttribute(reinterpret_cast<const void*>(&gemm_pp_kernel<EPI, MT, F8>), hipFuncAttributeMaxDynamicSharedMemorySize, Cfg::LDS);
+    (void)hipFuncSetAttribute(reinterpret_cast<const void*>(&gemm_pp_kernel<EPI, MT, F8, P>), hipFuncAttributeMaxDynamicSharedMemorySize, Cfg::LDS);
     attr = true;
   }
   p.tiles_m = (p.M + Cfg::BM - 1) / Cfg::BM;
   p.tiles_n = (p.N + 255) / 256;
-  hipLaunchKernelGGL((gemm_pp_kernel<EPI, MT, F8>), dim3(p.tiles_m * p.tiles_n), dim3(PP_THREADS), Cfg::LDS, s, p);
+  hipLaunchKernelGGL((gemm_pp_kernel<EPI, MT, F8, P>), dim3(p.tiles_m * p.tiles_n), dim3(PP_THREADS), Cfg::LDS, s, p);
   return 0;
 }
 
@@ -698,7 +740,9 @@
 }
 
 template <bool F8>
-int run_gemm(const sf_gemm_args* a, GemmP& p, const char* name, hipStream_t s) {
+int run_gemm(const sf_gemm_args* a, GemmP& p, const GemmRd* rd, const char* name, hipStream_t s) {
+  GemmPRd prd;
+  if (rd) { static_cast<GemmP&>(prd) = p; prd.rd = *rd; }
   int st = a->structure;
   const int nk = p.K / BK;
   const bool pp_ok = a->batch <= 1 && a->epilogue != SF_EPI_F32 && nk >= 2;
@@ -718,7 +762,14 @@
   }
   const bool is_pp = st == SF_GEMM_PP256 || st == SF_GEMM_PP224 || st == SF_GEMM_PP192 || st == SF_GEMM_PP128;
   if (is_pp && !pp_ok) st = SF_GEMM_T128;
-  else if (is_pp) {
+  else if (is_pp && rd) {
+    if (st == SF_GEMM_PP256) launch_pp<SF_EPI_BIAS, 8, F8>(prd, s);
+    else if (st == SF_GEMM_PP224) launch_pp<SF_EPI_BIAS, 7, F8>(prd, s);
+    else if (st == SF_GEMM_PP192) launch_pp<SF_EPI_BIAS, 6, F8>(prd, s);
+    else launch_pp2<SF_EPI_BIAS, F8>(prd, s);
+    SF_HIP_LAUNCH_CHECK(name);
+    return 0;
+  } else if (is_pp) {
     const int rc = st == SF_GEMM_PP256 ? launch_pp_epi<8, F8>(p, a->epilogue, s)
                  : st == SF_GEMM_PP224 ? launch_pp_epi<7, F8>(p, a->epilogue, s)
                  : st == SF_GEMM_PP192 ? launch_pp_epi<6, F8>(p, a->epilogue, s) : launch_pp2_epi<F8>(p, a->epilogue, s);
@@ -731,17 +782,22 @@
   SF_CHECK(batch == 1 || (a->a_bstride % 8 == 0 && a->w_bstride % 8 == 0 && a->o_bstride % 4 == 0 && a->r_bstride % 4 == 0),
            "%s: batch strides must keep 16-byte (operands) / 8-byte (output) alignment", name);
   const dim3 grid(p.tiles_m * p.tiles_n, batch), block(GEMM_THREADS);
+  if (rd) {
+    hipLaunchKernelGGL((gemm_bf16_kernel<SF_EPI_BIAS, F8, GemmPRd>), grid, block, GEMM_LDS, s, prd);
+    SF_HIP_LAUNCH_CHECK(name);
+    return 0;
+  }
   switch (a->epilogue) {
-    case SF_EPI_BIAS: hipLaunchKernelGGL((gemm_bf16_kernel<SF_EPI_BIAS, F8>), grid, block, GEMM_LDS, s, p); break;
-    case SF_EPI_BIAS_GELU: hipLaunchKernelGGL((gemm_bf16_kernel<SF_EPI_BIAS_GELU, F8>), grid, block, GEMM_LDS, s, p); break;
-    case SF_EPI_BIAS_RESID: hipLaunchKernelGGL((gemm_bf16_kernel<SF_EPI_BIAS_RESID, F8>), grid, block, GEMM_LDS, s, p); break;
-    case SF_EPI_BIAS_GATE_RESID: hipLaunchKernelGGL((gemm_bf16_kernel<SF_EPI_BIAS_GATE_RESID, F8>), grid, block, GEMM_LDS, s, p); break;
+    case SF_EPI_BIAS: hipLaunchKernelGGL((gemm_bf16_kernel<SF_EPI_BIAS, F8, GemmP>), grid, block, GEMM_LDS, s, p); break;
+    case SF_EPI_BIAS_GELU: hipLaunchKernelGGL((gemm_bf16_kernel<SF_EPI_BIAS_GELU, F8, GemmP>), grid, block, GEMM_LDS, s, p); break;
+    case SF_EPI_BIAS_RESID: hipLaunchKernelGGL((gemm_bf16_kernel<SF_EPI_BIAS_RESID, F8, GemmP>), grid, block, GEMM_LDS, s, p); break;
+    case SF_EPI_BIAS_GATE_RESID: hipLaunchKernelGGL((gemm_bf16_kernel<SF_EPI_BIAS_GATE_RESID, F8, GemmP>), grid, block, GEMM_LDS, s, p); break;
     case SF_EPI_F32:
       if constexpr (F8) {
         SF_CHECK(false, "%s: the raw fp32 epilogue is bf16-only", name);
       } else {
         SF_CHECK((uintptr_t)a->out % 16 == 0, "%s: fp32 output must be 16-byte aligned", name);
-        hipLaunchKernelGGL((gemm_bf16_kernel<SF_EPI_F32, false>), grid, block, GEMM_LDS, s, p);
+        hipLaunchKernelGGL((gemm_bf16_kernel<SF_EPI_F32, false, GemmP>), grid, block, GEMM_LDS, s, p);
       }
       break;
     default: SF_CHECK(false, "%s: unknown epilogue %d", name, a->epilogue);
@@ -761,16 +817,40 @@
   p.a_scale = nullptr; p.w_scale = nullptr; p.rows_per_seg = 1;
 }
 
-}
-
-extern "C" int sf_gemm_bf16(const sf_gemm_args* a, void* stream) {
+int set_redirect(const sf_gemm_args* a, const sf_gemm_redirect* r, GemmRd& rd, const char* name) {
+  SF_CHECK(a->epilogue == SF_EPI_BIAS && a->batch <= 1, "%s: the redirect is built for the bias-only epilogue without a batch", name);
+  SF_CHECK(r->col0 >= 0 && r->col0 % 64 == 0 && r->col0 < a->N, "%s: redirect col0=%d must be a multiple of 64 below N=%d", name, r->col0, a->N);
+  SF_CHECK(r->seg_rows > 0 && r->n_seg > 0 && r->n_seg <= SF_GEMM_REDIRECT_MAX && ((int64_t)a->M + r->seg_rows - 1) / r->seg_rows <= r->n_seg,
+           "%s: redirect of M=%d rows in segments of %d needs more than the %d bases given (at most %d)", name, a->M, r->seg_rows, r->n_seg,
+           SF_GEMM_REDIRECT_MAX);
+  const int al = (a->N % 8 == 0 && a->ldo % 8 == 0) ? 8 : 4;
+  SF_CHECK(r->ld >= a->N - r->col0 && r->ld % al == 0, "%s: redirect ld=%lld must be >= %d and a multiple of %d", name, (long long)r->ld,
+           a->N - r->col0, al);
+  for (int i = 0; i < r->n_seg; ++i) {
+    SF_CHECK(r->seg_base[i] && (uintptr_t)r->seg_base[i] % (2 * al) == 0, "%s: redirect base %d is null or not %d-byte aligned", name, i, 2 * al);
+    rd.base[i] = (bf16_t*)r->seg_base[i];
+  }
+  for (int i = r->n_seg; i < SF_GEMM_REDIRECT_MAX; ++i) rd.base[i] = nullptr;
+  rd.col0 = r->col0; rd.seg_rows = r->seg_rows; rd.ld = r->ld;
+  return 0;
+}
+
+}
+
+extern "C" int sf_gemm_bf16_redirect(const sf_gemm_args* a, const sf_gemm_redirect* redirect, void* stream) {
   if (const int rc = check_args(a, "sf_gemm_bf16", BK)) return rc;
   GemmP p;
   fill_params(a, p, 1);
-  return run_gemm<false>(a, p, "sf_gemm_bf16", (hipStream_t)stream);
-}
-
-extern "C" int sf_gemm_fp8(const sf_gemm_args* a, const float* a_scale, int rows_per_segment, const float* w_scale, void* stream) {
+  GemmRd rd;
+  if (redirect)
+    if (const int rc = set_redirect(a, redirect, rd, "sf_gemm_bf16")) return rc;
+  return run_gemm<false>(a, p, redirect ? &rd : nullptr, "sf_gemm_bf16", (hipStream_t)stream);
+}
+
+extern "C" int sf_gemm_bf16(const sf_gemm_args* a, void* stream) { return sf_gemm_bf16_redirect(a, nullptr, stream); }
+
+extern "C" int sf_gemm_fp8_redirect(const sf_gemm_args* a, const float* a_scale, int rows_per_segment, const float* w_scale,
+                                    const sf_gemm_redirect* redirect, void* stream) {
   if (const int rc = check_args(a, "sf_gemm_fp8", 2 * BK)) return rc;
   SF_CHECK(a->batch <= 1, "sf_gemm_fp8: batched products are bf16-only");
   SF_CHECK(a_scale && w_scale && rows_per_segment > 0, "sf_gemm_fp8: needs a_scale, w_scale and rows_per_segment > 0");
@@ -778,5 +858,12 @@
   GemmP p;
   fill_params(a, p, 2);
   p.a_scale = a_scale; p.w_scale = w_scale; p.rows_per_seg = rows_per_segment;
-  return run_gemm<true>(a, p, "sf_gemm_fp8", (hipStream_t)stream);
-}
+  GemmRd rd;
+  if (redirect)
+    if (const int rc = set_redirect(a, redirect, rd, "sf_gemm_fp8")) return rc;
+  return run_gemm<true>(a, p, redirect ? &rd : nullptr, "sf_gemm_fp8", (hipStream_t)stream);
+}
+
+extern "C" int sf_gemm_fp8(const sf_gemm_args* a, const float* a_scale, int rows_per_segment, const float* w_scale, void* stream) {
+  return sf_gemm_fp8_redirect(a, a_scale, rows_per_segment, w_scale, nullptr, stream);
+}
diff --git a/self-forcing_amd/csrc/sf_host.h b/self-forcing_amd/csrc/sf_host.h
--- a/self-forcing_amd/csrc/sf_host.h
+++ b/self-forcing_amd/csrc/sf_host.h
@@ -30,6 +30,7 @@
   const void* wq = nullptr;
   const float* w_scale = nullptr;
   int rows_per_segment = 0;
+  const sf_gemm_redirect* rd = nullptr;
   Gemm(const void* a, int lda, const void* w, int ldw, void* out, int ldo, int M, int N, int K) {
     memset(&g, 0, sizeof(g));
     g.a = a; g.lda = lda; g.w = w; g.ldw = ldw; g.out = out; g.ldo = ldo; g.M = M; g.N = N; g.K = K;
@@ -51,10 +52,11 @@
     wq = w_e4m3; w_scale = scale; rows_per_segment = rows_per_seg;
     return *this;
   }
-  int bf16(void* stream) const { return sf_gemm_bf16(&g, stream); }
+  Gemm& redirect(const sf_gemm_redirect* r) { rd = r; return *this; }
+  int bf16(void* stream) const { return sf_gemm_bf16_redirect(&g, rd, stream); }
   int fp8(const void* aq, const float* a_scale, void* stream) const {
     sf_gemm_args q = g;
     q.a = aq; q.lda = g.K; q.w = wq;
-    return sf_gemm_fp8(&q, a_scale, rows_per_segment, w_scale, stream);
+    return sf_gemm_fp8_redirect(&q, a_scale, rows_per_segment, w_scale, rd, stream);
   }
 };
diff --git a/self-forcing_amd/ops.py b/self-forcing_amd/ops.py
--- a/self-forcing_amd/ops.py
+++ b/self-forcing_amd/ops.py
@@ -56,6 +56,45 @@
     if out is None:
         return torch.ops.sf_hip.gemm(a, w, bias, epi, resid, gate_mod, gate_e0, rows_per_group, st)
     torch.ops.sf_hip.gemm_out(out, a, w, bias, epi, resid, gate_mod, gate_e0, rows_per_group, st)
+    return out
+
+
+def gemm_redirect(a: Tensor, w: Tensor, bias: Optional[Tensor], dests, col0: int, seg_rows: int, out: Optional[Tensor] = None,
+                  structure: str = "auto", a_scale: Optional[Tensor] = None, w_scale: Optional[Tensor] = None,
+                  rows_per_segment: Optional[int] = None) -> Tensor:
+    fp8 = a_scale is not None
+    dt = torch.float8_e4m3fn if fp8 else torch.bfloat16
+    a, w = _rows(a, "a", dt), _rows(w, "w", dt)
+    M, K = a.shape
+    N = w.shape[0]
+    if out is None:
+        out = torch.empty(M, N, dtype=torch.bfloat16, device=a.device)
+    _rows(out, "out")
+    r = _lib.GemmRedirect()
+    r.col0, r.seg_rows, r.n_seg = col0, seg_rows, len(dests)
+    if not 0 < len(dests) <= _lib.GEMM_REDIRECT_MAX or seg_rows <= 0 or (M + seg_rows - 1) // seg_rows > len(dests):
+        raise ValueError(f"gemm_redirect: {len(dests)} destinations for {M} rows in segments of {seg_rows}")
+    for i, d in enumerate(dests):
+        _rows(d, f"dests[{i}]")
+        rows = min(seg_rows, M - i * seg_rows)
+        if d.shape[1] < N - col0 or d.shape[0] < rows or d.stride(0) != dests[0].stride(0):
+            raise ValueError(f"gemm_redirect: dests[{i}] {tuple(d.shape)} (row stride {d.stride(0)}) cannot take {rows} x {N - col0}")
+        r.seg_base[i] = d.data_ptr()
+    r.ld = dests[0].stride(0)
+    g = GemmArgs()
+    g.a, g.w, g.bias, g.out = a.data_ptr(), w.data_ptr(), _ptr(bias), out.data_ptr()
+    g.M, g.N, g.K = M, N, K
+    g.lda, g.ldw, g.ldo = a.stride(0), w.stride(0), out.stride(0)
+    g.epilogue, g.rows_per_group, g.structure = EPI_BIAS, 1, _lib.GEMM_STRUCTURES[structure]
+    if fp8:
+        a_scale, w_scale = a_scale.float().contiguous(), w_scale.float().contiguous()
+        rps = rows_per_segment or M
+        if a_scale.numel() != (M + rps - 1) // rps or w_scale.numel() != N or not (a_scale.is_cuda and w_scale.is_cuda):
+            raise ValueError(f"gemm_redirect: a_scale / w_scale must be CUDA vectors of {(M + rps - 1) // rps} / {N}")
+        check(lib().sf_gemm_fp8_redirect(g, a_scale.data_ptr(), rows_per_segment or M, w_scale.data_ptr(), r, stream_handle()),
+              "sf_gemm_fp8_redirect")
+    else:
+        check(lib().sf_gemm_bf16_redirect(g, r, stream_handle()), "sf_gemm_bf16_redirect")
     return out
 
 
@@ -149,6 +188,33 @@
                                        v_cache.data_ptr(), rope_cos.data_ptr(), rope_sin.data_ptr(), B, f, h, w, Cc, H, S,
                                        write_start, start_frame, eps, stream_handle()), "sf_qkv_norm_rope_cache")
     return q
+
+
+def qk_norm_rope_cache(qkv: Tensor, norm_q_w: Tensor, norm_k_w: Tensor, k_cache: Tensor, rope_cos: Tensor, rope_sin: Tensor, grid,
+                       write_start: int, start_frame: int, eps: float = 1e-6) -> Tensor:
+    qkv = _rows(qkv, "qkv").contiguous()
+    B, S, H, D = k_cache.shape
+    f, h, w = grid
+    if not k_cache.is_contiguous():
+        raise ValueError("qk_norm_rope_cache: the cache must be contiguous [B, S, H, D]")
+    q = torch.empty(qkv.shape[0], H * D, dtype=torch.bfloat16, device=qkv.device)
+    check(lib().sf_qk_norm_rope_cache(qkv.data_ptr(), norm_q_w.data_ptr(), norm_k_w.data_ptr(), q.data_ptr(), k_cache.data_ptr(),
+                                      rope_cos.data_ptr(), rope_sin.data_ptr(), B, f, h, w, H * D, H, S, write_start, start_frame, eps,
+                                      stream_handle()), "sf_qk_norm_rope_cache")
+    return q
+
+
+def dit_v_redirect(enable: Optional[bool] = None) -> bool:
+    return bool(lib().sf_dit_v_redirect(-1 if enable is None else int(bool(enable))))
+
+
+def dit_v_redirect_plan(pass0: dict, pass1: Optional[dict], dim: int) -> int:
+    def args(d):
+        a = _lib.ForwardArgs()
+        for k, v in d.items():
+            setattr(a, k, v)
+        return a
+    return lib().sf_dit_v_redirect_plan(args(pass0), None if pass1 is None else args(pass1), dim)
 
 
 def kv_evict(cache: Tensor, sink: int, evict: int, keep: int, scratch: Tensor) -> None:
```
